# google-research/se3ds

Measured on AMD Instinct MI355X. Metric: panoramas/sec (G+D train step) at 512x1024 RGB-D, higher is better.
Workload: dtype bf16; 1 GPU; configs/highres 512x1024 full GAN step train_g_d (G+D+hinge+depth+wc losses, clip, Adam, EMA), ResNet-101 gen_dims 128, per-GPU batch 8, d_step_per_g_step 1; per_gpu_batch=8, global_batch=8, parallelism=dp1

## Files before the change

### include/se3ds_hip.h

```cpp
#ifndef SE3DS_HIP_H_
#define SE3DS_HIP_H_

#include <stddef.h>
#include <stdint.h>

#ifdef __cplusplus
extern "C" {
#endif

#define SE3DS_OK 0
#define SE3DS_E_BADSHAPE (-1)
#define SE3DS_E_BADDTYPE (-2)
#define SE3DS_E_WORKSPACE (-3)
#define SE3DS_E_LAUNCH (-4)
#define SE3DS_E_UNSUPPORTED (-5)

#define SE3DS_F32 0
#define SE3DS_I32 1
#define SE3DS_U8 2
#define SE3DS_BF16 3
#define SE3DS_FEAT_BYTE_RANGE 0x100
#define SE3DS_XYZ1_ONES_PRESET 0x200

const char* se3ds_version(void);
// ... 31 lines not shown
                                  int feat_dtype, int n, int64_t m, int64_t capacity, int channels,
                                  int height, int width, float depth_scale, float input_void,
                                  float output_void, float* depth, float* feat, float* mask,
                                  float mask_void, void* workspace, size_t workspace_bytes,
                                  void* stream);

int se3ds_warp_views_to_target(const void* const* view_feats, int feat_dtype,
                               const float* const* view_depth, const float* const* view_position,
                               int views, int n, int height, int width, int channels,
                               float void_class, float depth_scale, const float* sin_el,
                               const float* cos_el, const float* sin_hd, const float* cos_hd,
                               float* mem_xyz1, void* mem_feats, int64_t capacity, int64_t m_offset,
                               const float* target, int out_height, int out_width,
                               float output_void, float* depth, float* feat, float* mask,
                               float mask_void, void* workspace, size_t workspace_bytes,
                               void* stream);

int se3ds_project_to_feat(const float* coords, const void* feats, int feat_dtype, int n, int64_t m,
                          int channels, int height, int width, float depth_scale,
                          float input_void, float output_void, float* depth, float* feat,
                          float* mask, float mask_void, void* workspace, size_t workspace_bytes,
                          void* stream);

int se3ds_splat_debug_indices(const void* workspace, int n, int64_t m, int32_t* idx_out,
                              float* z_out, void* stream);

int se3ds_debug_fast_fxy(const float* xyz, int64_t m, int width, int height, float* fx, float* fy,
                         int32_t* verdict, void* stream);

int se3ds_unproject_perspective(const int32_t* feats, const float* depth, const float* xs,
                                const float* ys, const float* kinv, int n, int height, int width,
                                int channels, float depth_scale, float* xyz, float* feats_out,
                                void* stream);

int se3ds_interp_bilinear(const float* grid, const float* query, int b, int height, int width,
                          int channels, int64_t q, int indexing_xy, float* out, void* stream);

int se3ds_rotate_coords(const float* rays, const float* matrix, int n, int64_t q, int src_h,
                        int src_w, float* out, void* stream);

int se3ds_perspective_coords(const float* rays, const float* w2i, int64_t q, int round_nearest,
                             float add, float* out, void* stream);

int se3ds_persp_from_equirect_coords(const float* kinv_t, const float* rot, int height, int width,
                                     int eq_h, int eq_w, float* out, void* stream);

int se3ds_perspective_to_pointcloud(const float* image, const float* depth, int ih, int iw,
                                    int channels, const float* rays, const float* w2i,
                                    int round_nearest, float pad_value, const float* sin_el,
                                    const float* cos_el, const float* sin_hd, const float* cos_hd,
                                    const float* position, int height, int width, float void_class,
                                    float depth_scale, float* xyz1, int32_t* feats_out, void* stream);
int se3ds_perspective_guidance(const float* pred_rgb, const float* pred_depth, int eq_h, int eq_w,
                               const float* kinv_t, const float* rot, int height, int width,
                               float* proj_image, float* proj_depth, float* proj_mask,
                               void* stream);

int se3ds_resize(const void* x, int dtype, int n, int h, int w, int c, int oh, int ow, int method,
                 void* y, void* stream);
int se3ds_mean_f32(const float* x, int64_t n, float* out, void* stream);

int se3ds_mask_pano(const void* pano, int dtype, int n, int height, int width, int channels,
                    int masked_height, float value, void* out, void* stream);

size_t se3ds_compact_workspace_bytes(int64_t m);
int se3ds_compact_valid(const float* xyz1, const void* feats, int feat_dtype, int n, int64_t m,
                        int channels, float void_class, float* xyz1_out, void* feats_out,
                        int64_t* count_out, void* workspace, size_t workspace_bytes, void* stream);


int se3ds_weight_prep(const float* w, int64_t k, int cout, int dtype, void* wt, void* wn,
                      void* stream);
#define SE3DS_WEIGHT_PREP_FIELDS 6
int se3ds_weight_prep_multi(const int64_t* table, int nlayers, int64_t total_tiles, void* stream);

int se3ds_conv2d_fwd(const void* x, const void* wt, void* y, int dtype, int n, int h, int w,
                     int cin, int ho, int wo, int cout, int kh, int kw, int stride, int pad_t,
                     int pad_l, int wrap_w, const float* in_mask, int in_mask_binary,
                     const float* scale, const float* bias, const float* row_a,
                     const float* row_b, int act, float act_alpha, void* stream);

int se3ds_conv_transpose2x2_fwd(const void* x, const void* wn, void* y, int dtype, int n, int hi, int wi,
                                int cin, int cout, const float* bias, void* stream);

int64_t se3ds_conv2d_fwd_stats_rows(int dtype, int n, int cin, int ho, int wo, int cout, int kh,
                                    int kw, int stride, int has_in_mask, int in_mask_binary);
int se3ds_conv2d_fwd_stats(const void* x, const void* wt, void* y, int dtype, int n, int h, int w,
                           int cin, int ho, int wo, int cout, int kh, int kw, int stride,
                           int pad_t, int pad_l, int wrap_w, const float* in_mask,
                           int in_mask_binary, const float* scale, const float* bias,
                           const float* row_a, const float* row_b, int act, float act_alpha,
                           float* stats, void* stream);

int se3ds_conv2d_dgrad(const void* dy, const void* wn, void* dx, int dtype, int n, int h, int w,
                       int cin, int ho, int wo, int cout, int kh, int kw, int stride, int pad_t,
                       int pad_l, int wrap_w, const float* dy_row_scale, const float* scale,
                       const float* bias, const float* row_a, int act, float act_alpha,
                       void* stream);
int se3ds_conv2d_dgrad_acc(const void* dy, const void* wn, void* dx, int dtype, int n, int h, int w,
                       int cin, int ho, int wo, int cout, int kh, int kw, int stride, int pad_t,
                       int pad_l, int wrap_w, const float* dy_row_scale, const float* scale,
                       const float* bias, const float* row_a, int act, float act_alpha,
                       const void* addend, void* stream);

int64_t se3ds_conv2d_dgrad_bnstats_rows(int dtype, int n, int h, int w, int cin, int cout, int kh,
                                        int kw, int stride, int has_row_scale);
int se3ds_conv2d_dgrad_bnstats(const void* dy, const void* wn, void* dx, int dtype, int n, int h,
                               int w, int cin, int ho, int wo, int cout, int kh, int kw, int stride,
                               int pad_t, int pad_l, int wrap_w, const float* scale,
                               const float* row_a, const void* addend, const void* bn_x,
                               const uint8_t* bn_mask, const float* bn_mean, const float* bn_rstd,
                               int bn_act, float bn_alpha, float* stats, void* stream);

size_t se3ds_conv2d_wgrad_workspace_bytes(int n, int ho, int wo, int cin, int cout, int kh,
                                          int kw);
int se3ds_conv2d_wgrad(const void* x, const void* dy, float* dw, int dtype, int n, int h, int w,
                       int cin, int ho, int wo, int cout, int kh, int kw, int stride, int pad_t,
                       int pad_l, int wrap_w, const float* in_mask, int in_mask_binary,
                       const float* row_scale, const float* out_scale, int accumulate,
                       void* workspace, size_t workspace_bytes, void* stream);
int se3ds_conv2d_wgrad_partial(const void* x, const void* dy, float* dw, int dtype, int n, int h,
                               int w, int cin, int ho, int wo, int cout, int kh, int kw, int stride,
                               int pad_t, int pad_l, int wrap_w, const float* in_mask,
                               int in_mask_binary, const float* row_scale, void* workspace,
                               size_t workspace_bytes, int64_t* reduce_row, void* stream);
int se3ds_wgrad_reduce_multi(const int64_t* table, int rows, int64_t workgroups, void* stream);
int se3ds_wgrad_reduce_tile(void);
uint32_t se3ds_fastdiv_host(uint32_t n, uint32_t d);
int se3ds_debug_last_conv_route(void);
int se3ds_debug_conv_route_history(int back);
const char* se3ds_debug_conv_route_name(int route);

size_t se3ds_conv2d_wgrad_swapped_workspace_bytes(int n, int h, int w, int cin, int cout, int k);
int se3ds_conv2d_wgrad_swapped(const void* x, const void* dy, float* dw, int dtype, int n, int h,
                               int w, int cin, int cout, int k, int pad, int accumulate,
                               void* workspace, size_t workspace_bytes, void* stream);

int se3ds_mask_window(const float* mask, int n, int h, int w, int ho, int wo, int kh, int kw,
                      int stride, int pad_t, int pad_l, int wrap_w, float* ratio, float* um,
                      float* ru, float* bu, void* stream);

int se3ds_norm_reduce_rows_finalize(const float* partial, int64_t rows, int c, float count,
                                    const float* gamma, const float* beta, float eps, float momentum,
                                    float* moving_mean, float* moving_var, float* scale, float* shift,
                                    float* mean, float* rstd, void* stream);

int se3ds_colsum_row_scale(const void* x, int dtype, int64_t r, int c, const float* sum_row_scale,
                           const float* out_row_scale, void* scaled_out, float* sums,
                           float* colsum_out, void* workspace, size_t workspace_bytes,
                           void* stream);

size_t se3ds_norm_workspace_bytes(int g, int c);
int se3ds_norm_stats(const void* x, int dtype, int g, int64_t r, int c, const float* row_scale,
                     float* sums, float* colsum_out, void* workspace, size_t workspace_bytes,
                     void* stream);
int se3ds_norm_reduce_rows(const float* partial, int64_t rows, int c, float* sums, void* workspace,
                           size_t workspace_bytes, void* stream);
int se3ds_norm_reduce_rows_dst(const float* partial, int64_t rows, int c, float* sums, float* dst0,
                               float* dst1, void* workspace, size_t workspace_bytes, void* stream);
int se3ds_norm_finalize(const float* sums, float count, int g, int c, const float* gamma,
                        const float* beta, float eps, float momentum, float* moving_mean,
                        float* moving_var, int use_moving, float* scale, float* shift, float* mean,
                        float* rstd, void* stream);
int se3ds_norm_apply(const void* x, int dtype, int g, int64_t r, int c, const float* scale,
                     const float* shift, const void* res, const void* post, int act, float alpha,
                     void* y, void* act_mask, void* stream);
int se3ds_norm_bwd_stats(const void* dy, const void* y, const void* x, int dtype, int g, int64_t r,
                         int c, const float* mean, const float* rstd, int act, float alpha,
                         float* sums, float* dbeta_out, float* dgamma_out, const void* act_mask,
                         void* workspace, size_t workspace_bytes, void* stream);
int se3ds_norm_bwd_apply(const void* dy, const void* y, const void* x, int dtype, int g, int64_t r,
                         int c, const float* mean, const float* rstd, const float* gamma,
                         const float* sums, float count, int act, float alpha, void* dx,
                         void* dres, const void* act_mask, int in_act, float in_alpha,
                         void* stream);
int se3ds_norm_bwd_apply_rows(const void* dy, const void* x, int dtype, int64_t r, int c,
                              const float* mean, const float* rstd, const float* gamma,
                              const float* sums, float count, int act, float alpha, void* dx,
                              void* dres, const void* act_mask, const float* sum_row,
                              const float* out_row, float* colsum_dst, void* workspace,
                              size_t workspace_bytes, void* stream);
int se3ds_norm_bwd_cg_supported(int dtype, int64_t r, int c, int act, int has_mask, int in_act);
size_t se3ds_norm_bwd_cg_workspace_bytes(int c);
int se3ds_norm_bwd_cg_col_rows(int64_t r, int c);
int se3ds_norm_bwd_cg(const void* dy, const void* x, int dtype, int64_t r, int c, const float* mean,
                      const float* rstd, const float* gamma, float count, int act, float alpha,
                      void* dx, void* dres, const void* act_mask, int in_act, float in_alpha,
                      float* dbeta_out, float* dgamma_out, float* sums_out, const float* sum_row,
                      const float* out_row, float* colpart, void* workspace, size_t workspace_bytes,
                      void* stream);
int se3ds_affine_bwd(const void* dy, const void* y, int dtype, int g, int64_t r, int c,
                     const float* scale, int act, float alpha, void* dx, void* dres,
                     const void* act_mask, void* stream);

int se3ds_act_bwd(const void* dy, const void* y, int dtype, int64_t n, int act, float alpha,
                  void* dx, void* stream);
int se3ds_add(const void* a, const void* b, int dtype, int64_t n, void* out, void* stream);
int se3ds_row_scale(const void* x, int dtype, int64_t rows, int c, const float* scale, void* out,
                    void* stream);
int se3ds_maxpool2x2_fwd(const void* x, int dtype, int n, int h, int w, int c, void* y,
                         void* stream);
int se3ds_maxpool2x2_bwd(const void* dy, const void* x, const void* y, int dtype, int n, int h,
                         int w, int c, void* dx, void* stream);
int se3ds_avgpool3s2_fwd(const void* x, int dtype, int n, int h, int w, int c, void* y,
                         void* stream);
int se3ds_avgpool3s2_bwd(const void* dy, int dtype, int n, int h, int w, int c, void* dx,
                         void* stream);
int se3ds_upsample2x_fwd(const void* x, int dtype, int n, int h, int w, int c, void* y,
                         void* stream);
int se3ds_upsample2x_bwd(const void* dy, int dtype, int n, int h, int w, int c, void* dx,
                         void* stream);
int se3ds_copy_channels(const void* src, int src_dtype, int src_c, int src_c0, void* dst,
                        int dst_dtype, int dst_c, int dst_c0, int ncopy, int64_t rows,
                        void* stream);
int se3ds_fill(void* p, int dtype, int64_t n, float value, void* stream);
int se3ds_quantize(const void* in, int in_dtype, int64_t n, int pre_clamp, float pre_lo,
                   float pre_hi, float mul, float div, float lo, float hi, void* out, int out_dtype,
                   void* stream);
int se3ds_pad2d(const void* x, int dtype, int n, int h, int w, int c, int pad, int mode, int wrap_w,
// ... 204 lines not shown
```

### se3ds_amd/csrc/common.h

```cpp
#pragma once
#include <hip/hip_runtime.h>
#include <stdint.h>

#include "../../include/se3ds_hip.h"

namespace se3ds {

void set_last_error(hipError_t e, const char* where);

inline int check_launch(const char* where) {
  hipError_t e = hipGetLastError();
  if (e != hipSuccess) {
    set_last_error(e, where);
    return SE3DS_E_LAUNCH;
  }
  return SE3DS_OK;
}

#define SE3DS_CONV_ROUTES(X)                                                                      \
  X(thin_s2_dgrad) X(thin_cin_fwd) X(thin_cout_dgrad) X(thin_cout_fwd)                             \
  X(halo256_fwd_m16) X(halo256_dgrad_m16) X(halo256_dgrad_bn_m16)                                  \
  X(halo256_fwd_m32) X(halo256_dgrad_m32) X(halo256_dgrad_bn_m32)                                  \
  X(halo128_fwd_m16) X(halo128_dgrad_m16) X(halo128_dgrad_bn_m16)                                  \
  X(halo128_fwd_m32) X(halo128_dgrad_m32) X(halo128_dgrad_bn_m32)                                  \
  X(big256_fwd_m16) X(big256_dgrad_m16) X(big256_dgrad_bn_m16)                                     \
  X(big256_fwd_m32) X(big256_dgrad_m32) X(big256_dgrad_bn_m32)                                     \
  X(big128_fwd_m16) X(big128_dgrad_m16) X(big128_dgrad_bn_m16)                                     \
  X(big128_fwd_m32) X(big128_dgrad_m32) X(big128_dgrad_bn_m32)                                     \
  X(glds_f32_fwd) X(glds_f32_dgrad)                                                                \
  X(glds_bf16_fwd_m16) X(glds_bf16_dgrad_m16) X(glds_bf16_dgrad_bn_m16)                            \
  X(glds_bf16_fwd_m32) X(glds_bf16_dgrad_m32) X(glds_bf16_dgrad_bn_m32)                            \
  X(igemm_f32_fwd) X(igemm_f32_dgrad) X(igemm_bf16_fwd) X(igemm_bf16_dgrad)                        \
  X(wgrad_taps3_m16) X(wgrad_taps3_m32) X(wgrad_taps_wrap) X(thin_cin_wgrad)                       \
  X(wgrad_glds_f32) X(wgrad_glds_bf16) X(wgrad_f32) X(wgrad_bf16)                                  \
  X(wgrad_reduce_vec) X(wgrad_reduce_scalar) X(wgrad_reduce_multi)                                 \
  X(thin_cout_wgrad_t2) X(thin_cout_wgrad_t3) X(thin_cout_wgrad_t4) X(thin_cout_wgrad_t5)          \
  X(pad_channels8) X(wgrad_taps_thin) X(wgrad_swap_fixup)                                          \
  X(weight_prep_f32) X(weight_prep_bf16) X(weight_prep_vec) X(weight_prep_multi)
enum ConvRoute {
#define SE3DS_ROUTE_ENUM(name) kRoute_##name,
  SE3DS_CONV_ROUTES(SE3DS_ROUTE_ENUM)
#undef SE3DS_ROUTE_ENUM
  kConvRouteCount
};
void note_conv_route(int route);
#define SE3DS_LAUNCH(route, ...)                       \
  do {                                                 \
    ::se3ds::note_conv_route(::se3ds::kRoute_##route); \
    hipLaunchKernelGGL(__VA_ARGS__);                   \
  } while (0)

inline hipStream_t as_stream(void* s) { return reinterpret_cast<hipStream_t>(s); }

constexpr int kWave = 64;

__host__ __device__ inline int64_t ceil_div(int64_t a, int64_t b) { return (a + b - 1) / b; }

inline int grid_for(int64_t work_items, int block) {
  int64_t g = ceil_div(work_items, block);
  if (g < 1) g = 1;
  if (g > 256 * 16) g = 256 * 16;
  return (int)g;
}

__device__ __forceinline__ float bf16_to_f32(uint16_t h) {
  return __uint_as_float(((uint32_t)h) << 16);
}
typedef float se3ds_f32x2 __attribute__((ext_vector_type(2)));
typedef __bf16 se3ds_bf16x2 __attribute__((ext_vector_type(2)));
__device__ __forceinline__ uint32_t pack2_bf16(float a, float b) {
  const se3ds_f32x2 v = {a, b};
  return __builtin_bit_cast(uint32_t, __builtin_convertvector(v, se3ds_bf16x2));
}
__device__ __forceinline__ uint16_t f32_to_bf16(float f) {
  return (uint16_t)(pack2_bf16(f, f) & 0xffffu);
}

__device__ __forceinline__ float wave_sum(float v) {
#pragma unroll
  for (int o = 32; o > 0; o >>= 1) v += __shfl_xor(v, o, 64);
  return v;
}
__device__ __forceinline__ uint32_t wave_min_u32(uint32_t v) {
#pragma unroll
  for (int o = 32; o > 0; o >>= 1) {
    uint32_t t = (uint32_t)__shfl_xor((int)v, o, 64);
    v = t < v ? t : v;
  }
  return v;
}
__device__ __forceinline__ uint32_t wave_max_u32(uint32_t v) {
#pragma unroll
  for (int o = 32; o > 0; o >>= 1) {
    uint32_t t = (uint32_t)__shfl_xor((int)v, o, 64);
    v = t > v ? t : v;
  }
  return v;
}

template <typename T> struct VT;
template <> struct VT<float> {
  static constexpr int V = 4;
  static __device__ __forceinline__ void load(const float* p, float (&o)[4]) {
    float4 v = *reinterpret_cast<const float4*>(p);
    o[0] = v.x; o[1] = v.y; o[2] = v.z; o[3] = v.w;
  }
  static __device__ __forceinline__ void store(float* p, const float (&o)[4]) {
    *reinterpret_cast<float4*>(p) = make_float4(o[0], o[1], o[2], o[3]);
  }
  static __device__ __forceinline__ float ld1(const float* p) { return *p; }
  static __device__ __forceinline__ void st1(float* p, float v) { *p = v; }
};
template <> struct VT<uint16_t> {
  static constexpr int V = 8;
  static __device__ __forceinline__ void load(const uint16_t* p, float (&o)[8]) {
    uint4 v = *reinterpret_cast<const uint4*>(p);
    const uint32_t q[4] = {v.x, v.y, v.z, v.w};
#pragma unroll
    for (int e = 0; e < 4; ++e) {
      o[2 * e] = __uint_as_float(q[e] << 16);
      o[2 * e + 1] = __uint_as_float(q[e] & 0xffff0000u);
    }
  }
  static __device__ __forceinline__ void store(uint16_t* p, const float (&o)[8]) {
    uint32_t q[4];
#pragma unroll
    for (int e = 0; e < 4; ++e)
      q[e] = pack2_bf16(o[2 * e], o[2 * e + 1]);
    *reinterpret_cast<uint4*>(p) = make_uint4(q[0], q[1], q[2], q[3]);
  }
  static __device__ __forceinline__ float ld1(const uint16_t* p) { return bf16_to_f32(*p); }
  static __device__ __forceinline__ void st1(uint16_t* p, float v) { *p = f32_to_bf16(v); }
};

__device__ __forceinline__ float act_apply(float v, int act, float alpha) {
  if (act == 1) return v > 0.f ? v : 0.f;
  if (act == 2) return v > 0.f ? v : v * alpha;
  return v;
}
__device__ __forceinline__ float act_grad_from_out(float y, int act, float alpha) {
  if (act == 1) return y > 0.f ? 1.f : 0.f;
  if (act == 2) return y > 0.f ? 1.f : alpha;
  return 1.f;
}
__device__ __forceinline__ float act_grad_from_bit(unsigned bit, int act, float alpha) {
  if (act == 1) return bit ? 1.f : 0.f;
  if (act == 2) return bit ? 1.f : alpha;
  return 1.f;
}

}
```

### se3ds_amd/csrc/conv.hip

```cpp
#include <stdlib.h>

#include <cmath>
#include <type_traits>
#include "common.h"

namespace se3ds {
namespace {

typedef __attribute__((ext_vector_type(8))) __bf16 bf16x8_t;
typedef __attribute__((ext_vector_type(4))) short s16x4_t;
typedef __attribute__((ext_vector_type(16))) float f32x16_t;

constexpr int BM = 128;
constexpr int BN = 128;
constexpr int kThreads = 256;
constexpr int ROWB = 64;
constexpr int TILE_BYTES = 128 * ROWB;

enum { MODE_FWD = 0, MODE_DGRAD = 1 };

template <typename T> struct TT;
template <> struct TT<float> {
  static constexpr int EPC = 4;
  static constexpr int BK = 16;
  static __device__ __forceinline__ float to_f(float v) { return v; }
  static __device__ __forceinline__ float from_f(float v) { return v; }
};
template <> struct TT<uint16_t> {
  static constexpr int EPC = 8;
  static constexpr int BK = 32;
  static __device__ __forceinline__ float to_f(uint16_t v) { return bf16_to_f32(v); }
  static __device__ __forceinline__ uint16_t from_f(float v) { return f32_to_bf16(v); }
};

struct FastDiv { uint32_t m, s1, s2; };
inline FastDiv make_fastdiv(uint32_t d) {
  FastDiv f;
  if (d == 0) d = 1;
  uint32_t l = 0;
  while (l < 32 && ((uint64_t)1 << l) < d) ++l;
  f.m = (uint32_t)((((uint64_t)1 << 32) * (((uint64_t)1 << l) - d)) / d + 1);
  f.s1 = l < 1 ? l : 1;
  f.s2 = l - f.s1;
  return f;
}
__device__ __forceinline__ uint32_t fd_div(uint32_t n, const FastDiv& f) {
  const uint32_t t = __umulhi(n, f.m);
  return (t + ((n - t) >> f.s1)) >> f.s2;
}

struct IgemmParams {
  const void* src; int sH, sW, sC;
  const void* w; int64_t w_tap, w_n;
  void* out;
  int N, oH, oW, oC;
  int kh, kw, stride, pad_t, pad_l, wrap_w;
  int n_classes; int cls_tile_start[5]; int cls_py[4], cls_px[4];
  FastDiv fd_hw[4], fd_w[4];
  const float* src_mask;
  int mask_binary;
  const float* scale;
  const float* bias;
  const float* row_a;
  const float* row_b;
  int act; float act_alpha;
  int vec;
  int halo_ty, halo_tx;
  float* stats;
  const void* addend;
  const uint16_t* bn_x; const uint8_t* bn_mask; const float* bn_mean; const float* bn_rstd;
  int bn_act; float bn_alpha;
  int64_t o_pitch, o_off;
  int bias_mod;
#ifdef SE3DS_PROBE
  int probe;
#endif
};

__device__ __forceinline__ int swz(int row, int chunk) { return chunk ^ ((row >> 2) & 3); }

__device__ __forceinline__ void pix_of(const IgemmParams& p, int cls, int64_t m, int cH, int cW, int& n,
                                       int& a, int& b) {
  const uint32_t mu = (uint32_t)m;
  const uint32_t nn = fd_div(mu, p.fd_hw[cls]);
  const uint32_t rem = mu - nn * (uint32_t)(cH * cW);
  const uint32_t aa = fd_div(rem, p.fd_w[cls]);
  n = (int)nn; a = (int)aa; b = (int)(rem - aa * (uint32_t)cW);
}

template <typename T>
__device__ __forceinline__ void mfma_tile(f32x16_t (&acc)[2][2], const uint4 (&wf)[2][2],
                                          const uint4 (&xf)[2][2]);

template <>
__device__ __forceinline__ void mfma_tile<uint16_t>(f32x16_t (&acc)[2][2],
                                                    const uint4 (&wf)[2][2],
                                                    const uint4 (&xf)[2][2]) {
#pragma unroll
  for (int ks = 0; ks < 2; ++ks)
#pragma unroll
    for (int i = 0; i < 2; ++i)
#pragma unroll
      for (int j = 0; j < 2; ++j)
        acc[i][j] = __builtin_amdgcn_mfma_f32_32x32x16_bf16(
            __builtin_bit_cast(bf16x8_t, wf[i][ks]), __builtin_bit_cast(bf16x8_t, xf[j][ks]),
            acc[i][j], 0, 0, 0);
}

template <>
__device__ __forceinline__ void mfma_tile<float>(f32x16_t (&acc)[2][2], const uint4 (&wf)[2][2],
                                                 const uint4 (&xf)[2][2]) {
#pragma unroll
  for (int ks = 0; ks < 2; ++ks)
#pragma unroll
    for (int e = 0; e < 4; ++e)
#pragma unroll
      for (int i = 0; i < 2; ++i)
#pragma unroll
        for (int j = 0; j < 2; ++j) {
          const uint32_t wa = e == 0 ? wf[i][ks].x : e == 1 ? wf[i][ks].y
                            : e == 2 ? wf[i][ks].z : wf[i][ks].w;
          const uint32_t xb = e == 0 ? xf[j][ks].x : e == 1 ? xf[j][ks].y
                            : e == 2 ? xf[j][ks].z : xf[j][ks].w;
          acc[i][j] = __builtin_amdgcn_mfma_f32_32x32x2f32(__uint_as_float(wa),
                                                           __uint_as_float(xb), acc[i][j], 0, 0, 0);
        }
}

constexpr int kFlushSteps = 4;
template <typename T>
__device__ __forceinline__ void flush_acc(f32x16_t (&tot)[2][2], f32x16_t (&acc)[2][2]) {
  if constexpr (sizeof(T) == 4) {
#pragma unroll
    for (int i = 0; i < 2; ++i)
#pragma unroll
      for (int j = 0; j < 2; ++j)
#pragma unroll
        for (int r = 0; r < 16; ++r) {
          tot[i][j][r] += acc[i][j][r];
          acc[i][j][r] = 0.f;
        }
  }
}

struct RowInfo {
  int n, a, b;
  bool valid;
};

template <typename T, int NI>
__device__ __forceinline__ void store_pixel(const IgemmParams& p, f32x16_t (&acc)[NI][2], int j,
                                            int64_t opix, int co_base, int half, float scale) {
  using tt = TT<T>;
  T* __restrict__ out = (T*)p.out;
  const float ra = p.row_a ? p.row_a[opix] : 1.0f;
  const float rb = p.row_b ? p.row_b[opix] : 1.0f;
#pragma unroll
  for (int i = 0; i < NI; ++i)
#pragma unroll
    for (int g = 0; g < 4; ++g) {
      const int co = co_base + i * 32 + g * 8 + half * 4;
      float v[4];
// ... 102 lines not shown
            if (o < 0) pk = make_uint2(0u, 0u);
            if (mine)
              *reinterpret_cast<uint2*>(scratch + lp * RB + (i * 32 + g * 8 + half * 4) * 2) = pk;
          }
      };
      if (form == 0) emit(std::integral_constant<int, 0>());
      else if (form == 1) emit(std::integral_constant<int, 1>());
      else if (form == 2) emit(std::integral_constant<int, 2>());
      else emit(std::integral_constant<int, 3>());
      __builtin_amdgcn_wave_barrier();
      if (NI == 2 && NPASS == 1 && stats_row != nullptr && !bnb) {
#pragma unroll 8
        for (int px = 0; px < PXC; ++px) {
          const float v = bf16_to_f32(*reinterpret_cast<const uint16_t*>(scratch + px * RB + lane * 2));
          cs1 += v;
          cs2 += v * v;
        }
      }
#pragma unroll
      for (int k = 0; k < PXC / PPI; ++k) {
        const int px = k * PPI + lane / LPP, c16 = lane % LPP;
        uint4 v = *reinterpret_cast<const uint4*>(scratch + px * RB + c16 * 16);
        const int64_t po = offs[px];
        if (po >= 0) {
          if (p.addend) {
            const uint4 a = *reinterpret_cast<const uint4*>((const uint16_t*)p.addend + po * p.oC +
                                                            co_base + c16 * 8);
            uint32_t* vw = reinterpret_cast<uint32_t*>(&v);
            const uint32_t* aw = reinterpret_cast<const uint32_t*>(&a);
#pragma unroll
            for (int q = 0; q < 4; ++q) {
              const float lo = __uint_as_float(vw[q] << 16) + __uint_as_float(aw[q] << 16);
              const float hi = __uint_as_float(vw[q] & 0xffff0000u) + __uint_as_float(aw[q] & 0xffff0000u);
              vw[q] = pack2_bf16(lo, hi);
            }
          }
          *reinterpret_cast<uint4*>(out + po * p.oC + co_base + c16 * 8) = v;
          if (BNB && NI == 2 && bnb) {
            const int64_t e0 = po * p.oC + co_base + c16 * 8;
            const uint4 xr = *reinterpret_cast<const uint4*>(p.bn_x + e0);
            const unsigned mb = p.bn_mask ? p.bn_mask[e0 >> 3] : 0xffu;
            const uint32_t* vw = reinterpret_cast<const uint32_t*>(&v);
            const uint32_t* xw = reinterpret_cast<const uint32_t*>(&xr);
#pragma unroll
            for (int q = 0; q < 4; ++q) {
              const float d0 = __uint_as_float(vw[q] << 16) *
                               act_grad_from_bit((mb >> (2 * q)) & 1u, p.bn_act, p.bn_alpha);
              const float d1 = __uint_as_float(vw[q] & 0xffff0000u) *
                               act_grad_from_bit((mb >> (2 * q + 1)) & 1u, p.bn_act, p.bn_alpha);
              const float x0 = __uint_as_float(xw[q] << 16), x1 = __uint_as_float(xw[q] & 0xffff0000u);
              bs1[2 * q] += d0;
              bs2[2 * q] += d0 * (x0 - bmu[2 * q]);
              bs1[2 * q + 1] += d1;
              bs2[2 * q + 1] += d1 * (x1 - bmu[2 * q + 1]);
            }
          }
        }
      }
      __builtin_amdgcn_wave_barrier();
    }
  }
  if (BNB && NI == 2 && bnb) {
#pragma unroll
    for (int e = 0; e < 8; ++e) {
#pragma unroll
      for (int m = 8; m < 64; m <<= 1) {
        bs1[e] += __shfl_xor(bs1[e], m, 64);
        bs2[e] += __shfl_xor(bs2[e], m, 64);
      }
    }
    if (lane < 8) {
      float* r1 = stats_row + co_base + lane * 8;
      float* r2 = stats_row + p.oC + co_base + lane * 8;
      const float4 ra4 = *reinterpret_cast<const float4*>(p.bn_rstd + co_base + lane * 8);
      const float4 rb4 = *reinterpret_cast<const float4*>(p.bn_rstd + co_base + lane * 8 + 4);
      bs2[0] *= ra4.x; bs2[1] *= ra4.y; bs2[2] *= ra4.z; bs2[3] *= ra4.w;
      bs2[4] *= rb4.x; bs2[5] *= rb4.y; bs2[6] *= rb4.z; bs2[7] *= rb4.w;
      *reinterpret_cast<float4*>(r1) = make_float4(bs1[0], bs1[1], bs1[2], bs1[3]);
      *reinterpret_cast<float4*>(r1 + 4) = make_float4(bs1[4], bs1[5], bs1[6], bs1[7]);
      *reinterpret_cast<float4*>(r2) = make_float4(bs2[0], bs2[1], bs2[2], bs2[3]);
      *reinterpret_cast<float4*>(r2 + 4) = make_float4(bs2[4], bs2[5], bs2[6], bs2[7]);
    }
  } else if (NI == 2 && stats_row != nullptr) {
    stats_row[co_base + lane] = cs1;
    stats_row[p.oC + co_base + lane] = cs2;
  }
}

typedef __attribute__((ext_vector_type(4))) float f32x4_t;
template <bool BNB = false, bool HOIST = false, bool BATCH = false>
__device__ __forceinline__ void store_wave_lds16(const IgemmParams& p, f32x4_t (&acc)[4][4],
                                                 const int64_t (&opix)[4], int co_base, int lane,
                                                 unsigned char* scratch, float* stats_row = nullptr) {
  constexpr int NI = 2, PXC = 32;
  constexpr int RB = NI * 64;
  constexpr int LPP = NI * 4;
  constexpr int PPI = 64 / LPP;
  const float scale = p.scale ? *p.scale : 1.0f;
  const int g = lane >> 4, c16 = lane & 15;
  const float slope = p.act == 0 ? 1.0f : (p.act == 1 ? 0.0f : p.act_alpha);
  uint16_t* __restrict__ out = (uint16_t*)p.out;
  int64_t* offs = reinterpret_cast<int64_t*>(scratch + PXC * RB);
  float4 bv[4];
#pragma unroll
  for (int i = 0; i < 4; ++i)
    bv[i] = p.bias ? *reinterpret_cast<const float4*>(
                         p.bias + (p.bias_mod ? (co_base + i * 16 + g * 4) % p.bias_mod : co_base + i * 16 + g * 4))
                   : make_float4(0.f, 0.f, 0.f, 0.f);
  const int form = p.row_a ? (p.bias ? 3 : 2) : (p.bias ? 1 : 0);
  float ra4[4], rb4[4];
  if (HOIST) {
#pragma unroll
    for (int j = 0; j < 4; ++j) {
      const int64_t oc = opix[j] < 0 ? 0 : opix[j];
      ra4[j] = p.row_a ? p.row_a[oc] : 1.0f;
      rb4[j] = p.row_b ? p.row_b[oc] : 1.0f;
    }
  }
  float cs1 = 0.f, cs2 = 0.f;
  const bool bnb = BNB && stats_row != nullptr && p.bn_x != nullptr;
  float bs1[8], bs2[8], bmu[8];
  if (BNB && bnb) {
    const int c0 = co_base + (lane % LPP) * 8;
#pragma unroll
    for (int h4 = 0; h4 < 2; ++h4) {
      const float4 m4 = *reinterpret_cast<const float4*>(p.bn_mean + c0 + h4 * 4);
      bmu[h4 * 4] = m4.x; bmu[h4 * 4 + 1] = m4.y; bmu[h4 * 4 + 2] = m4.z; bmu[h4 * 4 + 3] = m4.w;
    }
#pragma unroll
    for (int e = 0; e < 8; ++e) { bs1[e] = 0.f; bs2[e] = 0.f; }
  }
#pragma unroll
  for (int J = 0; J < 2; ++J) {
#pragma unroll
    for (int jj = 0; jj < 2; ++jj) {
      const int j = J * 2 + jj;
      const int64_t o = opix[j];
      const int64_t oc = o < 0 ? 0 : o;
      const float ra = HOIST ? ra4[j] : (p.row_a ? p.row_a[oc] : 1.0f);
      const float rb = HOIST ? rb4[j] : (p.row_b ? p.row_b[oc] : 1.0f);
      const int lp = jj * 16 + c16;
      if (g == 0) offs[lp] = o;
      auto emit = [&](auto form_c) {
        constexpr int F = decltype(form_c)::value;
#pragma unroll
        for (int i = 0; i < 4; ++i) {
          const float b4[4] = {bv[i].x, bv[i].y, bv[i].z, bv[i].w};
          float v[4];
#pragma unroll
          for (int e = 0; e < 4; ++e) {
            float t = acc[i][j][e] * scale;
            if (F == 1) t = t + b4[e];
            else if (F == 2) t = t * ra;
            else if (F == 3) t = ((t - b4[e]) * ra + b4[e]) * rb;
            v[e] = t > 0.f ? t : t * slope;
          }
          uint2 pk;
          pk.x = pack2_bf16(v[0], v[1]);
          pk.y = pack2_bf16(v[2], v[3]);
          if (o < 0) pk = make_uint2(0u, 0u);
          *reinterpret_cast<uint2*>(scratch + lp * RB + (((2 * i + (g >> 1)) ^ (lp & 7)) << 4) + (g & 1) * 8) = pk;
        }
      };
      if (form == 0) emit(std::integral_constant<int, 0>());
      else if (form == 1) emit(std::integral_constant<int, 1>());
      else if (form == 2) emit(std::integral_constant<int, 2>());
      else emit(std::integral_constant<int, 3>());
    }
// ... 41 lines not shown
          for (int q = 0; q < 4; ++q) {
            const float lo = __uint_as_float(vw[q] << 16) + __uint_as_float(aw[q] << 16);
            const float hi = __uint_as_float(vw[q] & 0xffff0000u) + __uint_as_float(aw[q] & 0xffff0000u);
            vw[q] = pack2_bf16(lo, hi);
          }
        }
      }
#pragma unroll
      for (int k = 0; k < NK; ++k)
        if (po[k] >= 0) *reinterpret_cast<uint4*>(out + po[k] * p.oC + co_base + c8 * 8) = vv[k];
    } else {
#pragma unroll
    for (int k = 0; k < PXC / PPI; ++k) {
      const int px = k * PPI + lane / LPP, c8 = lane % LPP;
      uint4 v = *reinterpret_cast<const uint4*>(scratch + px * RB + ((c8 ^ (px & 7)) << 4));
      const int64_t po = offs[px];
      if (po >= 0) {
        if (p.addend) {
          const uint4 a = *reinterpret_cast<const uint4*>((const uint16_t*)p.addend + po * p.oC +
                                                          co_base + c8 * 8);
          uint32_t* vw = reinterpret_cast<uint32_t*>(&v);
          const uint32_t* aw = reinterpret_cast<const uint32_t*>(&a);
#pragma unroll
          for (int q = 0; q < 4; ++q) {
            const float lo = __uint_as_float(vw[q] << 16) + __uint_as_float(aw[q] << 16);
            const float hi = __uint_as_float(vw[q] & 0xffff0000u) + __uint_as_float(aw[q] & 0xffff0000u);
            vw[q] = pack2_bf16(lo, hi);
          }
        }
#ifdef SE3DS_PROBE
        if (p.probe == 3) {
          typedef __attribute__((ext_vector_type(4))) uint32_t u32x4_t;
          __builtin_nontemporal_store(__builtin_bit_cast(u32x4_t, v),
                                      reinterpret_cast<u32x4_t*>(out + po * p.oC + co_base + c8 * 8));
        } else
#endif
        *reinterpret_cast<uint4*>(out + po * p.oC + co_base + c8 * 8) = v;
        if (BNB && bnb) {
          const int64_t e0 = po * p.oC + co_base + c8 * 8;
          const uint4 xr = *reinterpret_cast<const uint4*>(p.bn_x + e0);
          const unsigned mb = p.bn_mask ? p.bn_mask[e0 >> 3] : 0xffu;
          const uint32_t* vw = reinterpret_cast<const uint32_t*>(&v);
          const uint32_t* xw = reinterpret_cast<const uint32_t*>(&xr);
#pragma unroll
          for (int q = 0; q < 4; ++q) {
            const float d0 = __uint_as_float(vw[q] << 16) *
                             act_grad_from_bit((mb >> (2 * q)) & 1u, p.bn_act, p.bn_alpha);
            const float d1 = __uint_as_float(vw[q] & 0xffff0000u) *
                             act_grad_from_bit((mb >> (2 * q + 1)) & 1u, p.bn_act, p.bn_alpha);
            const float x0 = __uint_as_float(xw[q] << 16), x1 = __uint_as_float(xw[q] & 0xffff0000u);
            bs1[2 * q] += d0;
            bs2[2 * q] += d0 * (x0 - bmu[2 * q]);
            bs1[2 * q + 1] += d1;
            bs2[2 * q + 1] += d1 * (x1 - bmu[2 * q + 1]);
          }
        }
      }
    }
    }
    __builtin_amdgcn_wave_barrier();
  }
  if (BNB && bnb) {
#pragma unroll
    for (int e = 0; e < 8; ++e) {
#pragma unroll
      for (int m = 8; m < 64; m <<= 1) {
        bs1[e] += __shfl_xor(bs1[e], m, 64);
        bs2[e] += __shfl_xor(bs2[e], m, 64);
      }
    }
    if (lane < 8) {
      float* r1 = stats_row + co_base + lane * 8;
      float* r2 = stats_row + p.oC + co_base + lane * 8;
      const float4 ra4 = *reinterpret_cast<const float4*>(p.bn_rstd + co_base + lane * 8);
      const float4 rb4 = *reinterpret_cast<const float4*>(p.bn_rstd + co_base + lane * 8 + 4);
      bs2[0] *= ra4.x; bs2[1] *= ra4.y; bs2[2] *= ra4.z; bs2[3] *= ra4.w;
      bs2[4] *= rb4.x; bs2[5] *= rb4.y; bs2[6] *= rb4.z; bs2[7] *= rb4.w;
      *reinterpret_cast<float4*>(r1) = make_float4(bs1[0], bs1[1], bs1[2], bs1[3]);
      *reinterpret_cast<float4*>(r1 + 4) = make_float4(bs1[4], bs1[5], bs1[6], bs1[7]);
      *reinterpret_cast<float4*>(r2) = make_float4(bs2[0], bs2[1], bs2[2], bs2[3]);
      *reinterpret_cast<float4*>(r2 + 4) = make_float4(bs2[4], bs2[5], bs2[6], bs2[7]);
    }
  } else if (stats_row != nullptr) {
    stats_row[co_base + lane] = cs1;
    stats_row[p.oC + co_base + lane] = cs2;
  }
}

template <int NI, bool BNB = false>
__device__ __forceinline__ void store_wave_lds(const IgemmParams& p, f32x16_t (&acc)[NI][2],
                                               const int64_t (&opix)[2], int co_base, int lane,
                                               unsigned char* scratch, float* stats_row = nullptr) {
  const float scale = p.scale ? *p.scale : 1.0f;
  auto bias4 = [&](int cl) {
    return p.bias ? *reinterpret_cast<const float4*>(
                        p.bias + (p.bias_mod ? (co_base + cl) % p.bias_mod : co_base + cl))
                  : make_float4(0.f, 0.f, 0.f, 0.f);
  };
  store_wave_lds_impl<NI, 32, BNB>(p, acc, opix, co_base, lane, scratch, scale, bias4, stats_row);
}

template <typename T, int MODE, int NI = 2, bool BNB = false>
__device__ __forceinline__ void store_tile(const IgemmParams& p, f32x16_t (&acc)[NI][2],
                                           int64_t m_base, int co_base, int64_t Mc, int cH, int cW,
                                           int py, int px, int half, int l32,
                                           unsigned char* scratch = nullptr,
                                           float* stats_row = nullptr, int cls = 0) {
  const int s = p.stride;
  const float scale = p.scale ? *p.scale : 1.0f;
  int64_t opix[2];
#pragma unroll
  for (int j = 0; j < 2; ++j) {
    int64_t m = m_base + j * 32 + l32;
    opix[j] = -1;
    if (m >= Mc) continue;
    int n, a, b;
    pix_of(p, cls, m, cH, cW, n, a, b);
    if (MODE == MODE_DGRAD) { a = py + a * s; b = px + b * s; }
    opix[j] = ((int64_t)n * p.oH + a) * p.o_pitch + p.o_off + b;
  }
  if (sizeof(T) == 2 && scratch != nullptr && (p.oC & 7) == 0 && co_base + NI * 32 <= p.oC) {
    if (NI == 4 && stats_row != nullptr) {
      store_wave_lds<2, BNB>(p, *reinterpret_cast<f32x16_t(*)[2][2]>(&acc[0]), opix, co_base,
                             half * 32 + l32, scratch, stats_row);
      store_wave_lds<2, BNB>(p, *reinterpret_cast<f32x16_t(*)[2][2]>(&acc[NI - 2]), opix,
                             co_base + 64, half * 32 + l32, scratch, stats_row);
    } else {
      store_wave_lds<NI, BNB>(p, acc, opix, co_base, half * 32 + l32, scratch, stats_row);
    }
    return;
  }
#pragma unroll
  for (int j = 0; j < 2; ++j)
    if (opix[j] >= 0) store_pixel<T, NI>(p, acc, j, opix[j], co_base, half, scale);
}

template <int MODE, int CB, bool BNB = false>
__device__ __forceinline__ void store_tile16(const IgemmParams& p, f32x4_t (&acc)[CB][4], int64_t m_base,
                                             int co_base, int64_t Mc, int cH, int cW, int py, int px,
                                             int lane, unsigned char* scratch, float* stats_row,
                                             int cls = 0) {
  const int s = p.stride;
  int64_t opix[4];
#pragma unroll
  for (int j = 0; j < 4; ++j) {
    const int64_t m = m_base + j * 16 + (lane & 15);
    opix[j] = -1;
    if (m >= Mc) continue;
    int n, a, b;
    pix_of(p, cls, m, cH, cW, n, a, b);
    if (MODE == MODE_DGRAD) { a = py + a * s; b = px + b * s; }
    opix[j] = ((int64_t)n * p.oH + a) * p.o_pitch + p.o_off + b;
  }
  store_wave_lds16<BNB, true, true>(p, *reinterpret_cast<f32x4_t(*)[4][4]>(&acc[0]), opix, co_base, lane,
                                    scratch, stats_row);
  if (CB == 8)
    store_wave_lds16<BNB, true, true>(p, *reinterpret_cast<f32x4_t(*)[4][4]>(&acc[CB - 4]), opix, co_base + 64,
                                      lane, scratch, stats_row);
}

template <typename T, int MODE>
__global__ void __launch_bounds__(kThreads, 2)
igemm_kernel(const IgemmParams p) {
  using tt = TT<T>;
  constexpr int EPC = tt::EPC, BK = tt::BK;
  __shared__ __attribute__((aligned(16))) unsigned char smem[4 * TILE_BYTES];
  const int tid = threadIdx.x;
  const int lane = tid & 63, wave = tid >> 6;
// ... 2443 lines not shown
        d[0] = make_uint2(v[u].x, v[u].y);
        d[1] = make_uint2(v[u].z, v[u].w);
      }
    }
    {
      constexpr int kB = 2;
      const int npix = PH * PW;
      for (int q0 = tid; q0 < npix; q0 += kB * NT) {
        uint16_t v[kB][kThinCinMax];
        float mk[kB];
#pragma unroll
        for (int u = 0; u < kB; ++u) {
          const int pix = q0 + u * NT;
          mk[u] = 1.0f;
#pragma unroll
          for (int c = 0; c < kThinCinMax; ++c) v[u][c] = 0;
          if (pix < npix) {
            const int r = pix / PW, q = pix - r * PW;
            const int sy = oy0 * st - p.pad_t + r;
            int sx = ox0 * st - p.pad_l + q;
            if (p.wrap_w) sx = sx < 0 ? sx + p.W : (sx >= p.W ? sx - p.W : sx);
            if (sy >= 0 && sy < p.H && sx >= 0 && sx < p.W) {
              const int64_t sp = ((int64_t)n * p.H + sy) * p.W + sx;
              const uint16_t* px = p.x + sp * Ci;
#pragma unroll
              for (int c = 0; c < kThinCinMax; ++c)
                if (c < Ci) v[u][c] = px[c];
              if (p.src_mask) mk[u] = p.src_mask[sp];
            }
          }
        }
#pragma unroll
        for (int u = 0; u < kB; ++u) {
          const int pix = q0 + u * NT;
          if (pix < npix) {
#pragma unroll
            for (int c = 0; c < kThinCinMax; ++c)
              if (c < Ci)
                xs[pix * Ci + c] = p.src_mask ? f32_to_bf16(bf16_to_f32(v[u][c]) * mk[u]) : v[u][c];
          }
        }
      }
    }
    __syncthreads();
    for (int sidx = 0; sidx < PX / 16; ++sidx) {
      const int row = sidx >> 1, col0 = (sidx & 1) * 16 + half * 8;
      uint16_t eb[8];
      const unsigned char* dp = dys + (row * kThinCols + col0) * DYS + (nb * 32 + l32) * 2;
#pragma unroll
      for (int j = 0; j < 8; ++j) eb[j] = *reinterpret_cast<const uint16_t*>(dp + j * DYS);
      const uint4 bf = make_uint4((uint32_t)eb[0] | ((uint32_t)eb[1] << 16), (uint32_t)eb[2] | ((uint32_t)eb[3] << 16),
                                  (uint32_t)eb[4] | ((uint32_t)eb[5] << 16), (uint32_t)eb[6] | ((uint32_t)eb[7] << 16));
      const int xbase = (row * st * PW + col0 * st) * Ci;
#pragma unroll
      for (int i = 0; i < 4; ++i) {
        if (((wave + 8 * i) >> 2) >= MB) break;
        uint16_t ea[8];
#pragma unroll
        for (int j = 0; j < 8; ++j) ea[j] = xs[xbase + ko[i] + j * st * Ci];
        const uint4 af = make_uint4((uint32_t)ea[0] | ((uint32_t)ea[1] << 16), (uint32_t)ea[2] | ((uint32_t)ea[3] << 16),
                                    (uint32_t)ea[4] | ((uint32_t)ea[5] << 16), (uint32_t)ea[6] | ((uint32_t)ea[7] << 16));
        acc[i] = __builtin_amdgcn_mfma_f32_32x32x16_bf16(__builtin_bit_cast(bf16x8_t, af),
                                                         __builtin_bit_cast(bf16x8_t, bf), acc[i], 0, 0,
                                                         0);
      }
    }
  }
  float* slab = p.part + (int64_t)blockIdx.x * K * 128;
#pragma unroll
  for (int i = 0; i < 4; ++i) {
    const int mb = (wave + 8 * i) >> 2;
    if (mb >= MB) break;
#pragma unroll
    for (int e = 0; e < 16; ++e) {
      const int k = mb * 32 + (e >> 2) * 8 + half * 4 + (e & 3);
      if (k < K) slab[(int64_t)k * 128 + nb * 32 + l32] = acc[i][e];
    }
  }
}

struct ThinCoutWgradParams {
  const uint16_t* x; const uint16_t* dy; float* part;
  int N, H, W, Cin, Cout, pad;
};
constexpr int kThinQRows = 8, kThinQSlabs = 256;
__host__ __device__ inline int thin_cw_pixel_bytes(int cin) { return cin * 2 + 32; }
__host__ __device__ inline size_t thin_cout_wgrad_lds(int cin) {
  return (size_t)(kThinQRows + 2) * (kThinCols + 2) * thin_cw_pixel_bytes(cin) +
         (size_t)kThinQRows * kThinCols * 4 * 2;
}
template <int MAXT>
__global__ void __launch_bounds__(kThinWThreads)
thin_cout_wgrad_kernel(const ThinCoutWgradParams p) {
  typedef __attribute__((address_space(3))) s16x4_t* lds_seg;
  constexpr int NT = kThinWThreads, PX = kThinQRows * kThinCols;
  constexpr int PH = kThinQRows + 2, PW = kThinCols + 2;
  extern __shared__ __attribute__((aligned(16))) unsigned char tq_smem[];
  const int Ci = p.Cin, Co = p.Cout, PB = thin_cw_pixel_bytes(Ci);
  unsigned char* xs = tq_smem;
  uint16_t* dys = reinterpret_cast<uint16_t*>(tq_smem + (size_t)PH * PW * PB);
  const int tid = threadIdx.x, lane = tid & 63;
  const int wave = __builtin_amdgcn_readfirstlane(tid >> 6);
  const int half = lane >> 5, l32 = lane & 31;
  const int g16 = (lane >> 4) & 1, i16 = lane & 15, jrow = i16 >> 2, qcol = i16 & 3;
  const int cblocks = Ci / 32, ntile = 9 * cblocks;
  f32x16_t acc[MAXT];
#pragma unroll
  for (int i = 0; i < MAXT; ++i)
#pragma unroll
    for (int e = 0; e < 16; ++e) acc[i][e] = 0.f;
  int xoff[MAXT];
#pragma unroll
  for (int i = 0; i < MAXT; ++i) {
    int t = wave + 8 * i;
    t = t < ntile ? t : ntile - 1;
    const int tap = t / cblocks, cb = t - tap * cblocks;
    const int ky = tap / 3, kx = tap - ky * 3;
    xoff[i] = (ky * PW + kx + half * 8 + jrow) * PB + (cb * 32 + g16 * 16 + qcol * 4) * 2;
  }
  const int tiles_x = ceil_div(p.W, kThinCols), tiles_y = ceil_div(p.H, kThinQRows);
  const int64_t n_tiles = (int64_t)p.N * tiles_y * tiles_x;
  constexpr int NV = (PH * PW * 16 + NT - 1) / NT;
  const int cpp = Ci / 8, total = PH * PW * cpp;
  const bool pow2 = (cpp & (cpp - 1)) == 0;
  const int csh = 31 - __builtin_clz((unsigned)cpp);
  const int fc = tid & (cpp - 1), fp0 = tid >> csh, fpp = NT >> csh;
  auto chunk_of = [&](int u, int& pix, int& c) -> bool {
    if (pow2) {
      pix = fp0 + u * fpp; c = fc;
      return pix < PH * PW;
    }
    const int i = tid + u * NT;
    pix = i / cpp; c = i - pix * cpp;
    return i < total;
  };
  const uint32_t utiles_x = (uint32_t)tiles_x, utiles_y = (uint32_t)tiles_y;
  auto tile_pos = [&](uint32_t t, int& n, int& oy0, int& ox0) {
    const uint32_t ty_n = t / utiles_x;
    ox0 = (int)(t - ty_n * utiles_x) * kThinCols;
    const uint32_t nn = ty_n / utiles_y;
    oy0 = (int)(ty_n - nn * utiles_y) * kThinQRows;
    n = (int)nn;
  };
  uint4 nxt[NV];
  constexpr int ND = (PX * 4 + NT - 1) / NT;
  uint16_t nxd[ND];
  const int rowlen = kThinCols * Co;
  auto fetch = [&](int64_t tile) {
    int n, oy0, ox0;
    tile_pos((uint32_t)tile, n, oy0, ox0);
#pragma unroll
    for (int u = 0; u < ND; ++u) {
      const int i = tid + u * NT;
      nxd[u] = 0;
      if (i < kThinQRows * rowlen) {
        const int ry = i / rowlen, e = i - ry * rowlen;
        const int oy = oy0 + ry, ox_e = ox0 * Co + e;
        if (oy < p.H && ox_e < p.W * Co) nxd[u] = p.dy[((int64_t)n * p.H + oy) * p.W * Co + ox_e];
      }
    }
    const int sy0 = oy0 - p.pad, sx0 = ox0 - p.pad;
    const bool interior = sy0 >= 0 && sy0 + PH <= p.H && sx0 >= 0 && sx0 + PW <= p.W;
    const int64_t base = (((int64_t)n * p.H + sy0) * p.W + sx0) * Ci;
#pragma unroll
    for (int u = 0; u < NV; ++u) {
      int pix, c;
      nxt[u] = make_uint4(0u, 0u, 0u, 0u);
      if (chunk_of(u, pix, c)) {
        const int r = pix / PW, q = pix - r * PW;
        if (interior || ((unsigned)(sy0 + r) < (unsigned)p.H && (unsigned)(sx0 + q) < (unsigned)p.W))
          nxt[u] = *reinterpret_cast<const uint4*>(p.x + (base + (int64_t)((r * p.W + q) * Ci + c * 8)));
      }
    }
  };
  if ((int64_t)blockIdx.x < n_tiles) fetch(blockIdx.x);
  for (int64_t tile = blockIdx.x; tile < n_tiles; tile += gridDim.x) {
    int n, oy0, ox0;
    tile_pos((uint32_t)tile, n, oy0, ox0);
    __syncthreads();
#pragma unroll
    for (int u = 0; u < ND; ++u) {
      const int i = tid + u * NT;
      if (i < kThinQRows * rowlen) {
        const int ry = i / rowlen, e = i - ry * rowlen;
        int cx, c;
        switch (Co) {
          case 1: cx = e; c = 0; break;
          case 2: cx = e >> 1; c = e & 1; break;
          case 3: cx = e / 3; c = e - cx * 3; break;
          default: cx = e >> 2; c = e & 3; break;
        }
        dys[c * PX + ry * kThinCols + cx] = nxd[u];
      }
    }
#pragma unroll
    for (int u = 0; u < NV; ++u) {
      int pix, c;
      if (chunk_of(u, pix, c)) *reinterpret_cast<uint4*>(xs + pix * PB + c * 16) = nxt[u];
    }
    __syncthreads();
    if (tile + gridDim.x < n_tiles) fetch(tile + gridDim.x);
#pragma unroll 2
    for (int sidx = 0; sidx < PX / 16; ++sidx) {
      const int row = sidx >> 1, cs = (sidx & 1) * 16;
      uint4 af = make_uint4(0u, 0u, 0u, 0u);
      if (l32 < Co)
        af = *reinterpret_cast<const uint4*>(dys + l32 * PX + row * kThinCols + cs + half * 8);
      const unsigned char* sp = xs + (row * PW + cs) * PB;
      uint4 bf[MAXT];
#pragma unroll
      for (int i = 0; i < MAXT; ++i) {
        const unsigned char* xp = sp + xoff[i];
        const uint2 b0 = __builtin_bit_cast(uint2, __builtin_amdgcn_ds_read_tr16_b64_v4i16((lds_seg)xp));
        const uint2 b1 = __builtin_bit_cast(
            uint2, __builtin_amdgcn_ds_read_tr16_b64_v4i16((lds_seg)(xp + 4 * PB)));
        bf[i] = make_uint4(b0.x, b0.y, b1.x, b1.y);
      }
#pragma unroll
      for (int i = 0; i < MAXT; ++i)
        acc[i] = __builtin_amdgcn_mfma_f32_32x32x16_bf16(__builtin_bit_cast(bf16x8_t, af),
                                                         __builtin_bit_cast(bf16x8_t, bf[i]), acc[i], 0,
                                                         0, 0);
    }
  }
  float* slab = p.part + (int64_t)blockIdx.x * 9 * Ci * Co;
  if (half == 0) {
#pragma unroll
    for (int i = 0; i < MAXT; ++i) {
      const int t = wave + 8 * i;
      if (t >= ntile) break;
      const int tap = t / cblocks, cb = t - tap * cblocks;
#pragma unroll
      for (int c = 0; c < 4; ++c)
        if (c < Co) slab[((int64_t)tap * Ci + cb * 32 + l32) * Co + c] = acc[i][c];
    }
  }
}

constexpr int kThinFRows = 16, kThinFThreads = 512;
struct ThinCinLds {
  int kp, ws, ph, pw;
  size_t xs_off, wk_off, koff_off, bytes;
};
__host__ __device__ inline ThinCinLds thin_cin_lds(int kh, int kw, int cin, int stride) {
  ThinCinLds l;
  l.kp = (kh * kw * cin + 15) / 16 * 16;
  l.ws = l.kp + 8;
  l.ph = (kThinFRows - 1) * stride + kh;
  l.pw = (kThinCols - 1) * stride + kw;
  l.xs_off = (size_t)(kThinFThreads / 64) * kEpiScratch<2>;
  l.wk_off = l.xs_off + ((size_t)l.ph * l.pw * cin * 2 + 15) / 16 * 16;
  l.koff_off = l.wk_off + (size_t)128 * l.ws * 2;
  l.bytes = l.koff_off + (size_t)l.kp * 2;
  return l;
}
__global__ void __launch_bounds__(kThinFThreads)
thin_cin_fwd_kernel(const IgemmParams p) {
  constexpr int NI = 4, NT = kThinFThreads;
  extern __shared__ __attribute__((aligned(16))) unsigned char tc_smem[];
  const ThinCinLds L = thin_cin_lds(p.kh, p.kw, p.sC, p.stride);
  unsigned char* scratch = tc_smem;
  uint16_t* xs = reinterpret_cast<uint16_t*>(tc_smem + L.xs_off);
  uint16_t* wk = reinterpret_cast<uint16_t*>(tc_smem + L.wk_off);
  int16_t* koff = reinterpret_cast<int16_t*>(tc_smem + L.koff_off);
  const int tid = threadIdx.x, lane = tid & 63;
  const int wave = __builtin_amdgcn_readfirstlane(tid >> 6);
  const int half = lane >> 5, l32 = lane & 31;
  const int Ci = p.sC, K = p.kh * p.kw * Ci, KP = L.kp, WS = L.ws;
  const int st = p.stride;
  const int PH = L.ph, PW = L.pw;
  const int tiles_x = ceil_div(p.oW, kThinCols), tiles_y = ceil_div(p.oH, kThinFRows);
  const int64_t n_tiles = (int64_t)p.N * tiles_y * tiles_x;
  const uint16_t* __restrict__ src = (const uint16_t*)p.src;
  const uint16_t* __restrict__ wt = (const uint16_t*)p.w;
  for (int k = tid; k < KP; k += NT) {
    int o = 0;
    if (k < K) {
      const int tap = k / Ci, ci = k - tap * Ci;
      const int ky = tap / p.kw, kx = tap - ky * p.kw;
      o = (ky * PW + kx) * Ci + ci;
    }
// ... 32 lines not shown
            int sx = ox0 * st - p.pad_l + q;
            if (p.wrap_w) sx = sx < 0 ? sx + p.sW : (sx >= p.sW ? sx - p.sW : sx);
            if (sy >= 0 && sy < p.sH && sx >= 0 && sx < p.sW) {
              const int64_t sp = ((int64_t)n * p.sH + sy) * p.sW + sx;
              const uint16_t* px = src + sp * Ci;
#pragma unroll
              for (int c = 0; c < kThinCinMax; ++c)
                if (c < Ci) v[u][c] = px[c];
              if (p.src_mask) mk[u] = p.src_mask[sp];
            }
          }
        }
#pragma unroll
        for (int u = 0; u < kB; ++u) {
          const int pix = q0 + u * NT;
          if (pix < npix) {
#pragma unroll
            for (int c = 0; c < kThinCinMax; ++c)
              if (c < Ci)
                xs[pix * Ci + c] = p.src_mask ? f32_to_bf16(bf16_to_f32(v[u][c]) * mk[u]) : v[u][c];
          }
        }
      }
    }
    for (int g = 0; g < p.oC; g += NI * 32) {
      if (!one_group) {
        __syncthreads();
        load_weights(g);
      }
      __syncthreads();
      f32x16_t acc[NI][2];
#pragma unroll
      for (int i = 0; i < NI; ++i)
#pragma unroll
        for (int j = 0; j < 2; ++j)
#pragma unroll
          for (int e = 0; e < 16; ++e) acc[i][j][e] = 0.f;
      const int base0 = ((wave * 2) * st * PW + l32 * st) * Ci;
      const int base1 = base0 + st * PW * Ci;
      for (int ks = 0; ks < KP; ks += 16) {
        uint4 xf[2];
        int o[8];
#pragma unroll
        for (int q = 0; q < 8; ++q) o[q] = koff[ks + half * 8 + q];
#pragma unroll
        for (int j = 0; j < 2; ++j) {
          const int base = j ? base1 : base0;
          uint16_t e[8];
#pragma unroll
          for (int q = 0; q < 8; ++q) e[q] = xs[base + o[q]];
          xf[j] = make_uint4((uint32_t)e[0] | ((uint32_t)e[1] << 16), (uint32_t)e[2] | ((uint32_t)e[3] << 16),
                             (uint32_t)e[4] | ((uint32_t)e[5] << 16), (uint32_t)e[6] | ((uint32_t)e[7] << 16));
        }
#pragma unroll
        for (int i = 0; i < NI; ++i) {
          const uint4 wf = *reinterpret_cast<const uint4*>(&wk[(i * 32 + l32) * WS + ks + half * 8]);
#pragma unroll
          for (int j = 0; j < 2; ++j)
            acc[i][j] = __builtin_amdgcn_mfma_f32_32x32x16_bf16(__builtin_bit_cast(bf16x8_t, wf),
                                                                __builtin_bit_cast(bf16x8_t, xf[j]),
                                                                acc[i][j], 0, 0, 0);
        }
      }
      int64_t opix[2];
#pragma unroll
      for (int j = 0; j < 2; ++j) {
        const int oy = oy0 + wave * 2 + j, ox = ox0 + l32;
        opix[j] = (oy < p.oH && ox < p.oW) ? ((int64_t)n * p.oH + oy) * p.oW + ox : -1;
      }
      unsigned char* scr = scratch + wave * kEpiScratch<2>;
      store_wave_lds<2>(p, *reinterpret_cast<f32x16_t(*)[2][2]>(&acc[0]), opix, g, lane, scr);
      store_wave_lds<2>(p, *reinterpret_cast<f32x16_t(*)[2][2]>(&acc[2]), opix, g + 64, lane, scr);
    }
  }
}

constexpr int kThinRows = 4, kThinPH = kThinRows + 2, kThinPW = kThinCols + 2;
__host__ __device__ inline int thin_pixel_bytes(int cin) { return cin * 2 + 16; }
__host__ __device__ inline int thin_weight_bytes(int cin) { return 9 * cin * 2 + 16; }
__host__ __device__ inline size_t thin_lds_bytes(int cin, int cout) {
  return (size_t)kThinPH * kThinPW * thin_pixel_bytes(cin) + (size_t)(cout + 1) * thin_weight_bytes(cin);
}

__global__ void __launch_bounds__(256)
thin_cout_fwd_kernel(const IgemmParams p) {
  extern __shared__ __attribute__((aligned(16))) unsigned char t_smem[];
  const int C = p.sC, K = 9 * C;
  const int pstride = thin_pixel_bytes(C), wstride = thin_weight_bytes(C);
  unsigned char* xs = t_smem;
  unsigned char* ws = t_smem + kThinPH * kThinPW * pstride;
  const int tid = threadIdx.x, lane = tid & 63;
  const int wave = __builtin_amdgcn_readfirstlane(tid >> 6);
  const int half = lane >> 5, l32 = lane & 31;
  const int tiles_x = ceil_div(p.oW, kThinCols), tiles_y = ceil_div(p.oH, kThinRows);
  const int64_t n_tiles = (int64_t)p.N * tiles_y * tiles_x;
  const uint16_t* __restrict__ src = (const uint16_t*)p.src;
  {
    const uint16_t* __restrict__ w = (const uint16_t*)p.w;
    const int chunks = K / 8;
    for (int i = tid; i < p.oC * chunks; i += 256) {
      const int co = i / chunks, c = i - co * chunks;
      *reinterpret_cast<uint4*>(ws + co * wstride + c * 16) =
          *reinterpret_cast<const uint4*>(w + (int64_t)co * K + c * 8);
    }
    for (int i = tid; i < chunks; i += 256)
      *reinterpret_cast<uint4*>(ws + p.oC * wstride + i * 16) = make_uint4(0u, 0u, 0u, 0u);
  }
  constexpr int NV = (kThinPH * kThinPW * 16 + 255) / 256;
  const int cpp = C / 8;
  const int csh = 31 - __builtin_clz((unsigned)cpp);
  const int fc = tid & (cpp - 1), fp0 = tid >> csh, fpp = 256 >> csh;
  const uint32_t utiles_x = (uint32_t)tiles_x, utiles_y = (uint32_t)tiles_y;
  auto tile_pos = [&](uint32_t t, int& n, int& oy0, int& ox0) {
    const uint32_t ty_n = t / utiles_x;
    ox0 = (int)(t - ty_n * utiles_x) * kThinCols;
    const uint32_t nn = ty_n / utiles_y;
    oy0 = (int)(ty_n - nn * utiles_y) * kThinRows;
    n = (int)nn;
  };
  uint4 nxt[NV];
  auto fetch = [&](int64_t tile) {
    int n, oy0, ox0;
    tile_pos((uint32_t)tile, n, oy0, ox0);
    const int sy0 = oy0 - p.pad_t, sx0 = ox0 - p.pad_l;
    const bool interior = sy0 >= 0 && sy0 + kThinPH <= p.sH && sx0 >= 0 && sx0 + kThinPW <= p.sW;
    const int64_t rowbase = ((int64_t)n * p.sH + sy0) * p.sW;
#pragma unroll
    for (int u = 0; u < NV; ++u) {
      const int pix = fp0 + u * fpp;
      nxt[u] = make_uint4(0u, 0u, 0u, 0u);
      if (pix < kThinPH * kThinPW) {
        const int r = pix / kThinPW, q = pix - r * kThinPW;
        if (interior) {
          nxt[u] = *reinterpret_cast<const uint4*>(
              src + ((rowbase + sx0) * C + (int64_t)((r * p.sW + q) * C + fc * 8)));
        } else {
          int sx = sx0 + q;
          if (p.wrap_w) sx = sx < 0 ? sx + p.sW : (sx >= p.sW ? sx - p.sW : sx);
          if ((unsigned)(sy0 + r) < (unsigned)p.sH && (unsigned)sx < (unsigned)p.sW)
            nxt[u] = *reinterpret_cast<const uint4*>(
                src + ((rowbase + (int64_t)r * p.sW + sx) * C + fc * 8));
        }
      }
    }
  };
  if ((int64_t)blockIdx.x < n_tiles) fetch(blockIdx.x);
  for (int64_t tile = blockIdx.x; tile < n_tiles; tile += gridDim.x) {
  int n, oy0, ox0;
  tile_pos((uint32_t)tile, n, oy0, ox0);
  __syncthreads();
#pragma unroll
  for (int u = 0; u < NV; ++u) {
    const int pix = fp0 + u * fpp;
    if (pix < kThinPH * kThinPW) *reinterpret_cast<uint4*>(xs + pix * pstride + fc * 16) = nxt[u];
  }
  __syncthreads();
  if (tile + gridDim.x < n_tiles) fetch(tile + gridDim.x);
  f32x16_t acc;
#pragma unroll
  for (int i = 0; i < 16; ++i) acc[i] = 0.f;
  const int kc_n = C / 16;
  const bool wrow_ok = l32 < p.oC;
#pragma unroll
  for (int tap = 0; tap < 9; ++tap) {
    const int ky = tap / 3, kx = tap - ky * 3;
    const unsigned char* xrow = xs + ((wave + ky) * kThinPW + l32 + kx) * pstride + half * 16;
    const unsigned char* wrow = ws + (wrow_ok ? l32 : p.oC) * wstride + tap * C * 2 + half * 16;
    for (int kc = 0; kc < kc_n; kc += 4) {
      uint4 xf[4], wf[4];
#pragma unroll
      for (int u = 0; u < 4; ++u) {
        xf[u] = *reinterpret_cast<const uint4*>(xrow + (kc + u) * 32);
        wf[u] = *reinterpret_cast<const uint4*>(wrow + (kc + u) * 32);
      }
#pragma unroll
      for (int u = 0; u < 4; ++u)
        acc = __builtin_amdgcn_mfma_f32_32x32x16_bf16(__builtin_bit_cast(bf16x8_t, wf[u]),
                                                      __builtin_bit_cast(bf16x8_t, xf[u]), acc, 0,
                                                      0, 0);
    }
  }
  const int oy = oy0 + wave, ox = ox0 + l32;
  if (half == 0 && oy < p.oH && ox < p.oW) {
    const float scale = p.scale ? *p.scale : 1.0f;
    uint16_t* out = (uint16_t*)p.out + (((int64_t)n * p.oH + oy) * p.oW + ox) * p.oC;
#pragma unroll
    for (int c = 0; c < 4; ++c)
      if (c < p.oC) {
        float t = acc[c] * scale;
        if (p.bias) t = t + p.bias[c];
        if (p.act == 1) t = t > 0.f ? t : 0.f;
        else if (p.act == 2) t = t > 0.f ? t : t * p.act_alpha;
        out[c] = f32_to_bf16(t);
      }
  }
  }
}

template <typename T>
__global__ void __launch_bounds__(256)
weight_prep_kernel(const float* __restrict__ w, int64_t K, int Cout, T* __restrict__ wt,
                   T* __restrict__ wn) {
  __shared__ float tile[32][33];
  const int64_t k0 = (int64_t)blockIdx.x * 32;
  const int c0 = blockIdx.y * 32;
  const int tx = threadIdx.x & 31, ty = threadIdx.x >> 5;
  for (int r = ty; r < 32; r += 8) {
    int64_t k = k0 + r;
    int c = c0 + tx;
    float v = (k < K && c < Cout) ? w[k * Cout + c] : 0.0f;
    tile[r][tx] = v;
    if (wn && k < K && c < Cout) wn[k * Cout + c] = TT<T>::from_f(v);
  }
  __syncthreads();
  for (int r = ty; r < 32; r += 8) {
    int c = c0 + r;
    int64_t k = k0 + tx;
    if (c < Cout && k < K) wt[(int64_t)c * K + k] = TT<T>::from_f(tile[tx][r]);
  }
}

__global__ void __launch_bounds__(256)
weight_prep_vec_kernel(const float* __restrict__ w, int64_t K, int Cout, uint16_t* __restrict__ wt,
                       uint16_t* __restrict__ wn) {
  __shared__ float tile[64][65];
  const int64_t k0 = (int64_t)blockIdx.x * 64;
  const int c0 = blockIdx.y * 64;
  const int tid = threadIdx.x;
  {
    const int cq = (tid & 15) * 4, r0 = tid >> 4;
#pragma unroll
    for (int i = 0; i < 4; ++i) {
      const int r = r0 + 16 * i;
      const int64_t k = k0 + r;
      const int c = c0 + cq;
      float4 v = make_float4(0.f, 0.f, 0.f, 0.f);
      if (k < K && c < Cout) {
// ... 81 lines not shown
  return total;
}

}

void note_conv_route(int route) { t_route_ring[t_route_n++ % kRouteRing] = route; }

}

using namespace se3ds;


static bool thin_on() { return getenv("SE3DS_NO_THIN") == nullptr; }

static int big_tile_mode() {
  const char* e = getenv("SE3DS_BIG_TILE");
  return e ? atoi(e) : -1;
}

static int halo_tile_channels(const IgemmParams& p) {
  const char* e = getenv("SE3DS_HALO_TILE");
  const int mode = e ? atoi(e) : -1;
  if (mode == 0) return 0;
  if ((p.oC % 128) != 0) return 0;
  if (mode == 128 || (p.oC % 256) != 0) return 128;
  if (mode == 256) return 256;
  const int64_t tiles = (int64_t)p.N * ceil_div(p.oH, 8) * ceil_div(p.oW, 32);
  const int64_t items256 = tiles * (p.oC / 256);
  const double eff256 = (double)items256 / (double)(ceil_div(items256, (int64_t)256) * 256);
  const int64_t items128 = items256 * 2;
  const double eff128 = 0.85 * (double)items128 / (double)(ceil_div(items128, (int64_t)256) * 256);
  return eff256 >= eff128 ? 256 : 128;
}

static bool halo_m16() {
  const char* e = getenv("SE3DS_HALO_M16");
  return e ? atoi(e) != 0 : true;
}

static int big_tile_channels(const IgemmParams& p, int mode) {
  const int g_big_tile = big_tile_mode();
  if (g_big_tile == 0) return 0;
  const int co = (p.oC % 256) == 0 ? 256 : ((p.oC % 128) == 0 ? 128 : 0);
  if (!co) return 0;
  if (g_big_tile == 1) return co;
  int64_t m = 0;
  const int s = mode == MODE_FWD ? 1 : p.stride;
  for (int py = 0; py < s; ++py)
    for (int px = 0; px < s; ++px)
      m += (int64_t)p.N * ((p.oH - py + s - 1) / s) * ((p.oW - px + s - 1) / s);
  const double kCus = 256.0;
  const double big_items = (double)ceil_div(m, (int64_t)256) * (p.oC / co);
  const double small_items = (double)ceil_div(m, (int64_t)128) * ceil_div(p.oC, 128);
  if (co != 256) return 0;
  const double gain = 1.25;
  const double t_small = std::ceil(small_items / (2 * kCus)) * 2.0;
  const double t_big = std::ceil(big_items / kCus) * (co == 256 ? 4.0 : 2.0) / gain;
  return t_big < t_small ? co : 0;
}

static int64_t fwd_stats_rows(const IgemmParams& p, int dtype, int stride, int kh, int kw,
                              bool glds, int mode = MODE_FWD) {
  if (!glds || dtype != SE3DS_BF16) return 0;
  if (mode == MODE_DGRAD && stride != 1) return 0;
  const int64_t M = (int64_t)p.N * p.oH * p.oW;
  if (stride == 1 && kh == 3 && kw == 3 && halo_tile_channels(p))
    return (int64_t)p.N * ceil_div(p.oH, 8) * ceil_div(p.oW, 32) * 4;
  if (big_tile_channels(p, mode)) return ceil_div(M, (int64_t)256) * 4;
  if ((p.oC % BN) == 0) return ceil_div(M, (int64_t)BM) * (BM / 64);
  return 0;
}

extern "C" {

static int conv_common(int mode, const void* src, const void* w, void* out, int dtype, int n,
                       int h, int wdt, int cin, int ho, int wo, int cout, int kh, int kw,
                       int stride, int pad_t, int pad_l, int wrap_w, const float* src_mask,
                       int mask_binary, const float* scale, const float* bias, const float* row_a,
                       const float* row_b, int act, float act_alpha, void* stream,
                       float* stats = nullptr, const void* addend = nullptr,
                       const void* bn_x = nullptr, const uint8_t* bn_mask = nullptr,
                       const float* bn_mean = nullptr, const float* bn_rstd = nullptr,
                       int bn_act = 0, float bn_alpha = 0.f, int64_t o_pitch = 0, int64_t o_off = 0,
                       int bias_mod = 0) {
  if (n <= 0 || h <= 0 || wdt <= 0 || cin <= 0 || ho <= 0 || wo <= 0 || cout <= 0 || kh <= 0 ||
      kw <= 0 || stride <= 0 || stride > 2)
    return SE3DS_E_BADSHAPE;
  if (wrap_w && mode == MODE_DGRAD && (stride != 1 || wo != wdt)) return SE3DS_E_UNSUPPORTED;
  if (dtype != SE3DS_F32 && dtype != SE3DS_BF16) return SE3DS_E_BADDTYPE;
  if ((int64_t)n * h * wdt >= ((int64_t)1 << 31) || (int64_t)n * ho * wo >= ((int64_t)1 << 31))
    return SE3DS_E_BADSHAPE;
  IgemmParams p;
  p.src = src; p.w = w; p.out = out;
  p.N = n; p.kh = kh; p.kw = kw; p.stride = stride; p.pad_t = pad_t; p.pad_l = pad_l;
  p.wrap_w = wrap_w; p.src_mask = src_mask; p.mask_binary = mask_binary; p.scale = scale;
  p.bias = bias; p.row_a = row_a;
  p.row_b = row_b; p.act = act; p.act_alpha = act_alpha;
  const int bk = dtype == SE3DS_F32 ? 16 : 32;
  const int64_t K = (int64_t)kh * kw * cin;
  if (mode == MODE_FWD) {
    p.sH = h; p.sW = wdt; p.sC = cin; p.oH = ho; p.oW = wo; p.oC = cout;
    p.w_tap = cin; p.w_n = K;
  } else {
    p.sH = ho; p.sW = wo; p.sC = cout; p.oH = h; p.oW = wdt; p.oC = cin;
    p.w_tap = (int64_t)cin * cout; p.w_n = cout;
  }
  p.vec = (p.sC % bk) == 0;
  p.o_pitch = o_pitch > 0 ? o_pitch : p.oW;
  p.o_off = o_off;
  p.bias_mod = bias_mod;
  const bool pitched = o_pitch > 0 || bias_mod > 0;
#ifdef SE3DS_PROBE
  { const char* e = getenv("SE3DS_PROBE_MODE"); p.probe = e ? atoi(e) : 0; }
#endif
  p.stats = nullptr;
  p.addend = addend;
  hipStream_t s = as_stream(stream);
  const bool glds = (p.sC % (2 * bk)) == 0 && (src_mask == nullptr || mask_binary);
  if (stats != nullptr && !(fwd_stats_rows(p, dtype, stride, kh, kw, glds, mode) > 0))
    return SE3DS_E_UNSUPPORTED;
  if (stats != nullptr && mode == MODE_DGRAD &&
      (bn_x == nullptr || bn_mean == nullptr || bn_rstd == nullptr || (p.oC & 7) != 0))
    return SE3DS_E_UNSUPPORTED;
  p.stats = stats;
  p.bn_x = (mode == MODE_DGRAD && stats != nullptr) ? (const uint16_t*)bn_x : nullptr;
  p.bn_mask = bn_mask; p.bn_mean = bn_mean; p.bn_rstd = bn_rstd;
  p.bn_act = bn_act; p.bn_alpha = bn_alpha;
  if (mode == MODE_DGRAD && dtype == SE3DS_BF16 && kh == 4 && kw == 4 && stride == 2 && cin <= 4 &&
      cout == 128 && src_mask == nullptr && row_a == nullptr && bias == nullptr && act == 0 &&
      !wrap_w && (pad_t == 0 || pad_t == 2) && (pad_l == 0 || pad_l == 2) &&
      thin_on()) {
    int64_t blocks = (int64_t)p.N * ceil_div(p.oH, kThinSRows) * ceil_div(p.oW, kThinSCols);
    if (blocks > 2 * 256) blocks = 2 * 256;
    SE3DS_LAUNCH(thin_s2_dgrad, thin_s2_dgrad_kernel, dim3((unsigned)blocks), dim3(256), 0, s, p);
    return check_launch("conv2d_dgrad(thin s2)");
  }
  if (mode == MODE_FWD && dtype == SE3DS_BF16 && cin <= kThinCinMax && (cout % 128) == 0 &&
      kh * kw * cin <= kThinKMax && kh <= 7 && kw <= 7 && stats == nullptr && addend == nullptr &&
      !pitched && thin_on()) {
    const ThinCinLds L = thin_cin_lds(kh, kw, cin, stride);
    static size_t lds_set = 0;
    if (L.bytes > lds_set) {
      if (hipFuncSetAttribute((const void*)thin_cin_fwd_kernel,
                              hipFuncAttributeMaxDynamicSharedMemorySize, (int)L.bytes) != hipSuccess)
        return SE3DS_E_LAUNCH;
      lds_set = L.bytes;
    }
    int64_t blocks = (int64_t)p.N * ceil_div(p.oH, kThinFRows) * ceil_div(p.oW, kThinCols);
    const int64_t resident = 256;
    if (blocks > resident) blocks = resident;
    SE3DS_LAUNCH(thin_cin_fwd, thin_cin_fwd_kernel, dim3((unsigned)blocks), dim3(kThinFThreads),
                 L.bytes, s, p);
    return check_launch("conv2d_fwd(thin cin)");
  }
  if (mode == MODE_DGRAD && dtype == SE3DS_BF16 && kh == 3 && kw == 3 && stride == 1 && cout <= 4 &&
      (cin % 64) == 0 && cin <= kThinDCinMax && src_mask == nullptr && row_a == nullptr &&
      thin_on()) {
    int64_t blocks = (int64_t)p.N * ceil_div(p.oH, kThinDRows) * ceil_div(p.oW, kThinCols);
    if (blocks > 2 * 256) blocks = 2 * 256;
    SE3DS_LAUNCH(thin_cout_dgrad, thin_cout_dgrad_kernel, dim3((unsigned)blocks), dim3(256), 0, s, p);
    return check_launch("conv2d_dgrad(thin)");
  }
  if (mode == MODE_FWD && dtype == SE3DS_BF16 && kh == 3 && kw == 3 && stride == 1 && cout <= 4 &&
      (cin % 64) == 0 && cin <= 128 && src_mask == nullptr && row_a == nullptr &&
      stats == nullptr && addend == nullptr && thin_on()) {
    const size_t lds = thin_lds_bytes(cin, cout);
    static size_t lds_set = 0;
    if (lds > lds_set) {
      if (hipFuncSetAttribute((const void*)thin_cout_fwd_kernel,
                              hipFuncAttributeMaxDynamicSharedMemorySize, (int)lds) != hipSuccess)
        return SE3DS_E_LAUNCH;
      lds_set = lds;
    }
    int64_t blocks = (int64_t)p.N * ceil_div(p.oH, kThinRows) * ceil_div(p.oW, kThinCols);
    if (blocks > 2 * 256) blocks = 2 * 256;
    SE3DS_LAUNCH(thin_cout_fwd, thin_cout_fwd_kernel, dim3((unsigned)blocks), dim3(256), lds, s, p);
    return check_launch("conv2d_fwd(thin)");
  }
  if (glds && dtype == SE3DS_BF16 && stride == 1 && kh == 3 && kw == 3) {
    const int co = halo_tile_channels(p);
    if (co) {
      p.halo_ty = ceil_div(p.oH, 8);
      p.halo_tx = ceil_div(p.oW, 32);
      const int64_t items = (int64_t)p.N * p.halo_ty * p.halo_tx * (p.oC / co);
      dim3 grid((unsigned)(items < 256 ? items : 256));
      if (co == 256 && halo_m16()) {
        if (mode == MODE_FWD) SE3DS_LAUNCH(halo256_fwd_m16, (igemm_halo_kernel<MODE_FWD, 256, 2, false, true>), grid, dim3(512), 0, s, p);
        else if (p.bn_x) SE3DS_LAUNCH(halo256_dgrad_bn_m16, (igemm_halo_kernel<MODE_DGRAD, 256, 2, true, true>), grid, dim3(512), 0, s, p);
        else SE3DS_LAUNCH(halo256_dgrad_m16, (igemm_halo_kernel<MODE_DGRAD, 256, 2, false, true>), grid, dim3(512), 0, s, p);
      } else if (co == 256) {
        if (mode == MODE_FWD) SE3DS_LAUNCH(halo256_fwd_m32, (igemm_halo_kernel<MODE_FWD, 256, 2>), grid, dim3(512), 0, s, p);
        else if (p.bn_x) SE3DS_LAUNCH(halo256_dgrad_bn_m32, (igemm_halo_kernel<MODE_DGRAD, 256, 2, true>), grid, dim3(512), 0, s, p);
        else SE3DS_LAUNCH(halo256_dgrad_m32, (igemm_halo_kernel<MODE_DGRAD, 256, 2>), grid, dim3(512), 0, s, p);
      } else {
        if (halo_m16()) {
          if (mode == MODE_FWD) SE3DS_LAUNCH(halo128_fwd_m16, (igemm_halo_kernel<MODE_FWD, 128, 3, false, true>), grid, dim3(512), 0, s, p);
          else if (p.bn_x) SE3DS_LAUNCH(halo128_dgrad_bn_m16, (igemm_halo_kernel<MODE_DGRAD, 128, 3, true, true>), grid, dim3(512), 0, s, p);
          else SE3DS_LAUNCH(halo128_dgrad_m16, (igemm_halo_kernel<MODE_DGRAD, 128, 3, false, true>), grid, dim3(512), 0, s, p);
        } else if (mode == MODE_FWD) SE3DS_LAUNCH(halo128_fwd_m32, (igemm_halo_kernel<MODE_FWD, 128, 3>), grid, dim3(512), 0, s, p);
        else if (p.bn_x) SE3DS_LAUNCH(halo128_dgrad_bn_m32, (igemm_halo_kernel<MODE_DGRAD, 128, 3, true>), grid, dim3(512), 0, s, p);
        else SE3DS_LAUNCH(halo128_dgrad_m32, (igemm_halo_kernel<MODE_DGRAD, 128, 3>), grid, dim3(512), 0, s, p);
      }
      return check_launch(mode == MODE_FWD ? "conv2d_fwd(halo)" : "conv2d_dgrad(halo)");
    }
  }
  if (glds && dtype == SE3DS_BF16) {
    const int co = big_tile_channels(p, mode);
    if (co) {
      const int tiles = fill_classes(p, mode, 256);
      if (tiles <= 0) return SE3DS_OK;
      dim3 grid((unsigned)tiles, (unsigned)(p.oC / co));
      if (co == 256 && halo_m16()) {
        if (mode == MODE_FWD) SE3DS_LAUNCH(big256_fwd_m16, (igemm_big_kernel<MODE_FWD, 256, false, true>), grid, dim3(512), 0, s, p);
        else if (p.bn_x) SE3DS_LAUNCH(big256_dgrad_bn_m16, (igemm_big_kernel<MODE_DGRAD, 256, true, true>), grid, dim3(512), 0, s, p);
        else SE3DS_LAUNCH(big256_dgrad_m16, (igemm_big_kernel<MODE_DGRAD, 256, false, true>), grid, dim3(512), 0, s, p);
      } else if (co == 256) {
        if (mode == MODE_FWD) SE3DS_LAUNCH(big256_fwd_m32, (igemm_big_kernel<MODE_FWD, 256>), grid, dim3(512), 0, s, p);
        else if (p.bn_x) SE3DS_LAUNCH(big256_dgrad_bn_m32, (igemm_big_kernel<MODE_DGRAD, 256, true>), grid, dim3(512), 0, s, p);
        else SE3DS_LAUNCH(big256_dgrad_m32, (igemm_big_kernel<MODE_DGRAD, 256>), grid, dim3(512), 0, s, p);
      } else if (halo_m16()) {
        if (mode == MODE_FWD) SE3DS_LAUNCH(big128_fwd_m16, (igemm_big_kernel<MODE_FWD, 128, false, true>), grid, dim3(512), 0, s, p);
        else if (p.bn_x) SE3DS_LAUNCH(big128_dgrad_bn_m16, (igemm_big_kernel<MODE_DGRAD, 128, true, true>), grid, dim3(512), 0, s, p);
        else SE3DS_LAUNCH(big128_dgrad_m16, (igemm_big_kernel<MODE_DGRAD, 128, false, true>), grid, dim3(512), 0, s, p);
      } else {
        if (mode == MODE_FWD) SE3DS_LAUNCH(big128_fwd_m32, (igemm_big_kernel<MODE_FWD, 128>), grid, dim3(512), 0, s, p);
        else if (p.bn_x) SE3DS_LAUNCH(big128_dgrad_bn_m32, (igemm_big_kernel<MODE_DGRAD, 128, true>), grid, dim3(512), 0, s, p);
        else SE3DS_LAUNCH(big128_dgrad_m32, (igemm_big_kernel<MODE_DGRAD, 128>), grid, dim3(512), 0, s, p);
      }
      return check_launch(mode == MODE_FWD ? "conv2d_fwd(big)" : "conv2d_dgrad(big)");
    }
  }
  int tiles = fill_classes(p, mode);
  if (tiles <= 0) return SE3DS_OK;
  dim3 grid((unsigned)tiles, (unsigned)ceil_div(p.oC, BN));
  if (glds) {
    if (dtype == SE3DS_F32) {
      if (mode == MODE_FWD) SE3DS_LAUNCH(glds_f32_fwd, (igemm_glds_kernel<float, MODE_FWD>), grid, dim3(kThreads), 0, s, p);
      else SE3DS_LAUNCH(glds_f32_dgrad, (igemm_glds_kernel<float, MODE_DGRAD>), grid, dim3(kThreads), 0, s, p);
    } else {
      if ((p.oC % BN) == 0 && halo_m16()) {
        if (mode == MODE_FWD) SE3DS_LAUNCH(glds_bf16_fwd_m16, (igemm_glds_kernel<uint16_t, MODE_FWD, false, true>), grid, dim3(kThreads), 0, s, p);
        else if (p.bn_x) SE3DS_LAUNCH(glds_bf16_dgrad_bn_m16, (igemm_glds_kernel<uint16_t, MODE_DGRAD, true, true>), grid, dim3(kThreads), 0, s, p);
        else SE3DS_LAUNCH(glds_bf16_dgrad_m16, (igemm_glds_kernel<uint16_t, MODE_DGRAD, false, true>), grid, dim3(kThreads), 0, s, p);
      } else if (mode == MODE_FWD) SE3DS_LAUNCH(glds_bf16_fwd_m32, (igemm_glds_kernel<uint16_t, MODE_FWD>), grid, dim3(kThreads), 0, s, p);
      else if (p.bn_x) SE3DS_LAUNCH(glds_bf16_dgrad_bn_m32, (igemm_glds_kernel<uint16_t, MODE_DGRAD, true>), grid, dim3(kThreads), 0, s, p);
      else SE3DS_LAUNCH(glds_bf16_dgrad_m32, (igemm_glds_kernel<uint16_t, MODE_DGRAD>), grid, dim3(kThreads), 0, s, p);
    }
    return check_launch(mode == MODE_FWD ? "conv2d_fwd(glds)" : "conv2d_dgrad(glds)");
  }
  if (dtype == SE3DS_F32) {
    if (mode == MODE_FWD) SE3DS_LAUNCH(igemm_f32_fwd, (igemm_kernel<float, MODE_FWD>), grid, dim3(kThreads), 0, s, p);
    else SE3DS_LAUNCH(igemm_f32_dgrad, (igemm_kernel<float, MODE_DGRAD>), grid, dim3(kThreads), 0, s, p);
  } else {
    if (mode == MODE_FWD) SE3DS_LAUNCH(igemm_bf16_fwd, (igemm_kernel<uint16_t, MODE_FWD>), grid, dim3(kThreads), 0, s, p);
    else SE3DS_LAUNCH(igemm_bf16_dgrad, (igemm_kernel<uint16_t, MODE_DGRAD>), grid, dim3(kThreads), 0, s, p);
  }
  return check_launch(mode == MODE_FWD ? "conv2d_fwd" : "conv2d_dgrad");
}

int se3ds_conv2d_fwd(const void* x, const void* wt, void* y, int dtype, int n, int h, int w,
                     int cin, int ho, int wo, int cout, int kh, int kw, int stride, int pad_t,
                     int pad_l, int wrap_w, const float* in_mask, int in_mask_binary,
                     const float* scale, const float* bias, const float* row_a,
                     const float* row_b, int act, float act_alpha, void* stream) {
  return conv_common(MODE_FWD, x, wt, y, dtype, n, h, w, cin, ho, wo, cout, kh, kw, stride, pad_t,
                     pad_l, wrap_w, in_mask, in_mask_binary, scale, bias, row_a, row_b, act,
                     act_alpha, stream);
}

int64_t se3ds_conv2d_fwd_stats_rows(int dtype, int n, int cin, int ho, int wo, int cout, int kh,
                                    int kw, int stride, int has_in_mask, int in_mask_binary) {
  if (dtype != SE3DS_BF16 || stride < 1 || stride > 2 || (cin % 64) != 0 ||
      (has_in_mask && !in_mask_binary))
    return 0;
  const char* e = getenv("SE3DS_FUSED_BN_STATS");
  const int lvl = e ? atoi(e) : 2;
  if (lvl == 0) return 0;
  IgemmParams p;
  p.N = n; p.oH = ho; p.oW = wo; p.oC = cout; p.stride = stride;
  if (lvl == 1 && !(stride == 1 && kh == 3 && kw == 3 && halo_tile_channels(p))) return 0;
  return fwd_stats_rows(p, dtype, stride, kh, kw, true);
}

int se3ds_conv_transpose2x2_fwd(const void* x, const void* wn, void* y, int dtype, int n, int hi, int wi,
                                int cin, int cout, const float* bias, void* stream) {
  if (cout % 4 != 0) return SE3DS_E_UNSUPPORTED;
  const size_t esz = dtype == SE3DS_F32 ? 4 : 2;
  for (int py = 0; py < 2; ++py) {
    const char* wpy = (const char*)wn + (size_t)py * 2 * cout * cin * esz;
    const int rc = conv_common(MODE_FWD, x, wpy, y, dtype, n, hi, wi, cin, hi, wi, 2 * cout, 1, 1, 1, 0, 0,
                               0, nullptr, 0, nullptr, bias, nullptr, nullptr, 0, 0.f, stream, nullptr,
                               nullptr, nullptr, nullptr, nullptr, nullptr, 0, 0.f, 2 * (int64_t)wi,
                               (int64_t)py * wi, cout);
    if (rc != SE3DS_OK) return rc;
  }
  return SE3DS_OK;
}

int se3ds_conv2d_fwd_stats(const void* x, const void* wt, void* y, int dtype, int n, int h, int w,
                           int cin, int ho, int wo, int cout, int kh, int kw, int stride,
                           int pad_t, int pad_l, int wrap_w, const float* in_mask,
                           int in_mask_binary, const float* scale, const float* bias,
                           const float* row_a, const float* row_b, int act, float act_alpha,
                           float* stats, void* stream) {
  return conv_common(MODE_FWD, x, wt, y, dtype, n, h, w, cin, ho, wo, cout, kh, kw, stride, pad_t,
                     pad_l, wrap_w, in_mask, in_mask_binary, scale, bias, row_a, row_b, act,
                     act_alpha, stream, stats);
}

int se3ds_conv2d_dgrad(const void* dy, const void* wn, void* dx, int dtype, int n, int h, int w,
                       int cin, int ho, int wo, int cout, int kh, int kw, int stride, int pad_t,
                       int pad_l, int wrap_w, const float* dy_row_scale, const float* scale,
                       const float* bias, const float* row_a, int act, float act_alpha,
                       void* stream) {
  return conv_common(MODE_DGRAD, dy, wn, dx, dtype, n, h, w, cin, ho, wo, cout, kh, kw, stride,
                     pad_t, pad_l, wrap_w, dy_row_scale, 0, scale, bias, row_a, nullptr, act,
                     act_alpha, stream);
}

int se3ds_conv2d_dgrad_acc(const void* dy, const void* wn, void* dx, int dtype, int n, int h, int w,
                           int cin, int ho, int wo, int cout, int kh, int kw, int stride, int pad_t,
                           int pad_l, int wrap_w, const float* dy_row_scale, const float* scale,
                           const float* bias, const float* row_a, int act, float act_alpha,
                           const void* addend, void* stream) {
  return conv_common(MODE_DGRAD, dy, wn, dx, dtype, n, h, w, cin, ho, wo, cout, kh, kw, stride,
                     pad_t, pad_l, wrap_w, dy_row_scale, 0, scale, bias, row_a, nullptr, act,
                     act_alpha, stream, nullptr, addend);
}

int64_t se3ds_conv2d_dgrad_bnstats_rows(int dtype, int n, int h, int w, int cin, int cout, int kh,
                                        int kw, int stride, int has_row_scale) {
  if (dtype != SE3DS_BF16 || stride != 1 || (cout % 64) != 0 || (cin % 8) != 0 || has_row_scale)
    return 0;
  IgemmParams p;
  p.N = n; p.oH = h; p.oW = w; p.oC = cin; p.stride = stride;
  return fwd_stats_rows(p, dtype, stride, kh, kw, true, MODE_DGRAD);
}

int se3ds_conv2d_dgrad_bnstats(const void* dy, const void* wn, void* dx, int dtype, int n, int h,
                               int w, int cin, int ho, int wo, int cout, int kh, int kw, int stride,
                               int pad_t, int pad_l, int wrap_w, const float* scale,
                               const float* row_a, const void* addend, const void* bn_x,
                               const uint8_t* bn_mask, const float* bn_mean, const float* bn_rstd,
                               int bn_act, float bn_alpha, float* stats, void* stream) {
  if (stats == nullptr) return SE3DS_E_UNSUPPORTED;
  return conv_common(MODE_DGRAD, dy, wn, dx, dtype, n, h, w, cin, ho, wo, cout, kh, kw, stride,
                     pad_t, pad_l, wrap_w, nullptr, 0, scale, nullptr, row_a, nullptr, 0, 0.f,
                     stream, stats, addend, bn_x, bn_mask, bn_mean, bn_rstd, bn_act, bn_alpha);
}

static int wgrad_splits(int64_t L, int64_t tiles, int64_t nel) {
  const double kStepUs = 2.15, kBytesPerUs = 3.0e6, kSlots = 512.0;
  int best = 1;
  double best_cost = 1e30;
  for (int s = 1; s <= 256; ++s) {
    int64_t per = (L + s - 1) / s;
    if (s > 1 && per < 256) break;
    double steps = (double)((per + 63) / 64);
    double rounds = (double)((tiles * s + (int64_t)kSlots - 1) / (int64_t)kSlots);
    double cost = rounds * steps * kStepUs + (s > 1 ? 5.0 : 0.0) +
                  (double)s * (double)nel * 8.0 / kBytesPerUs * (s > 1 ? 1.0 : 0.5);
    if (cost < best_cost) { best_cost = cost; best = s; }
  }
  return best;
}

static constexpr int wgrad_slots() { return 256; }

static int wgrad_taps_splits(int n, int ho, int wo, int cin, int cout, int kh, int kw, int* steps) {
  if (kh != 3 || kw != 3 || (cin % 64) != 0 || (cout % 128) != 0) return 0;
  const int64_t total = (int64_t)n * ceil_div(ho, 2) * ceil_div(wo, 32);
  if (total > (1 << 30)) return 0;
  *steps = (int)total;
  const int64_t tiles = (int64_t)(cin / 64) * (cout / 128);
  const double kStepUs = 1.3, kBytesPerUs = 3.0e6;
  const int64_t nel = (int64_t)9 * cin * cout;
  int best = 1;
  double best_cost = 1e30;
  for (int s = 1; s <= 512 && s <= total; ++s) {
    const double per = (double)ceil_div(total, (int64_t)s);
    if (s > 1 && per < 8) break;
    const double rounds = (double)ceil_div(tiles * s, (int64_t)wgrad_slots());
    const double cost = rounds * (per * kStepUs + 4.0) +
                        (double)s * (double)nel * 8.0 / kBytesPerUs * (s > 1 ? 1.0 : 0.5);
    if (cost < best_cost) { best_cost = cost; best = s; }
  }
  return best;
}

static bool thin_cin_wgrad_ok(int cin, int cout, int kh, int kw) {
  return cin <= kThinCinMax && cout == 128 && kh * kw * cin <= kThinKMax && kh <= 7 && kw <= 7 &&
         thin_on();
}

size_t se3ds_conv2d_wgrad_workspace_bytes(int n, int ho, int wo, int cin, int cout, int kh,
                                          int kw) {
  int tsteps = 0;
  const int tsplits = wgrad_taps_splits(n, ho, wo, cin, cout, kh, kw, &tsteps);
  const size_t taps_bytes = sizeof(float) * (size_t)tsplits * (size_t)kh * kw * cin * cout + 16;
  int64_t L = (int64_t)n * ho * wo;
  int64_t row_tiles = cin <= 16 ? ceil_div((int64_t)kh * kw * cin, 128)
                                : (int64_t)kh * kw * ceil_div(cin, 128);
  int64_t tiles = row_tiles * ceil_div(cout, 128);
  int splits = wgrad_splits(L, tiles, (int64_t)kh * kw * cin * cout);
  size_t bytes = sizeof(float) * (size_t)splits * (size_t)kh * kw * cin * cout + 16;
  if (thin_cin_wgrad_ok(cin, cout, kh, kw)) {
    const size_t thin = sizeof(float) * (size_t)256 * (size_t)kh * kw * cin * cout + 16;
    bytes = bytes > thin ? bytes : thin;
  }
  return bytes > taps_bytes ? bytes : taps_bytes;
}

int se3ds_conv2d_wgrad(const void* x, const void* dy, float* dw, int dtype, int n, int h, int w,
                       int cin, int ho, int wo, int cout, int kh, int kw, int stride, int pad_t,
                       int pad_l, int wrap_w, const float* in_mask, int in_mask_binary,
                       const float* row_scale, const float* out_scale, int accumulate,
                       void* workspace, size_t workspace_bytes, void* stream) {
  if (n <= 0 || h <= 0 || w <= 0 || cin <= 0 || ho <= 0 || wo <= 0 || cout <= 0 || kh <= 0 ||
      kw <= 0 || stride <= 0)
// ... 55 lines not shown
  p.dw = (float*)workspace;
  p.ci_tiles = (int)ceil_div(cin, 128);
  p.linear_k = cin <= 16 ? 1 : 0;
  const int64_t L = (int64_t)n * ho * wo;
  const int64_t row_tiles = p.linear_k ? ceil_div((int64_t)kh * kw * cin, 128)
                                       : (int64_t)kh * kw * p.ci_tiles;
  const int64_t tiles = row_tiles * ceil_div(cout, 128);
  p.splits = wgrad_splits(L, tiles, (int64_t)kh * kw * cin * cout);
  p.l_per_split = ceil_div(ceil_div(L, p.splits), WG_BL) * WG_BL;
  dim3 grid((unsigned)row_tiles, (unsigned)ceil_div(cout, 128), (unsigned)p.splits);
  const int epc = dtype == SE3DS_F32 ? 4 : 8;
  const bool glds = !p.linear_k && (in_mask == nullptr || in_mask_binary) &&
                    row_scale == nullptr &&
                    (cin % epc) == 0 && (cout % epc) == 0;
  if (glds) {
    p.l_per_split = ceil_div(ceil_div(L, p.splits), 64) * 64;
    if (dtype == SE3DS_F32) SE3DS_LAUNCH(wgrad_glds_f32, wgrad_glds_kernel<float>, grid, dim3(kThreads), 0, s, p);
    else SE3DS_LAUNCH(wgrad_glds_bf16, wgrad_glds_kernel<uint16_t>, grid, dim3(kThreads), 0, s, p);
  } else if (dtype == SE3DS_F32) {
    SE3DS_LAUNCH(wgrad_f32, wgrad_kernel<float>, grid, dim3(kThreads), 0, s, p);
  } else {
    SE3DS_LAUNCH(wgrad_bf16, wgrad_kernel<uint16_t>, grid, dim3(kThreads), 0, s, p);
  }
  const int64_t nel = (int64_t)kh * kw * cin * cout;
  launch_wgrad_reduce((const float*)workspace, p.splits, nel, accumulate, out_scale, dw, s);
  return check_launch("conv2d_wgrad");
}

int se3ds_conv2d_wgrad_partial(const void* x, const void* dy, float* dw, int dtype, int n, int h,
                               int w, int cin, int ho, int wo, int cout, int kh, int kw, int stride,
                               int pad_t, int pad_l, int wrap_w, const float* in_mask,
                               int in_mask_binary, const float* row_scale, void* workspace,
                               size_t workspace_bytes, int64_t* reduce_row, void* stream) {
  if (reduce_row == nullptr) return SE3DS_E_BADSHAPE;
  reduce_row[4] = 0;
  t_defer_row = reduce_row;
  const int rc = se3ds_conv2d_wgrad(x, dy, dw, dtype, n, h, w, cin, ho, wo, cout, kh, kw, stride,
                                    pad_t, pad_l, wrap_w, in_mask, in_mask_binary, row_scale,
                                    nullptr, 0, workspace, workspace_bytes, stream);
  t_defer_row = nullptr;
  return rc;
}

int se3ds_wgrad_reduce_multi(const int64_t* table, int rows, int64_t workgroups, void* stream) {
  if (rows <= 0 || workgroups <= 0) return SE3DS_OK;
  if (workgroups >= ((int64_t)1 << 31)) return SE3DS_E_BADSHAPE;
  SE3DS_LAUNCH(wgrad_reduce_multi, wgrad_reduce_multi_kernel, dim3((unsigned)workgroups), dim3(256),
               0, as_stream(stream), table, rows);
  return check_launch("wgrad_reduce_multi");
}

int se3ds_wgrad_reduce_tile(void) { return kRedTile; }

uint32_t se3ds_fastdiv_host(uint32_t n, uint32_t d) {
  const FastDiv f = make_fastdiv(d);
  const uint32_t t = (uint32_t)(((uint64_t)n * f.m) >> 32);
  return (t + ((n - t) >> f.s1)) >> f.s2;
}

static int wgrad_taps_thin_splits(int n, int h, int w, int cin, int cout, int k, int* steps) {
  if (k != 3 || cout > 8 || (cin % 64) != 0) return 0;
  const int64_t total = (int64_t)n * ceil_div(h, 2) * ceil_div(w, 32);
  if (total > (1 << 30)) return 0;
  *steps = (int)total;
  const int64_t tiles = cin / 64;
  int64_t sp = ceil_div((int64_t)256, tiles);
  if (sp > total / 8) sp = total / 8;
  if (sp < 1) sp = 1;
  return (int)sp;
}

size_t se3ds_conv2d_wgrad_swapped_workspace_bytes(int n, int h, int w, int cin, int cout, int k) {
  const size_t a = se3ds_conv2d_wgrad_workspace_bytes(n, h, w, cout, cin, k, k) +
                   sizeof(float) * (size_t)k * k * cin * cout + 64;
  int steps = 0;
  const int sp = wgrad_taps_thin_splits(n, h, w, cin, cout, k, &steps);
  const size_t b = sp ? (size_t)n * h * w * 16 + 256 + sizeof(float) * (size_t)sp * 9 * cin * cout + 64
                      : 0;
  const size_t c = (k == 3 && cout <= 4) ? sizeof(float) * (size_t)kThinQSlabs * 9 * cin * cout + 64 : 0;
  const size_t ab = a > b ? a : b;
  return ab > c ? ab : c;
}

int se3ds_conv2d_wgrad_swapped(const void* x, const void* dy, float* dw, int dtype, int n, int h,
                               int w, int cin, int cout, int k, int pad, int accumulate,
                               void* workspace, size_t workspace_bytes, void* stream) {
  if (workspace_bytes < se3ds_conv2d_wgrad_swapped_workspace_bytes(n, h, w, cin, cout, k))
    return SE3DS_E_WORKSPACE;
  if (dtype == SE3DS_BF16 && k == 3 && cout <= 4 && (cin % 32) == 0 && cin <= 128 &&
      workspace_bytes >= sizeof(float) * (size_t)kThinQSlabs * 9 * cin * cout &&
      thin_on()) {
    hipStream_t s = as_stream(stream);
    ThinCoutWgradParams q;
    q.x = (const uint16_t*)x; q.dy = (const uint16_t*)dy; q.part = (float*)workspace;
    q.N = n; q.H = h; q.W = w; q.Cin = cin; q.Cout = cout; q.pad = pad;
    const size_t lds = thin_cout_wgrad_lds(cin);
    int64_t blocks = (int64_t)n * ceil_div(h, kThinQRows) * ceil_div(w, kThinCols);
    if (blocks > kThinQSlabs) blocks = kThinQSlabs;
    const int tiles_per_wave = ceil_div(9 * (cin / 32), 8);
#define SE3DS_THIN_CW(M)                                                                          \
  do {                                                                                            \
    static size_t lds_set = 0;                                                                    \
    if (lds > lds_set) {                                                                          \
      if (hipFuncSetAttribute((const void*)thin_cout_wgrad_kernel<M>,                             \
                              hipFuncAttributeMaxDynamicSharedMemorySize, (int)lds) != hipSuccess) \
        return SE3DS_E_LAUNCH;                                                                    \
      lds_set = lds;                                                                              \
    }                                                                                             \
    SE3DS_LAUNCH(thin_cout_wgrad_t##M, thin_cout_wgrad_kernel<M>, dim3((unsigned)blocks),         \
                 dim3(kThinWThreads), lds, s, q);                                                 \
  } while (0)
    switch (tiles_per_wave) {
      case 2: SE3DS_THIN_CW(2); break;
      case 3: SE3DS_THIN_CW(3); break;
      case 4: SE3DS_THIN_CW(4); break;
      default: SE3DS_THIN_CW(5); break;
    }
#undef SE3DS_THIN_CW
    const int64_t tnel = (int64_t)9 * cin * cout;
    launch_wgrad_reduce((const float*)workspace, (int)blocks, tnel, accumulate, nullptr, dw, s);
    return check_launch("conv2d_wgrad(thin cout)");
  }
  if (dtype == SE3DS_BF16) {
    int tsteps = 0;
    const int tsplits = wgrad_taps_thin_splits(n, h, w, cin, cout, k, &tsteps);
    if (tsplits > 0) {
      hipStream_t s = as_stream(stream);
      const int64_t px = (int64_t)n * h * w;
      uint16_t* dyp = (uint16_t*)workspace;
      float* part = (float*)((char*)workspace + ((size_t)px * 16 + 255) / 256 * 256);
      SE3DS_LAUNCH(pad_channels8, pad_channels8_kernel, dim3(grid_for(px, 256)), dim3(256), 0, s,
                   (const uint16_t*)dy, cout, px, dyp);
      WgradTapsParams q;
      q.x = (const uint16_t*)x; q.H = h; q.W = w; q.Cin = cin;
      q.dy = dyp; q.Ho = h; q.Wo = w; q.Cout = cout;
      q.N = n; q.pad_t = pad; q.pad_l = pad; q.wrap_w = 0; q.src_mask = nullptr;
      q.dw = part;
      q.steps_y = ceil_div(h, 2); q.steps_x = ceil_div(w, 32);
      q.total_steps = tsteps;
      q.steps_per_split = ceil_div(tsteps, tsplits);
      q.dy_cstride = 8; q.co_valid = cout;
      dim3 tgrid((unsigned)(cin / 64), 1, (unsigned)tsplits);
      SE3DS_LAUNCH(wgrad_taps_thin, wgrad_taps_kernel, tgrid, dim3(512), 0, s, q);
      const int64_t tnel = (int64_t)9 * cin * cout;
      launch_wgrad_reduce((const float*)part, tsplits, tnel, accumulate, nullptr, dw, s);
      return check_launch("conv2d_wgrad(taps, thin)");
    }
  }
  float* tmp = (float*)workspace;
  const size_t tmp_bytes = (sizeof(float) * (size_t)k * k * cin * cout + 63) / 64 * 64;
  int rc = se3ds_conv2d_wgrad(dy, x, tmp, dtype, n, h, w, cout, h, w, cin, k, k, 1, k - 1 - pad,
                              k - 1 - pad, 0, nullptr, 0, nullptr, nullptr, 0,
                              (char*)workspace + tmp_bytes, workspace_bytes - tmp_bytes, stream);
  if (rc != SE3DS_OK) return rc;
  SE3DS_LAUNCH(wgrad_swap_fixup, wgrad_swap_fixup_kernel,
               dim3(grid_for((int64_t)k * k * cin * cout, 256)), dim3(256), 0, as_stream(stream),
               tmp, k, cin, cout, accumulate, dw);
  return check_launch("conv2d_wgrad_swapped");
}

int se3ds_debug_conv_route_history(int back) {
  if (back < 0 || back >= kRouteRing || (unsigned)back >= t_route_n) return -1;
  return t_route_ring[(t_route_n - 1 - (unsigned)back) % kRouteRing];
}
int se3ds_debug_last_conv_route(void) { return se3ds_debug_conv_route_history(0); }
const char* se3ds_debug_conv_route_name(int route) {
  static const char* const kNames[] = {
#define SE3DS_ROUTE_NAME(name) #name,
      SE3DS_CONV_ROUTES(SE3DS_ROUTE_NAME)
#undef SE3DS_ROUTE_NAME
  };
  return route >= 0 && route < kConvRouteCount ? kNames[route] : nullptr;
}

int se3ds_weight_prep(const float* w, int64_t k, int cout, int dtype, void* wt, void* wn,
                      void* stream) {
  if (k <= 0 || cout <= 0) return SE3DS_E_BADSHAPE;
  dim3 grid((unsigned)ceil_div(k, 32), (unsigned)ceil_div(cout, 32));
  hipStream_t s = as_stream(stream);
  if (dtype == SE3DS_F32)
    SE3DS_LAUNCH(weight_prep_f32, weight_prep_kernel<float>, grid, dim3(256), 0, s, w, k, cout,
                 (float*)wt, (float*)wn);
  else if (dtype == SE3DS_BF16 && (cout % 4) == 0 && (k % 8) == 0 &&
           (((uintptr_t)w | (uintptr_t)wt) & 15) == 0 && (((uintptr_t)wn) & 7) == 0)
    SE3DS_LAUNCH(weight_prep_vec, weight_prep_vec_kernel,
                 dim3((unsigned)ceil_div(k, 64), (unsigned)ceil_div(cout, 64)), dim3(256), 0, s, w,
                 k, cout, (uint16_t*)wt, (uint16_t*)wn);
  else if (dtype == SE3DS_BF16)
    SE3DS_LAUNCH(weight_prep_bf16, weight_prep_kernel<uint16_t>, grid, dim3(256), 0, s, w, k, cout,
                 (uint16_t*)wt, (uint16_t*)wn);
  else
    return SE3DS_E_BADDTYPE;
  return check_launch("weight_prep");
}

}
```

### se3ds_amd/csrc/norm.hip

```cpp
#include "common.h"
#include <type_traits>
#include <cstdlib>

namespace se3ds {
namespace {

struct Layout2D {
  int cx;
  int ry;
  int vec;
  int ctiles;
};
inline Layout2D make_layout(int C, int V) {
  Layout2D l;
  l.vec = (C % V == 0) ? V : 1;
  int cvec = C / l.vec;
  int cx = 1;
  while (cx < cvec && cx < 256) cx <<= 1;
  l.cx = cx;
  l.ry = 256 / cx;
  l.ctiles = (int)ceil_div(cvec, cx);
  return l;
}

// ... 314 lines not shown
    mean_out[c] = mean;
    rstd_out[c] = rstd;
  }
}


template <typename T, int VEC>
__global__ void __launch_bounds__(256)
norm_apply_kernel(const T* __restrict__ x, const float* __restrict__ scale,
                  const float* __restrict__ shift, const T* __restrict__ res,
                  const T* __restrict__ post, int64_t R, int C, int cx, int ry, int act,
                  float alpha, T* __restrict__ y, uint8_t* __restrict__ amask) {
  const int g = blockIdx.z;
  const int tx = threadIdx.x % cx, ty = threadIdx.x / cx;
  const int c0 = (blockIdx.y * cx + tx) * VEC;
  if (c0 >= C) return;
  float sc[VEC], sh[VEC];
#pragma unroll
  for (int e = 0; e < VEC; ++e) {
    sc[e] = scale[(int64_t)g * C + c0 + e];
    sh[e] = shift[(int64_t)g * C + c0 + e];
  }
  for (int64_t r = (int64_t)blockIdx.x * ry + ty; r < R; r += (int64_t)gridDim.x * ry) {
    const int64_t off = ((int64_t)g * R + r) * C + c0;
    float xv[VEC], rv[VEC], pv[VEC], o[VEC];
    if constexpr (VEC > 1) {
      VT<T>::load(x + off, reinterpret_cast<float(&)[VT<T>::V]>(xv));
      if (res) VT<T>::load(res + off, reinterpret_cast<float(&)[VT<T>::V]>(rv));
      if (post) VT<T>::load(post + off, reinterpret_cast<float(&)[VT<T>::V]>(pv));
    } else {
      xv[0] = VT<T>::ld1(x + off);
      if (res) rv[0] = VT<T>::ld1(res + off);
      if (post) pv[0] = VT<T>::ld1(post + off);
    }
#pragma unroll
    for (int e = 0; e < VEC; ++e) {
      float v = xv[e] * sc[e] + sh[e];
      if (res) v += rv[e];
      v = act_apply(v, act, alpha);
      if (post) v += pv[e];
      o[e] = v;
    }
    if constexpr (VEC > 1) VT<T>::store(y + off, reinterpret_cast<float(&)[VT<T>::V]>(o));
    else VT<T>::st1(y + off, o[0]);
    if constexpr (VEC == 8 && sizeof(T) == 2) {
      if (amask) {
        unsigned bits = 0;
#pragma unroll
        for (int e = 0; e < VEC; ++e) {
          const uint16_t hb = f32_to_bf16(o[e]);
          bits |= ((hb & 0x7fffu) != 0 && (hb & 0x8000u) == 0) ? (1u << e) : 0u;
        }
        amask[off >> 3] = (uint8_t)bits;
      }
    }
  }
}

template <int ACT, bool HAS_RES>
__global__ void __launch_bounds__(256)
norm_apply_fast_kernel(const uint16_t* __restrict__ x, const float* __restrict__ scale,
                       const float* __restrict__ shift, const uint16_t* __restrict__ res, int64_t R,
                       int C, int cx, int ry, float alpha, uint16_t* __restrict__ y,
                       uint8_t* __restrict__ amask) {
  typedef uint16_t T;
  constexpr int VEC = 8;
  const int g = blockIdx.z;
  const int tx = threadIdx.x % cx, ty = threadIdx.x / cx;
  const int c0 = (blockIdx.y * cx + tx) * VEC;
  if (c0 >= C) return;
  float sc[VEC], sh[VEC];
  VT<float>::load(scale + (int64_t)g * C + c0, reinterpret_cast<float(&)[4]>(sc[0]));
  VT<float>::load(scale + (int64_t)g * C + c0 + 4, reinterpret_cast<float(&)[4]>(sc[4]));
  VT<float>::load(shift + (int64_t)g * C + c0, reinterpret_cast<float(&)[4]>(sh[0]));
  VT<float>::load(shift + (int64_t)g * C + c0 + 4, reinterpret_cast<float(&)[4]>(sh[4]));
  for (int64_t r = (int64_t)blockIdx.x * ry + ty; r < R; r += (int64_t)gridDim.x * ry) {
    const int64_t off = ((int64_t)g * R + r) * C + c0;
    float xv[VEC], rv[VEC], o[VEC];
    VT<T>::load(x + off, xv);
    if (HAS_RES) VT<T>::load(res + off, rv);
    unsigned bits = 0;
#pragma unroll
    for (int e = 0; e < VEC; ++e) {
      float v = xv[e] * sc[e] + sh[e];
      if (HAS_RES) v += rv[e];
      if (ACT == 1) v = v > 0.f ? v : 0.f;
      if (ACT == 2) v = v > 0.f ? v : v * alpha;
      o[e] = v;
      const uint16_t hb = f32_to_bf16(v);
      bits |= ((hb & 0x7fffu) != 0 && (hb & 0x8000u) == 0) ? (1u << e) : 0u;
    }
    VT<T>::store(y + off, o);
    if (amask) amask[off >> 3] = (uint8_t)bits;
  }
}

template <typename T, int VEC>
__global__ void __launch_bounds__(256)
norm_bwd_apply_kernel(const T* __restrict__ dy, const T* __restrict__ y, const T* __restrict__ x,
                      const float* __restrict__ mean, const float* __restrict__ rstd,
                      const float* __restrict__ gamma, const float* __restrict__ sums, float count,
                      int64_t R, int C, int cx, int ry, int act, float alpha, T* __restrict__ dx,
                      T* __restrict__ dres, const uint8_t* __restrict__ amask, int in_act,
                      float in_alpha) {
  const int g = blockIdx.z;
  const int tx = threadIdx.x % cx, ty = threadIdx.x / cx;
  const int c0 = (blockIdx.y * cx + tx) * VEC;
  if (c0 >= C) return;
  float gr[VEC], k1[VEC], c0k[VEC];
  const float inv_count = 1.0f / count;
#pragma unroll
  for (int e = 0; e < VEC; ++e) {
    const int64_t gc = (int64_t)g * C + c0 + e;
    const float mu = mean[gc], rs = rstd[gc];
    gr[e] = (gamma ? gamma[c0 + e] : 1.0f) * rs;
    const float s0 = sums[((int64_t)g * 2) * C + c0 + e] * inv_count;
    const float s1 = sums[((int64_t)g * 2 + 1) * C + c0 + e] * inv_count;
    k1[e] = gr[e] * rs * s1;
    c0k[e] = mu * k1[e] - gr[e] * s0;
  }
  for (int64_t r = (int64_t)blockIdx.x * ry + ty; r < R; r += (int64_t)gridDim.x * ry) {
    const int64_t off = ((int64_t)g * R + r) * C + c0;
    float dv[VEC], yv[VEC], xv[VEC], o[VEC], dr[VEC];
    const bool use_mask = VEC == 8 && amask != nullptr;
    unsigned mbits = 0;
    if constexpr (VEC > 1) {
      VT<T>::load(dy + off, reinterpret_cast<float(&)[VT<T>::V]>(dv));
      if (act) {
        if (use_mask) mbits = amask[off >> 3];
        else VT<T>::load(y + off, reinterpret_cast<float(&)[VT<T>::V]>(yv));
      }
      VT<T>::load(x + off, reinterpret_cast<float(&)[VT<T>::V]>(xv));
    } else {
      dv[0] = VT<T>::ld1(dy + off);
      if (act) yv[0] = VT<T>::ld1(y + off);
      xv[0] = VT<T>::ld1(x + off);
    }
#pragma unroll
    for (int e = 0; e < VEC; ++e) {
      const float ag = !act ? 1.f
                       : (use_mask ? act_grad_from_bit((mbits >> e) & 1u, act, alpha)
                                   : act_grad_from_out(yv[e], act, alpha));
      float d = dv[e] * ag;
      dr[e] = d;
      o[e] = fmaf(gr[e], d, fmaf(-k1[e], xv[e], c0k[e]));
      if (in_act) o[e] *= act_grad_from_out(xv[e], in_act, in_alpha);
    }
    if constexpr (VEC > 1) {
      VT<T>::store(dx + off, reinterpret_cast<float(&)[VT<T>::V]>(o));
      if (dres) VT<T>::store(dres + off, reinterpret_cast<float(&)[VT<T>::V]>(dr));
    } else {
      VT<T>::st1(dx + off, o[0]);
      if (dres) VT<T>::st1(dres + off, dr[0]);
    }
  }
}

template <int ACT, int IN_ACT, bool ROWS = false, bool PRO = false>
__global__ void __launch_bounds__(256)
norm_bwd_apply_fast_kernel(const uint16_t* __restrict__ dy, const uint16_t* __restrict__ x,
                           const float* __restrict__ mean, const float* __restrict__ rstd,
                           const float* __restrict__ gamma, const float* __restrict__ sums,
                           float count, int64_t R, int C, int cx, int ry, float alpha,
                           uint16_t* __restrict__ dx, uint16_t* __restrict__ dres,
                           const uint8_t* __restrict__ amask, float in_alpha,
                           const float* __restrict__ sum_row = nullptr,
                           const float* __restrict__ out_row = nullptr,
// ... 575 lines not shown
```

### se3ds_amd/hipops/nn.py

```python
import math
import threading
from collections import namedtuple
from types import SimpleNamespace
from typing import List, Optional

import numpy as np
import os

import torch
import torch.distributed as dist

from se3ds_amd import _lib

ACT_NONE, ACT_RELU, ACT_LRELU = 0, 1, 2
BN_EPS, BN_MOMENTUM = 1e-3, 0.99
IN_EPS = 1e-3


def _L():
  return _lib.lib()


def _all_reduce_sum(t, group, kind):
  from se3ds_amd.trainers import dist_utils
# ... 68 lines not shown
        self.grad_views[name] = self._grad[o:o + n].view(shape)
    return self._grad

  def load_dict(self, d):
    for k, v in d.items():
      t = torch.as_tensor(np.asarray(v), dtype=torch.float32).to(self.theta.device)
      self.views[k].copy_(t.reshape(self.views[k].shape))
    self.version += 1

  def to_dict(self):
    return {k: v.detach().cpu().numpy().copy() for k, v in self.views.items()}

  def segments(self, groups):
    if not isinstance(groups, dict):
      groups = {g: (g,) for g in groups}
    out = {}
    for name, prefixes in groups.items():
      idx = [i for i, n in enumerate(self.trainable_names)
             if any(n.startswith(pre + '/') for pre in prefixes)]
      if not idx:
        continue
      assert idx == list(range(idx[0], idx[-1] + 1)), f'{name} is not contiguous'
      o0 = self._off_tr[self.trainable_names[idx[0]]][0]
      last = self._off_tr[self.trainable_names[idx[-1]]]
      out[name] = (idx[0], idx[-1] + 1, o0, last[0] + last[1])
    return out

  def chunk_tables(self, chunk=65536):
    chunks, starts = [], [0]
    for t, name in enumerate(self.trainable_names):
      o, n, _ = self._off_tr[name]
      for s in range(0, n, chunk):
        chunks.append((t, o + s, min(chunk, n - s)))
      starts.append(len(chunks))
    dev = self.theta.device
    return (torch.tensor(chunks, dtype=torch.int64, device=dev).reshape(-1, 3).contiguous(),
            torch.tensor(starts, dtype=torch.int64, device=dev))


class _LazyGradViews(dict):

  def __init__(self, store):
    super().__init__()
    self._store = store

  def __missing__(self, name):
    self._store.grad
    return dict.__getitem__(self, name)


def _gdev(gen):
  return gen.device if gen is not None else torch.device('cpu')


def glorot_uniform(shape, gen):
  rf = int(np.prod(shape[:-2])) if len(shape) > 2 else 1
  fan_in, fan_out = shape[-2] * rf, shape[-1] * rf
  limit = math.sqrt(6.0 / (fan_in + fan_out))
  return (torch.rand(shape, generator=gen, dtype=torch.float32, device=_gdev(gen)) * 2 - 1) * limit


def zeros_init(shape, gen):
  return torch.zeros(shape, dtype=torch.float32, device=_gdev(gen))


def ones_init(shape, gen):
  return torch.ones(shape, dtype=torch.float32, device=_gdev(gen))


def truncated_normal_init(shape, gen, std=0.05):
  dev = _gdev(gen)
  t = torch.randn(shape, generator=gen, dtype=torch.float32, device=dev)
  for _ in range(8):
    bad = t.abs() > 2
    if not bool(bad.any()):
      break
    t = torch.where(bad, torch.randn(shape, generator=gen, dtype=torch.float32, device=dev), t)
  return t.clamp(-2, 2) * std


BnSrc = namedtuple('BnSrc', 'x amask mean rstd act alpha')
BnStats = namedtuple('BnStats', 'rows gver')
RowSink = namedtuple('RowSink', 'out_scale bias_scale bias_grad')


class Var:
  __slots__ = ('data', '_grad', 'gver', 'requires_grad', 'col_stats', 'grad_pre_act', 'shared',
               'grad_ev', 'bn_src', 'bn_stats', 'row_sink', 'grad_scaled')

  def __init__(self, data, requires_grad=True):
    self.data = data
    self._grad = None
    self.gver = 0
    self.bn_src = None
    self.bn_stats = None
    self.row_sink = None
    self.grad_scaled = None
    self.requires_grad = requires_grad
    self.col_stats = None
    self.grad_pre_act = False
    self.shared = False
    self.grad_ev = None

  @property
  def shape(self):
    return self.data.shape

  @property
  def grad(self):
    return self._grad

  @grad.setter
  def grad(self, g):
    self._grad = g
    self.gver += 1

  def take_bn_stats(self):
    s, self.bn_stats = self.bn_stats, None
    return s.rows if s is not None and s.gver == self.gver else None

  def take_grad_scaled(self, who):
    gs = self.grad_scaled
    if gs is not None and gs != self.gver:
      raise RuntimeError(f'{who}: pre-scaled output gradient was modified by a second '
                         'consumer (set SE3DS_FUSED_ROW_SCALE=0)')
    self.grad_scaled = None
    return gs is not None


class Ctx:

  def __init__(self, device, dtype=torch.float32, training=False, record=False,
               group=None, world=None):
    self.device = torch.device(device)
    self.dtype = dtype
    self.code = _lib.dtype_code(torch.empty(0, dtype=dtype))
    self.training = training
    self.tape = [] if record else None
    self.param_grads = True
    self.binary_masks = True
    self.on_segment = None
    self.batch_limit = None
    self.act_taps = None
    self.taps = None
    self.bn_use_moving = False
    self.after_collective = None
    self._mask_cache = {}
    self.streams = None
    self.wgrad_defer = None
    self._tl = threading.local()
    self._forked = set()
    self.pair = None
    self.collectives = 0
    self._bwd_pending = None
    self._cur_paired = False
    self.group = group
    if world is None:
      world = dist.get_world_size(group) if group is not None else 1
    self.world = int(world)
    if group is not None and self.world != dist.get_world_size(group):
      raise ValueError(f'Ctx: world={self.world} does not match the replica group '
                       f'({dist.get_world_size(group)} ranks)')
    if group is None and self.world > 1 and not (dist.is_initialized() and
                                                 dist.get_world_size() == self.world):
      raise ValueError(f'Ctx: world={self.world} without a group needs a default process group '
                       'of that size')
    self._ws = {}

  def ws(self, key, nbytes):
    if self.streams is not None:
      key = (key, torch.cuda.current_stream(self.device).cuda_stream)
    elif self.pair is not None:
      key = (key, self.branch_tag)
    t = self._ws.get(key)
    if t is None or t.numel() < nbytes:
      t = torch.empty((int(nbytes),), dtype=torch.uint8, device=self.device)
      self._ws[key] = t
    return t

  def empty(self, shape, dtype=None):
    return torch.empty(shape, dtype=dtype or self.dtype, device=self.device)

  @property
  def branch_tag(self):
    return getattr(self._tl, 'tag', 0)

  @branch_tag.setter
  def branch_tag(self, tag):
    self._tl.tag = tag
# ... 577 lines not shown
_RED_TABLES = {}


def _wgrad(ctx, layer, args, wsz):
  L = _L()
  if ctx.wgrad_defer is None:
    ws = _global_ws(ctx.device, 'wgrad', wsz)
    _chk(L.se3ds_conv2d_wgrad(*args, None, 0, ws.data_ptr(), ws.numel(), _lib.stream()),
         'se3ds_conv2d_wgrad')
    return
  ws = layer._wgrad_slab
  if ws is None or ws.numel() < wsz:
    ws = torch.empty((int(wsz),), dtype=torch.uint8, device=ctx.device)
    layer._wgrad_slab = ws
    _RED_TABLES.clear()
  row = (_lib.c_i64 * 5)()
  _chk(L.se3ds_conv2d_wgrad_partial(*args, ws.data_ptr(), ws.numel(), row, _lib.stream()),
       'se3ds_conv2d_wgrad_partial')
  if row[4]:
    ctx.wgrad_defer.append((row[0], row[1], row[2], row[3]))


def flush_wgrad_reduces(ctx):
  rows = ctx.wgrad_defer
  if not rows:
    return
  ctx.wgrad_defer = []
  _reduce_rows(ctx, rows)


def reduce_or_defer(ctx, row):
  if ctx.wgrad_defer is not None:
    ctx.wgrad_defer.append(row)
  else:
    _reduce_rows(ctx, [row])


def _reduce_rows(ctx, rows):
  key = (str(ctx.device), tuple(rows))
  ent = _RED_TABLES.get(key)
  if ent is None:
    tile = int(_L().se3ds_wgrad_reduce_tile())
    tab, first = [], 0
    for part, splits, n4, dst in rows:
      tab.append([part, splits, n4, dst, first])
      first += (n4 + tile - 1) // tile
    ent = (torch.tensor(tab, dtype=torch.int64, device=ctx.device), first)
    if len(_RED_TABLES) >= 256:
      _RED_TABLES.clear()
    _RED_TABLES[key] = ent
  with _Timed('wgrad', 0.0, 'split reduce (batched)'):
    _chk(_L().se3ds_wgrad_reduce_multi(ent[0].data_ptr(), len(rows), ent[1], _lib.stream()),
         'se3ds_wgrad_reduce_multi')


_Geom = namedtuple('_Geom', 'code n h w cin ho wo cout kh kw stride pad_t pad_l wrap')

def _partial_masks(ctx, mask, geo, recording):
  _, n, h, w, _, ho, wo, _, k, _, s, pt, pl, wrap = geo
  m = in_mask = mask
  if m is None:
    m = torch.empty((n, h, w), dtype=torch.float32, device=ctx.device)
    _chk(_L().se3ds_fill(m.data_ptr(), _lib.F32, m.numel(), 1.0, _lib.stream()), 'se3ds_fill')
  cache = ctx._mask_cache if mask is not None else None
  key = (m.data_ptr(), tuple(m.shape), k, s, pt, pl, wrap, ho, wo, bool(recording))
  ent = cache.get(key) if cache is not None and _MASK_CACHE else None
  if ent is None:
    ratio, um, ru, bu = mask_window(ctx, m, n, h, w, ho, wo, k, s, pt, pl, wrap, recording)
    if (cache is not None and _MASK_CACHE and ctx.binary_masks and k == 1 and s == 1 and pt == 0 and
        pl == 0):
      um = m
    if cache is not None:
      cache[key] = (ratio, um, ru, bu, m)
  else:
    ratio, um, ru, bu = ent[:4]
  if in_mask is not None and k == 1 and ctx.binary_masks and _DROP_1X1_MASK:
    in_mask = None
  return ratio, um, ru, bu, in_mask


def conv2d(ctx: Ctx, x: Var, layer: ConvLayer, pad=0, wrap=False, mask=None, act=ACT_NONE,
           alpha=0.0):
  assert not layer.transpose
  xd = x.data
  n, h, w, cin = xd.shape
  assert cin == layer.cin, (cin, layer.cin)
  k, s = layer.k, layer.stride
  ho, pt = conv_out_size(h, k, s, layer.padding, pad)
  wo, pl = conv_out_size(w, k, s, layer.padding, pad)
  geo = _Geom(ctx.code, n, h, w, cin, ho, wo, layer.cout, k, k, s, pt, pl,
              1 if (wrap and pad > 0) else 0)
  L = _L()
  wt, wn = layer.operands(ctx)
  partial = layer.kind in ('partial', 'partial_spectral')
  recording = ctx.tape is not None
  ratio, um, ru, bu, in_mask = _partial_masks(ctx, mask, geo, recording) if partial else (None,) * 5
  scale = layer.sn['sig'][1:] if layer.kind == 'spectral' else None
  bias = layer.bias
  y = ctx.empty((n, ho, wo, layer.cout))
  flops = 2.0 * n * ho * wo * cin * layer.cout * k * k
  tag = f'{k}x{k}s{s} {cin}->{layer.cout} @{ho}x{wo} n{n} {layer.kind}'
  stats_rows = 0
  if ctx.training and recording and not ctx.bn_use_moving:
    stats_rows = int(L.se3ds_conv2d_fwd_stats_rows(ctx.code, n, cin, ho, wo, layer.cout, k, k, s,
                                                   1 if in_mask is not None else 0,
                                                   1 if ctx.binary_masks else 0))
  args = (xd.data_ptr(), wt.data_ptr(), y.data_ptr(), *geo, _lib.ptr(in_mask),
          1 if ctx.binary_masks else 0, _lib.ptr(scale), _lib.ptr(bias), _lib.ptr(ratio),
          _lib.ptr(um if (partial and bias is not None) else None), act, float(alpha))
  out = Var(y)
  with _Timed('fwd', flops, tag):
    if stats_rows > 0:
      out.col_stats = torch.empty((stats_rows, 2, layer.cout), dtype=torch.float32, device=ctx.device)
      _chk(L.se3ds_conv2d_fwd_stats(*args, out.col_stats.data_ptr(), _lib.stream()),
           'se3ds_conv2d_fwd_stats')
    else:
      _chk(L.se3ds_conv2d_fwd(*args, _lib.stream()), 'se3ds_conv2d_fwd')
  if act != ACT_NONE and ctx.act_taps is not None:
    ctx.act_taps[layer.name] = y
  if (recording and partial and bias is not None and ctx.binary_masks and act == ACT_NONE and
      layer.cout % 8 == 0 and xd.dtype == torch.bfloat16):
    out.row_sink = RowSink(ru, bu, lambda: layer.store.grad_views[layer.name + '/bias'])
  if recording:
    sv = SimpleNamespace(ctx=ctx, x=x, out=out, layer=layer, geo=geo, act=act, alpha=float(alpha),
                         partial=partial, ratio=ratio, ru=ru, bu=bu, in_mask=in_mask, wn=wn,
                         scale=scale, flops=flops, tag=tag)
    ctx.record(lambda: _conv2d_bwd(sv))
  return (out, um) if partial else out


def _conv2d_bwd(sv):
  ctx, out, layer, geo, L = sv.ctx, sv.out, sv.layer, sv.geo, _L()
  dy = out.grad
  pre_scaled = out.take_grad_scaled(layer.name)
  out.grad = None
  if dy is None:
    return
  lim = ctx.batch_limit
  if lim is not None and lim < geo.n:
    assert not sv.partial and dy.shape[0] == lim and not ctx.param_grads
    geo = geo._replace(n=lim)
  if sv.act != ACT_NONE and not out.grad_pre_act:
    _chk(L.se3ds_act_bwd(dy.data_ptr(), out.data.data_ptr(), ctx.code, dy.numel(), sv.act,
                         sv.alpha, dy.data_ptr(), _lib.stream()), 'se3ds_act_bwd')
  out.grad_pre_act = False
  rows, cout = geo.n * geo.ho * geo.wo, geo.cout
  dys, row_scale, bias_done = dy, None, False
  if sv.partial and pre_scaled:
    bias_done = True
  elif sv.partial:
    row_scale = sv.ru if layer.has_bias else sv.ratio
    if ctx.binary_masks:
      dys = ctx.empty(dy.shape)
      if ctx.param_grads and layer.has_bias and dy.dtype == torch.bfloat16 and cout % 8 == 0:
        sums = torch.empty((1, 2, cout), dtype=torch.float32, device=ctx.device)
        ws = ctx.ws('norm', L.se3ds_norm_workspace_bytes(1, cout))
        _chk(L.se3ds_colsum_row_scale(dy.data_ptr(), ctx.code, rows, cout, sv.bu.data_ptr(),
                                      row_scale.data_ptr(), dys.data_ptr(), sums.data_ptr(),
                                      layer.store.grad_views[layer.name + '/bias'].data_ptr(),
                                      ws.data_ptr(), ws.numel(), _lib.stream()),
             'se3ds_colsum_row_scale')
        bias_done = True
      else:
        _chk(L.se3ds_row_scale(dy.data_ptr(), ctx.code, rows, cout, row_scale.data_ptr(),
                               dys.data_ptr(), _lib.stream()), 'se3ds_row_scale')
      row_scale = None
  if ctx.param_grads:
    _conv2d_bwd_params(sv, geo, dy, dys, row_scale, bias_done)
  if sv.x.requires_grad:
    _conv2d_bwd_input(sv, geo, dys, row_scale, lim)


def _conv2d_bwd_params(sv, geo, dy, dys, row_scale, bias_done):
  ctx, layer, L = sv.ctx, sv.layer, _L()
  _, n, h, w, cin, ho, wo, cout, k, _, s, pt, pl, wrap = geo
  xd, st = sv.x.data, layer.store
  if layer.has_bias and not bias_done:
    _colsum(ctx, dy.data_ptr(), ctx.code, n * ho * wo, cout,
            row_scale=sv.bu if sv.partial else None, out=st.grad_views[layer.name + '/bias'])
  ptrs = (xd.data_ptr(), dys.data_ptr(), st.grad_views[layer.name + '/kernel'].data_ptr())
  if (cout <= 16 and cin > 16 and s == 1 and ho == h and wo == w and pt == pl and not wrap and
      not sv.partial):
    wsz = L.se3ds_conv2d_wgrad_swapped_workspace_bytes(n, h, w, cin, cout, k)
    ws = _global_ws(ctx.device, 'wgrad', wsz)
    with _Timed('wgrad', sv.flops, sv.tag):
      _chk(L.se3ds_conv2d_wgrad_swapped(*ptrs, ctx.code, n, h, w, cin, cout, k, pt, 0, ws.data_ptr(),
                                        ws.numel(), _lib.stream()), 'se3ds_conv2d_wgrad_swapped')
  else:
    wsz = L.se3ds_conv2d_wgrad_workspace_bytes(n, ho, wo, cin, cout, k, k)
    with _Timed('wgrad', sv.flops, sv.tag):
      _wgrad(ctx, layer, (*ptrs, *geo, _lib.ptr(sv.in_mask), 1 if ctx.binary_masks else 0,
                          _lib.ptr(row_scale)), wsz)


def _conv2d_bwd_input(sv, geo, dys, row_scale, lim):
  ctx, x, xd, n, L = sv.ctx, sv.x, sv.x.data, geo.n, _L()
  prev = x.grad
  shape = (n,) + tuple(xd.shape[1:])
  have_prev = prev is not None and tuple(prev.shape) == shape and prev.dtype == xd.dtype
  bn_rows = 0
  if (x.bn_src is not None and row_scale is None and lim is None and _FUSED_BN_BWD and
      (prev is None or have_prev)):
    bn_rows = int(L.se3ds_conv2d_dgrad_bnstats_rows(ctx.code, n, geo.h, geo.w, geo.cin, geo.cout,
                                                    geo.kh, geo.kw, geo.stride, 0))
  if bn_rows > 0:
    stats = torch.empty((bn_rows, 2, geo.cin), dtype=torch.float32, device=ctx.device)
  if have_prev:
    _grad_wait(x)
    dx = prev
  else:
    dx = ctx.empty(shape)
  args = (dys.data_ptr(), sv.wn.data_ptr(), dx.data_ptr(), *geo)
  tail = (_lib.ptr(row_scale), _lib.ptr(sv.scale), None, _lib.ptr(sv.in_mask), ACT_NONE, 0.0)
  with _Timed('dgrad', sv.flops if bn_rows > 0 else sv.flops * n / xd.shape[0], sv.tag):
    if bn_rows > 0:
      bn = x.bn_src
      _chk(L.se3ds_conv2d_dgrad_bnstats(
          *args, _lib.ptr(sv.scale), _lib.ptr(sv.in_mask), prev.data_ptr() if have_prev else None,
          bn.x.data_ptr(), _lib.ptr(bn.amask), bn.mean.data_ptr(), bn.rstd.data_ptr(), bn.act,
          float(bn.alpha), stats.data_ptr(), _lib.stream()), 'se3ds_conv2d_dgrad_bnstats')
    elif have_prev:
      _chk(L.se3ds_conv2d_dgrad_acc(*args, *tail, prev.data_ptr(), _lib.stream()),
           'se3ds_conv2d_dgrad_acc')
    else:
      _chk(L.se3ds_conv2d_dgrad(*args, *tail, _lib.stream()), 'se3ds_conv2d_dgrad')
  if have_prev:
    x.gver += 1
    _grad_mark(x)
  else:
    accumulate(x, dx)
  if bn_rows > 0:
    x.bn_stats = BnStats(stats, x.gver)


def conv_transpose2d(ctx: Ctx, x: Var, layer: ConvLayer):
  assert layer.transpose and layer.stride == 2 and layer.k in (2, 3)
  xd = x.data
  n, hi, wi, cin_t = xd.shape
  assert cin_t == layer.cin
  k = layer.k
  H, W = 2 * hi, 2 * wi
  geo = _Geom(ctx.code, n, H, W, layer.cout, hi, wi, cin_t, k, k, 2, 0, 0, 0)
  L = _L()
  wt, wn = layer.operands(ctx)
  y = ctx.empty((n, H, W, layer.cout))
  bias = layer.bias
  flops = 2.0 * n * hi * wi * cin_t * layer.cout * k * k
  tag = f'convT {k}x{k}s2 {cin_t}->{layer.cout} @{hi}x{wi}->{H}x{W} n{n}'
  with _Timed('convT_fwd', flops, tag):
    if k == 2 and layer.cout % 4 == 0 and _CONVT_2X2:
      _chk(L.se3ds_conv_transpose2x2_fwd(xd.data_ptr(), wn.data_ptr(), y.data_ptr(), ctx.code, n, hi,
                                         wi, cin_t, layer.cout, _lib.ptr(bias), _lib.stream()),
           'se3ds_conv_transpose2x2_fwd')
    else:
      _chk(L.se3ds_conv2d_dgrad(xd.data_ptr(), wn.data_ptr(), y.data_ptr(), *geo, None, None,
                                _lib.ptr(bias), None, ACT_NONE, 0.0, _lib.stream()),
           'se3ds_conv2d_dgrad')
  out = Var(y)
  if ctx.tape is not None:
    def bwd():
      dy = out.grad
      out.grad = None
      if dy is None:
        return
      if ctx.param_grads:
        if bias is not None:
          _colsum(ctx, dy.data_ptr(), ctx.code, n * H * W, layer.cout,
                  out=layer.store.grad_views[layer.name + '/bias'])
        wsz = L.se3ds_conv2d_wgrad_workspace_bytes(n, hi, wi, layer.cout, cin_t, k, k)
        gk = layer.store.grad_views[layer.name + '/kernel']
        with _Timed('convT_wgrad', flops, tag):
          _wgrad(ctx, layer, (dy.data_ptr(), xd.data_ptr(), gk.data_ptr(), *geo, None, 0, None), wsz)
      if x.requires_grad:
        dx = ctx.empty(xd.shape)
        with _Timed('convT_dgrad', flops, tag):
          _chk(L.se3ds_conv2d_fwd(dy.data_ptr(), wt.data_ptr(), dx.data_ptr(), *geo, None, 0, None,
                                  None, None, None, ACT_NONE, 0.0, _lib.stream()), 'se3ds_conv2d_fwd')
        accumulate(x, dx)
    ctx.record(bwd)
  return out


class NormLayer:

  def __init__(self, store: ParamStore, name, c, kind='batch'):
    self.store, self.name, self.c, self.kind = store, name, c, kind
    store.add(name + '/gamma', (c,), ones_init)
    store.add(name + '/beta', (c,), zeros_init)
    if kind == 'batch':
      store.add(name + '/moving_mean', (c,), zeros_init, trainable=False)
      store.add(name + '/moving_variance', (c,), ones_init, trainable=False)
    self._cg_colpart = None


_NORM_DEBUG = {} if os.environ.get('SE3DS_NORM_DEBUG') else None
_FUSED_BN_BWD = os.environ.get('SE3DS_FUSED_BN_BWD', '0') == '1'
_FUSED_ROW_SCALE = os.environ.get('SE3DS_FUSED_ROW_SCALE', '1') != '0'
_NORM_CG = os.environ.get('SE3DS_NORM_CG', '1') != '0'
_CONVT_2X2 = os.environ.get('SE3DS_CONVT_2X2', '1') != '0'
_MASK_CACHE = os.environ.get('SE3DS_MASK_CACHE', '1') != '0'
_DROP_1X1_MASK = os.environ.get('SE3DS_DROP_1X1_MASK', '1') != '0'


def _norm_debug(who, xd, layer):
  if _NORM_DEBUG is not None:
    key = (who, tuple(xd.shape), layer.kind)
    _NORM_DEBUG[key] = _NORM_DEBUG.get(key, 0) + 1


def _norm_stats(ctx, x, layer, g, r, c, use_moving):
  st, L, inst = layer.store, _L(), layer.kind == 'instance'
  scale = torch.empty((g, c), dtype=torch.float32, device=ctx.device)
  shift, mean, rstd = torch.empty_like(scale), torch.empty_like(scale), torch.empty_like(scale)
  count = float(r)
  affine = (st[layer.name + '/gamma'].data_ptr(), st[layer.name + '/beta'].data_ptr(),
            IN_EPS if inst else BN_EPS, BN_MOMENTUM)
  mm = st[layer.name + '/moving_mean'] if not inst else None
  mv = st[layer.name + '/moving_variance'] if not inst else None
  outs = (scale.data_ptr(), shift.data_ptr(), mean.data_ptr(), rstd.data_ptr(), _lib.stream())
  fused = x.col_stats
  fused = fused if fused is not None and not inst and fused.shape[2] == c else None
  if use_moving:
    _chk(L.se3ds_norm_finalize(None, 1.0, g, c, *affine, mm.data_ptr(), mv.data_ptr(), 1, *outs),
         'se3ds_norm_finalize')
  elif fused is not None and ctx.world == 1 and fused.shape[0] <= 2048:
    _chk(L.se3ds_norm_reduce_rows_finalize(fused.data_ptr(), fused.shape[0], c, count, *affine,
                                           mm.data_ptr(), mv.data_ptr(), *outs),
         'se3ds_norm_reduce_rows_finalize')
    x.col_stats = None
  else:
    if fused is not None:
      sums = torch.empty((1, 2, c), dtype=torch.float32, device=ctx.device)
      ws = ctx.ws('norm', L.se3ds_norm_workspace_bytes(max(1, (fused.shape[0] + 511) // 512), c))
      _chk(L.se3ds_norm_reduce_rows(fused.data_ptr(), fused.shape[0], c, sums.data_ptr(),
                                    ws.data_ptr(), ws.numel(), _lib.stream()),
           'se3ds_norm_reduce_rows')
      x.col_stats = None
    else:
      _norm_debug(layer.name, x.data, layer)
      sums = _colsum(ctx, x.data.data_ptr(), ctx.code, r, c, groups=g)
    if not inst and ctx.world > 1:
      ctx.allreduce_sum(sums)
      count = float(r * ctx.world)
    _chk(L.se3ds_norm_finalize(sums.data_ptr(), count, g, c, *affine, _lib.ptr(mm), _lib.ptr(mv), 0,
                               *outs), 'se3ds_norm_finalize')
  return scale, shift, mean, rstd, count


def norm_act(ctx: Ctx, x: Var, layer: NormLayer, act=ACT_NONE, alpha=0.0, res: Var = None,
             post: Var = None, in_act=None) -> Var:
  xd, inst = x.data, layer.kind == 'instance'
  n, h, w, c = xd.shape
  g, r = (n, h * w) if inst else (1, n * h * w)
  use_moving = (not inst) and (not ctx.training or ctx.bn_use_moving)
  scale, shift, mean, rstd, count = _norm_stats(ctx, x, layer, g, r, c, use_moving)
  y = ctx.empty(xd.shape)
  amask = None
  if (ctx.tape is not None and act != ACT_NONE and post is None and c % 8 == 0 and
      xd.dtype == torch.bfloat16):
    amask = torch.empty(xd.numel() // 8, dtype=torch.uint8, device=ctx.device)
  _chk(_L().se3ds_norm_apply(xd.data_ptr(), ctx.code, g, r, c, scale.data_ptr(), shift.data_ptr(),
                             _lib.ptr(res.data if res is not None else None),
                             _lib.ptr(post.data if post is not None else None), act, float(alpha),
                             y.data_ptr(), _lib.ptr(amask), _lib.stream()), 'se3ds_norm_apply')
  out = Var(y)
  if act != ACT_NONE and ctx.act_taps is not None:
    ctx.act_taps[layer.name] = y
  if (ctx.tape is not None and not inst and not use_moving and post is None and c % 8 == 0 and
      xd.dtype == torch.bfloat16 and (act == ACT_NONE or amask is not None)):
    out.bn_src = BnSrc(xd, amask, mean, rstd, act, alpha)
  sync_bwd = (not inst) and ctx.world > 1 and not use_moving
  if ctx.tape is not None:
    sv = SimpleNamespace(ctx=ctx, x=x, out=out, layer=layer, res=res, post=post, act=act,
                         alpha=float(alpha), in_act=in_act, amask=amask, scale=scale, mean=mean,
                         rstd=rstd, gamma=layer.store[layer.name + '/gamma'], count=count, g=g, r=r,
                         c=c, use_moving=use_moving, sync_bwd=sync_bwd)
    ctx.record(lambda: _norm_bwd(sv), sync=sync_bwd)
  return out


def _norm_bwd(sv):
  ctx, out, xd, c, L = sv.ctx, sv.out, sv.x.data, sv.c, _L()
  dy = out.grad
  fused = out.take_bn_stats()
  out.grad = None
  if dy is None:
    if sv.sync_bwd:
      ctx.allreduce_then(torch.zeros((sv.g, 2, c), dtype=torch.float32, device=ctx.device),
                         lambda: None)
    return
  if sv.post is not None:
    raise NotImplementedError
  lim = ctx.batch_limit
  g, shape = sv.g, xd.shape
  if lim is not None and lim < xd.shape[0]:
    assert sv.layer.kind == 'instance' and dy.shape[0] == lim and not ctx.param_grads
    g, shape = lim, (lim,) + tuple(xd.shape[1:])
  ws = ctx.ws('norm', L.se3ds_norm_workspace_bytes(g, c))
  dres = ctx.empty(shape) if sv.res is not None and sv.res.requires_grad else None
  dx = ctx.empty(shape)
  if sv.use_moving:
    _norm_bwd_moving(sv, dy, dx, dres, g, ws)
  elif (_NORM_CG and not sv.sync_bwd and g == 1 and fused is None and lim is None and
        L.se3ds_norm_bwd_cg_supported(ctx.code, sv.r, c, sv.act, 1 if sv.amask is not None else 0,
                                      sv.in_act[0] if sv.in_act else 0)):
    _norm_bwd_cg(sv, dy, dx, dres)
  else:
    _norm_bwd_split(sv, dy, dx, dres, g, ws, fused, lim)


def _norm_deliver(sv, dx, dres, pre_act, scaled=False):
  if pre_act:
    sv.x.grad_pre_act = True
  accumulate(sv.x, dx)
  if scaled:
    sv.x.grad_scaled = sv.x.gver
  if dres is not None:
    accumulate(sv.res, dres)


def _norm_bwd_sums(sv, dy, g, ws, fused):
  ctx, xd, c, L = sv.ctx, sv.x.data, sv.c, _L()
  bs = torch.empty((g, 2, c), dtype=torch.float32, device=ctx.device)
  direct = ctx.param_grads and g == 1
  gv, name = sv.layer.store.grad_views, sv.layer.name
  dst = lambda which: gv[name + which].data_ptr() if direct else None
  if fused is not None and g == 1 and fused.shape[2] == c:
    rows = fused.shape[0]
    rws = ctx.ws('norm', L.se3ds_norm_workspace_bytes(max(1, (rows + 511) // 512), c))
    _chk(L.se3ds_norm_reduce_rows_dst(fused.data_ptr(), rows, c, bs.data_ptr(), dst('/beta'),
                                      dst('/gamma'), rws.data_ptr(), rws.numel(), _lib.stream()),
         'se3ds_norm_reduce_rows_dst')
    _norm_debug('fused-bwd', xd, sv.layer)
  else:
    _chk(L.se3ds_norm_bwd_stats(
        dy.data_ptr(), sv.out.data.data_ptr(), xd.data_ptr(), ctx.code, g, sv.r, c,
        sv.mean.data_ptr(), sv.rstd.data_ptr(), sv.act, sv.alpha, bs.data_ptr(), dst('/beta'),
        dst('/gamma'), _lib.ptr(sv.amask), ws.data_ptr(), ws.numel(), _lib.stream()),
         'se3ds_norm_bwd_stats')
  if ctx.param_grads and not direct:
    tot = _colsum(ctx, bs.data_ptr(), _lib.F32, g, 2 * c)
    gv[name + '/beta'].copy_(tot[0, 0, :c])
    gv[name + '/gamma'].copy_(tot[0, 0, c:])
  return bs


def _norm_bwd_moving(sv, dy, dx, dres, g, ws):
  ctx = sv.ctx
  if ctx.param_grads:
    _norm_bwd_sums(sv, dy, g, ws, None)
  _chk(_L().se3ds_affine_bwd(dy.data_ptr(), sv.out.data.data_ptr(), ctx.code, g, sv.r, sv.c,
                             sv.scale.data_ptr(), sv.act, sv.alpha, dx.data_ptr(), _lib.ptr(dres),
                             _lib.ptr(sv.amask), _lib.stream()), 'se3ds_affine_bwd')
  _norm_deliver(sv, dx, dres, False)


def _norm_bwd_cg(sv, dy, dx, dres):
  ctx, x, layer, r, c, L = sv.ctx, sv.x, sv.layer, sv.r, sv.c, _L()
  sink = x.row_sink
  use_rows = (sink is not None and _FUSED_ROW_SCALE and ctx.param_grads and not sv.in_act and
              x.grad is None)
  cws = ctx.ws('norm_cg', L.se3ds_norm_bwd_cg_workspace_bytes(c))
  colpart, nrows = None, 0
  if use_rows:
    nrows = int(L.se3ds_norm_bwd_cg_col_rows(r, c))
    colpart = layer._cg_colpart
    if colpart is None or colpart.numel() < nrows * c:
      colpart = layer._cg_colpart = torch.empty(nrows * c, dtype=torch.float32, device=ctx.device)
  gv, pg = layer.store.grad_views, ctx.param_grads
  in_a, in_alpha = sv.in_act or (0, 0.0)
  _chk(L.se3ds_norm_bwd_cg(
      dy.data_ptr(), x.data.data_ptr(), ctx.code, r, c, sv.mean.data_ptr(), sv.rstd.data_ptr(),
      sv.gamma.data_ptr(), sv.count, sv.act, sv.alpha, dx.data_ptr(), _lib.ptr(dres),
      _lib.ptr(sv.amask), in_a, float(in_alpha),
      gv[layer.name + '/beta'].data_ptr() if pg else None,
      gv[layer.name + '/gamma'].data_ptr() if pg else None, None,
      sink.bias_scale.data_ptr() if use_rows else None,
      sink.out_scale.data_ptr() if use_rows else None, _lib.ptr(colpart), cws.data_ptr(),
      cws.numel(), _lib.stream()), 'se3ds_norm_bwd_cg')
  _norm_debug('cg', x.data, layer)
  if use_rows:
    _norm_debug('fused-rows', x.data, layer)
    reduce_or_defer(ctx, (colpart.data_ptr(), nrows, c // 4, sink.bias_grad().data_ptr()))
  _norm_deliver(sv, dx, dres, bool(sv.in_act), scaled=use_rows)


def _norm_bwd_split(sv, dy, dx, dres, g, ws, fused, lim):
  ctx, x, xd, c, L = sv.ctx, sv.x, sv.x.data, sv.c, _L()
  bs = _norm_bwd_sums(sv, dy, g, ws, fused)
  shared = (sv.r, c, sv.mean.data_ptr(), sv.rstd.data_ptr(), sv.gamma.data_ptr(), bs.data_ptr(),
            sv.count, sv.act, sv.alpha, dx.data_ptr(), _lib.ptr(dres), _lib.ptr(sv.amask))

  def finish():
    sink, rc = x.row_sink, -5
    if (sink is not None and _FUSED_ROW_SCALE and ctx.param_grads and g == 1 and not sv.in_act and
        x.grad is None and lim is None and xd.dtype == torch.bfloat16):
      cws = ctx.ws('norm_rows', L.se3ds_norm_workspace_bytes(3, c))
      rc = L.se3ds_norm_bwd_apply_rows(
          dy.data_ptr(), xd.data_ptr(), ctx.code, *shared, sink.bias_scale.data_ptr(),
          sink.out_scale.data_ptr(), sink.bias_grad().data_ptr(), cws.data_ptr(), cws.numel(),
          _lib.stream())
      if rc == 0:
        _norm_debug('fused-rows', xd, sv.layer)
      elif rc not in (-5, -3):
        _chk(rc, 'se3ds_norm_bwd_apply_rows')
    if rc != 0:
      in_a, in_alpha = sv.in_act or (0, 0.0)
      _chk(L.se3ds_norm_bwd_apply(dy.data_ptr(), sv.out.data.data_ptr(), xd.data_ptr(), ctx.code,
                                  g, *shared, in_a, float(in_alpha), _lib.stream()),
           'se3ds_norm_bwd_apply')
    _norm_deliver(sv, dx, dres, bool(sv.in_act), scaled=rc == 0)
  if sv.sync_bwd:
    ctx.allreduce_then(bs, finish)
  else:
    finish()


def add(ctx: Ctx, a: Var, b: Var) -> Var:
  y = ctx.empty(a.data.shape)
  _chk(_L().se3ds_add(a.data.data_ptr(), b.data.data_ptr(), ctx.code, y.numel(), y.data_ptr(),
                      _lib.stream()), 'se3ds_add')
  out = Var(y)
  if ctx.tape is not None:
    def bwd():
      dy = out.grad
      out.grad = None
      if dy is None:
        return
      if a.requires_grad and b.requires_grad and a.grad is None and b.grad is None:
        a.grad = dy
        b.grad = dy.clone()
      else:
        accumulate(a, dy)
        accumulate(b, dy if a.grad is not dy else dy.clone())
    ctx.record(bwd)
  return out


def maxpool2x2(ctx: Ctx, x: Var) -> Var:
  xd = x.data
  n, h, w, c = xd.shape
  y = ctx.empty((n, (h + 1) // 2, (w + 1) // 2, c))
  L = _L()
  _chk(L.se3ds_maxpool2x2_fwd(xd.data_ptr(), ctx.code, n, h, w, c, y.data_ptr(), _lib.stream()),
       'se3ds_maxpool2x2_fwd')
  out = Var(y)
  if ctx.tape is not None:
    def bwd():
      dy = out.grad
      out.grad = None
      if dy is None or not x.requires_grad:
        return
      dx = ctx.empty(xd.shape)
      _chk(L.se3ds_maxpool2x2_bwd(dy.data_ptr(), xd.data_ptr(), y.data_ptr(), ctx.code, n, h, w, c,
                                  dx.data_ptr(), _lib.stream()), 'se3ds_maxpool2x2_bwd')
      accumulate(x, dx)
    ctx.record(bwd)
  return out


def maxpool2x2_mask(ctx: Ctx, m: torch.Tensor) -> torch.Tensor:
  n, h, w = m.shape
  y = torch.empty((n, (h + 1) // 2, (w + 1) // 2), dtype=torch.float32, device=m.device)
  _chk(_L().se3ds_maxpool2x2_fwd(m.data_ptr(), _lib.F32, n, h, w, 1, y.data_ptr(), _lib.stream()),
       'se3ds_maxpool2x2_fwd')
  return y


def avgpool3s2(ctx: Ctx, x: Var) -> Var:
  xd = x.data
  n, h, w, c = xd.shape
  y = ctx.empty((n, (h + 1) // 2, (w + 1) // 2, c))
  L = _L()
  _chk(L.se3ds_avgpool3s2_fwd(xd.data_ptr(), ctx.code, n, h, w, c, y.data_ptr(), _lib.stream()),
       'se3ds_avgpool3s2_fwd')
  out = Var(y, x.requires_grad)
  if ctx.tape is not None:
    def bwd(n=n):
      dy = out.grad
      out.grad = None
      if dy is None or not x.requires_grad:
        return
      lim = ctx.batch_limit
      if lim is not None and lim < n:
        assert dy.shape[0] == lim
        n = lim
      dx = ctx.empty((n,) + tuple(xd.shape[1:]))
      _chk(L.se3ds_avgpool3s2_bwd(dy.data_ptr(), ctx.code, n, h, w, c, dx.data_ptr(),
                                  _lib.stream()), 'se3ds_avgpool3s2_bwd')
      accumulate(x, dx)
    ctx.record(bwd)
# ... 50 lines not shown
```

### se3ds_amd/models/image_models.py

```python
import os
from typing import Dict, List, Optional, Tuple

import torch

from se3ds_amd import _lib
from se3ds_amd import constants
from se3ds_amd import gin_lite as gin
from se3ds_amd.hipops import nn
from se3ds_amd.hipops.nn import ACT_LRELU, ACT_NONE, ACT_RELU, Ctx, ParamStore, Var
from se3ds_amd.models import layers


_DUAL_STREAM = os.environ.get('SE3DS_DUAL_STREAM', '1') != '0'
_DUAL_STREAM_DP = os.environ.get('SE3DS_DUAL_STREAM_DP', '0') == '1'


def _conv_layers_of(obj, out=None, seen=None):
  out = [] if out is None else out
  seen = set() if seen is None else seen
  if id(obj) in seen:
    return out
  seen.add(id(obj))
  if isinstance(obj, nn.ConvLayer):
    out.append(obj)
# ... 122 lines not shown
    def agent(nm, cin, cout):
      conv = agent_fn(store, name + '/' + nm, cin, cout, 1, 1, 'SAME', use_bias=False)
      return conv, layers.SyncBatchNormalization(store, name + '/' + nm + '_bn', cout)
    self.agent4, self.agent4_bn = agent('agent4', d * 2, d * 8)
    if resnet_version == '50':
      filters = [6, 4, 3, 3]
    elif resnet_version == '101':
      filters = [23, 4, 3, 3]
    elif resnet_version == '152':
      filters = [36, 8, 3, 3]
    else:
      raise ValueError('resnet_version should be one of ["50", "101", "152"], '
                       f'got {resnet_version} instead.')
    self.deconv1 = layers.ResStackTranspose(store, name + '/deconv1', d * 8, d * 4, filters[0],
                                            strides=1, circular_pad=circular_pad, conv_fn=conv_fn)
    self.deconv2 = layers.ResStackTranspose(store, name + '/deconv2', d * 4, d * 2, filters[1],
                                            strides=2, circular_pad=circular_pad, conv_fn=conv_fn)
    self.deconv3 = layers.ResStackTranspose(store, name + '/deconv3', d * 2, d, filters[2],
                                            strides=2, circular_pad=circular_pad, conv_fn=conv_fn)
    self.deconv4 = layers.ResStackTranspose(store, name + '/deconv4', d, d, filters[3],
                                            strides=2, circular_pad=circular_pad, conv_fn=conv_fn)
    self.agent0, self.agent0_bn = agent('agent0', d, d)
    self.agent1, self.agent1_bn = agent('agent1', d * 4, d)
    self.agent2, self.agent2_bn = agent('agent2', d * 8, d * 2)
    self.agent3, self.agent3_bn = agent('agent3', d * 16, d * 4)
    self.final_conv = layers.ResStackTranspose(store, name + '/final_conv', d, d, 3,
                                               circular_pad=circular_pad)
    self.final_deconv = layers.Conv2DTranspose(store, name + '/final_deconv', d, output_dim, 2, 2,
                                               use_bias=True)

  SEGMENT_BLOCKS = 4

  def segments(self):
    n = self.name
    segs = {n + '_head': (n + '/upc', n + '/agent4', n + '/agent4_bn', n + '/deconv1/upsample')}
    nb, g = len(self.deconv1.block), self.SEGMENT_BLOCKS
    for i in range(0, nb, g):
      segs[f'{n}/deconv1/blocks{i}'] = tuple(f'{n}/deconv1/block{j}' for j in range(i, min(i + g, nb)))
    tail = [n + '/deconv2', n + '/deconv3', n + '/deconv4']
    for k in range(4):
      tail += [f'{n}/agent{k}', f'{n}/agent{k}_bn']
    segs[n + '_tail'] = tuple(tail + [n + '/final_conv', n + '/final_deconv'])
    return segs

  def _agent(self, ctx, conv, bn, x, mask):
    if self.partial_conv:
      y, _ = conv(ctx, x, mask)
    else:
      y = conv(ctx, x)
    return bn(ctx, y, act=ACT_RELU)

  def __call__(self, ctx: Ctx, x: Var, skip: List[Var], masks=None) -> Var:
    if masks is None:
      masks = [None] * len(skip)
    ctx.mark_segment(self.name + '_head')
    out = self.upc_conv(ctx, x)
    out = self.upc_bn(ctx, out, act=ACT_LRELU, alpha=0.2)
    out = nn.upsample2x(ctx, out)
    out = self._agent(ctx, self.agent4, self.agent4_bn, out, None)
    out = self.deconv1(ctx, out, mark=self.name + '/deconv1', group=self.SEGMENT_BLOCKS)
    ctx.mark_segment(self.name + '_tail')
    out = nn.add(ctx, out, self._agent(ctx, self.agent3, self.agent3_bn, skip[3], masks[3]))
    out = self.deconv2(ctx, out)
    out = nn.add(ctx, out, self._agent(ctx, self.agent2, self.agent2_bn, skip[2], masks[2]))
    out = self.deconv3(ctx, out)
    out = nn.add(ctx, out, self._agent(ctx, self.agent1, self.agent1_bn, skip[1], masks[1]))
    out = self.deconv4(ctx, out)
    out = nn.add(ctx, out, self._agent(ctx, self.agent0, self.agent0_bn, skip[0], masks[0]))
    out = self.final_conv(ctx, out)
    return self.final_deconv(ctx, out)


class _Head:

  def __init__(self, store, name, d, out_ch, circular_pad, conv_fn):
    self.bn = [layers.SyncBatchNormalization(store, name + f'/bn{i}', d) for i in range(3)]
    self.pad = layers.PadLayer(1, circular_pad=circular_pad)
    self.conv = [conv_fn(store, name + '/conv0', d, d, 3, 1, 'VALID'),
                 conv_fn(store, name + '/conv1', d, d, 3, 1, 'VALID'),
                 conv_fn(store, name + '/conv2', d, out_ch, 3, 1, 'VALID')]

  def __call__(self, ctx, x):
    for i in range(3):
      x = self.bn[i](ctx, x, in_act=(ACT_LRELU, 0.3) if i > 0 else None)
      x = self.conv[i](ctx, x, pad=self.pad, act=ACT_LRELU if i < 2 else ACT_NONE, alpha=0.3)
    return x


@gin.configurable
class ResNetGenerator(_Model):
  _SEGMENTS = {
      'encoder_head': ('encoder/conv1', 'encoder/bn1'),
      'encoder/stack1': ('encoder/stack1',), 'encoder/stack2': ('encoder/stack2',),
      'encoder/stack3': ('encoder/stack3',), 'encoder/stack4': ('encoder/stack4',),
      'encoder_tail': ('encoder/final_conv', 'encoder/final_bn'),
      'rgb_conv': ('rgb_conv',), 'depth_conv': ('depth_conv',), 'context': ('context',)}

  def __init__(self, image_size: int = 256, gen_dims: int = 96, z_dim: int = 128,
               resnet_version: str = '50', context_layer: str = 'convs',
               conv_mode: str = 'spectral', use_blurred_mask: bool = True, device='cuda',
               seed: Optional[int] = 0, dtype=torch.float32):
    self.hidden_dims = gen_dims
    self.resnet_version = resnet_version
    self.z_dim = z_dim
    self.circular_pad = True
    if context_layer not in ['convs', 'none']:
      raise NotImplementedError
    self.context_layer = context_layer
    self.use_blurred_mask = use_blurred_mask
    conv_fn = layers.SpectralConv if conv_mode == 'spectral' else layers.Conv2D
    self.store = ParamStore()
    d, s = gen_dims, self.store
    cin = 5 if use_blurred_mask else 4
    self.encoder = ResNetEncoder(s, 'encoder', image_size=image_size, in_channels=cin,
                                 hidden_dims=d, resnet_version=resnet_version,
                                 flatten_output=False, circular_pad=True, conv_fn=conv_fn)
    self.decoder = ResNetDecoder(s, 'decoder', output_dim=d, image_size=image_size, hidden_dims=d,
                                 resnet_version=resnet_version, flatten_output=False,
                                 circular_pad=True, conv_fn=conv_fn)
    self.depth_decoder = ResNetDecoder(s, 'depth_decoder', output_dim=d, image_size=image_size,
                                       hidden_dims=d, resnet_version=resnet_version,
                                       flatten_output=False, circular_pad=True, conv_fn=conv_fn)
    self.rgb_conv = _Head(s, 'rgb_conv', d, 3, True, conv_fn)
    self.depth_conv = _Head(s, 'depth_conv', d, 1, True, conv_fn)
    if context_layer == 'convs':
      chans = [d * 4, d * 4, d * 8, d * 4, d * 4]
      self.ctx_bn = [layers.SyncBatchNormalization(s, f'context/bn{i}', chans[i]) for i in range(4)]
      self.ctx_pad = layers.PadLayer(1, circular_pad=True)
      self.ctx_conv = [layers.SpectralConv(s, f'context/conv{i}', chans[i], chans[i + 1], 3, 1,
                                           'VALID') for i in range(4)]
    self.SEGMENTS = dict(self._SEGMENTS)
    self.SEGMENTS.update(self.decoder.segments())
    self.SEGMENTS.update(self.depth_decoder.segments())
    self._finish(device, seed, dtype)

  def forward(self, ctx: Ctx, cond: Dict[str, torch.Tensor]):
    gi, gd = cond['proj_image'], cond['proj_depth']
    gm, bm = cond['proj_mask'], cond['blurred_mask']
    _lib.require_cuda(gi, gd, gm, bm)
    parts = [gi, gd, bm] if self.use_blurred_mask else [gi, gd]
    x = Var(nn.concat_channels(ctx, [p.to(torch.float32) for p in parts]), requires_grad=False)
    n, h, w, _ = x.shape
    mask = gm.to(torch.float32).reshape(n, h, w).contiguous()
    sn_ev = None
    if ctx.streams is not None:
      side = ctx.streams[1]
      side.wait_stream(torch.cuda.current_stream(ctx.device))
      with torch.cuda.stream(side):
        self.spectral.power_iteration(ctx.training)
        sn_ev = torch.cuda.Event()
        sn_ev.record()
    else:
      self.spectral.power_iteration(ctx.training)
    hidden, skip = self.encoder(ctx, x, mask)
    if sn_ev is not None:
      torch.cuda.current_stream(ctx.device).wait_event(sn_ev)
    taps = ctx.taps
    if taps is not None:
      taps.update(b1=skip[0], s1=skip[1], s2=skip[2], s3=skip[3], enc=hidden)
    if self.context_layer == 'convs':
      ctx.mark_segment('context')
      for i in range(4):
        hidden = self.ctx_bn[i](ctx, hidden, in_act=(ACT_LRELU, 0.3) if i > 0 else None)
        hidden = self.ctx_conv[i](ctx, hidden, pad=self.ctx_pad,
                                  act=ACT_LRELU if i < 3 else ACT_NONE, alpha=0.3)
    hh, hw = hidden.shape[1], hidden.shape[2]
    if ctx.streams is not None:
# ... 103 lines not shown
```

### se3ds_amd/models/layers.py

```python
from typing import Optional, Tuple

import torch

from se3ds_amd.hipops import nn
from se3ds_amd.hipops.nn import ACT_LRELU, ACT_NONE, ACT_RELU, ConvLayer, Ctx, NormLayer, Var


class PadLayer:

  def __init__(self, padding: int, circular_pad: bool = False, mode='CONSTANT',
               constant_value=0):
    self.padding = padding
    self.circular_pad = circular_pad
    self.mode = mode
    self.constant_value = constant_value

  def wraps(self, training) -> bool:
    return bool(self.circular_pad and not training)

  def __call__(self, inputs: torch.Tensor, training=None) -> torch.Tensor:
    return nn.pad2d(inputs, self.padding, self.wraps(training), self.mode, self.constant_value)


class PartialConv:
  spectral_norm = False

  def __init__(self, store, name, in_channels, filters, kernel_size, strides=1, padding='VALID',
               use_bias=True):
    kind = 'partial_spectral' if self.spectral_norm else 'partial'
    self.conv = ConvLayer(store, name, in_channels, filters, kernel_size, strides, padding,
                          use_bias, kind)

  def __call__(self, ctx: Ctx, feature: Var, mask: Optional[torch.Tensor] = None,
               pad: Optional[PadLayer] = None) -> Tuple[Var, torch.Tensor]:
    p = pad.padding if pad is not None else 0
    wrap = pad.wraps(ctx.training) if pad is not None else False
    return nn.conv2d(ctx, feature, self.conv, pad=p, wrap=wrap, mask=mask)


class PartialSpectralConv(PartialConv):
  spectral_norm = True


class SpectralConv:

  def __init__(self, store, name, in_channels, filters, kernel_size, strides=1, padding='VALID',
               use_bias=True):
    self.conv = ConvLayer(store, name, in_channels, filters, kernel_size, strides, padding,
                          use_bias, 'spectral')

  def __call__(self, ctx: Ctx, feature: Var, pad: Optional[PadLayer] = None, act=ACT_NONE,
               alpha=0.0) -> Var:
    p = pad.padding if pad is not None else 0
    wrap = pad.wraps(ctx.training) if pad is not None else False
    return nn.conv2d(ctx, feature, self.conv, pad=p, wrap=wrap, act=act, alpha=alpha)


class Conv2D:

  def __init__(self, store, name, in_channels, filters, kernel_size, strides=1, padding='VALID',
               use_bias=True):
    self.conv = ConvLayer(store, name, in_channels, filters, kernel_size, strides, padding,
                          use_bias, 'plain')

  def __call__(self, ctx: Ctx, feature: Var, pad: Optional[PadLayer] = None, act=ACT_NONE,
               alpha=0.0) -> Var:
    p = pad.padding if pad is not None else 0
    wrap = pad.wraps(ctx.training) if pad is not None else False
    return nn.conv2d(ctx, feature, self.conv, pad=p, wrap=wrap, act=act, alpha=alpha)


class Conv2DTranspose:

  def __init__(self, store, name, in_channels, filters, kernel_size, strides=2, use_bias=True):
    self.conv = ConvLayer(store, name, in_channels, filters, kernel_size, strides, 'SAME',
                          use_bias, 'plain', transpose=True)

  def __call__(self, ctx: Ctx, x: Var) -> Var:
    return nn.conv_transpose2d(ctx, x, self.conv)


class SyncBatchNormalization:
  def __init__(self, store, name, channels):
    self.norm = NormLayer(store, name, channels, 'batch')

  def __call__(self, ctx: Ctx, x: Var, act=ACT_NONE, alpha=0.0, res: Var = None,
               in_act=None) -> Var:
    return nn.norm_act(ctx, x, self.norm, act=act, alpha=alpha, res=res, in_act=in_act)


class InstanceNormalization:
  def __init__(self, store, name, channels):
    self.norm = NormLayer(store, name, channels, 'instance')

  def __call__(self, ctx: Ctx, x: Var, act=ACT_NONE, alpha=0.0) -> Var:
    return nn.norm_act(ctx, x, self.norm, act=act, alpha=alpha)


class Bottleneck:

  def __init__(self, store, name, in_channels, filters=128, strides=1, expansion=4,
               downsample=None, circular_pad=False, partial_fn=PartialConv):
    self.conv1 = partial_fn(store, name + '/conv1', in_channels, filters, 1, 1, 'SAME')
    self.bn1 = SyncBatchNormalization(store, name + '/bn1', filters)
    self.pad1 = PadLayer(1, circular_pad=circular_pad)
    self.conv2 = partial_fn(store, name + '/conv2', filters, filters, 3, strides, 'VALID')
    self.bn2 = SyncBatchNormalization(store, name + '/bn2', filters)
    self.conv3 = partial_fn(store, name + '/conv3', filters, expansion * filters, 1, 1, 'SAME')
    self.bn3 = SyncBatchNormalization(store, name + '/bn3', expansion * filters)
    self.downsample = downsample
    if downsample is not None:
      self.ds_norm = SyncBatchNormalization(store, name + '/ds_norm', expansion * filters)

  def __call__(self, ctx: Ctx, x: Var, mask=None):
    out, update_mask = self.conv1(ctx, x, mask)
    out = self.bn1(ctx, out, act=ACT_RELU)
    out, update_mask = self.conv2(ctx, out, update_mask, pad=self.pad1)
    out = self.bn2(ctx, out, act=ACT_RELU)
    out, update_mask = self.conv3(ctx, out, update_mask)
    residual = x
    if self.downsample is not None:
      residual, _ = self.downsample(ctx, x, mask)
      residual = self.ds_norm(ctx, residual)
    out = self.bn3(ctx, out, act=ACT_RELU, res=residual)
    return out, update_mask


class ResStack:

  def __init__(self, store, name, inplanes, planes, blocks, strides=1, expansion=4,
               circular_pad=False, conv_fn=Conv2D):
    partial_fn = PartialSpectralConv if conv_fn is SpectralConv else PartialConv
    downsample = None
    cin = inplanes
    if strides != 1 or inplanes != planes * expansion:
      downsample = partial_fn(store, name + '/downsample', cin, planes * expansion, 1, strides,
                              'SAME', use_bias=False)
    self.blocks = [Bottleneck(store, name + '/block0', cin, planes, strides, expansion, downsample,
                              circular_pad, partial_fn)]
    for i in range(1, blocks):
      self.blocks.append(Bottleneck(store, name + f'/block{i}', planes * expansion, planes,
                                    expansion=expansion, circular_pad=circular_pad,
                                    partial_fn=partial_fn))

  def __call__(self, ctx: Ctx, x: Var, mask=None):
    out, update_mask = self.blocks[0](ctx, x, mask)
    for block in self.blocks[1:]:
      out, update_mask = block(ctx, out, update_mask)
    return out, update_mask


class TransBasicBlock:

  def __init__(self, store, name, inplanes, planes, strides=1, upsample=None, circular_pad=False,
               conv_fn=Conv2D):
    self.pad_a = PadLayer(1, circular_pad=circular_pad)
    self.conv_a = conv_fn(store, name + '/conv_a', inplanes, inplanes, 3, 1, 'VALID',
                          use_bias=False)
    self.bn_a = SyncBatchNormalization(store, name + '/bn_a', inplanes)
    self.transposed = upsample is not None and strides != 1
    if self.transposed:
      self.conv_b = Conv2DTranspose(store, name + '/conv_b', inplanes, planes, 3, strides,
                                    use_bias=False)
    else:
      self.pad_b = PadLayer(1, circular_pad=circular_pad)
      self.conv_b = conv_fn(store, name + '/conv_b', inplanes, planes, 3, strides, 'VALID',
                            use_bias=False)
    self.bn_b = SyncBatchNormalization(store, name + '/bn_b', planes)
    self.upsample = upsample

  def __call__(self, ctx: Ctx, x: Var) -> Var:
# ... 48 lines not shown
```

Before: 41.72 panoramas/sec.

## Fuse BN affine into head convs and emit BN stats from 2x2 transposed conv

Adds pre-affine variants of the thin-Cout forward conv and the swapped wgrad kernel. They apply a BatchNorm scale/shift to bf16 inputs while staging them into LDS, so a separate norm_apply pass over the head activation can be deferred. It also lets the 2x2 transposed conv emit per-column BN statistics through a pitched stats layout, raises the default fused-BN-stats level, and adds a profitability gate for fused dgrad+BN stats. The Python-side head pre-affine and convT-stats paths default to off, so only the stats-level change and the dgrad gate affect the default run. These add template variants and extra per-element FMAs in load paths.

```diff
diff --git a/include/se3ds_hip.h b/include/se3ds_hip.h
--- a/include/se3ds_hip.h
+++ b/include/se3ds_hip.h
@@ -137,6 +137,10 @@
 
 int se3ds_conv_transpose2x2_fwd(const void* x, const void* wn, void* y, int dtype, int n, int hi, int wi,
                                 int cin, int cout, const float* bias, void* stream);
+int64_t se3ds_conv_transpose2x2_fwd_stats_rows(int dtype, int n, int hi, int wi, int cin, int cout);
+int se3ds_conv_transpose2x2_fwd_stats(const void* x, const void* wn, void* y, int dtype, int n, int hi,
+                                      int wi, int cin, int cout, const float* bias, float* stats,
+                                      void* stream);
 
 int64_t se3ds_conv2d_fwd_stats_rows(int dtype, int n, int cin, int ho, int wo, int cout, int kh,
                                     int kw, int stride, int has_in_mask, int in_mask_binary);
@@ -160,6 +164,8 @@
 
 int64_t se3ds_conv2d_dgrad_bnstats_rows(int dtype, int n, int h, int w, int cin, int cout, int kh,
                                         int kw, int stride, int has_row_scale);
+int se3ds_conv2d_dgrad_bn_stats_profitable(int dtype, int n, int h, int w, int cin, int cout, int kh,
+                                           int kw, int stride);
 int se3ds_conv2d_dgrad_bnstats(const void* dy, const void* wn, void* dx, int dtype, int n, int h,
                                int w, int cin, int ho, int wo, int cout, int kh, int kw, int stride,
                                int pad_t, int pad_l, int wrap_w, const float* scale,
@@ -190,6 +196,19 @@
 int se3ds_conv2d_wgrad_swapped(const void* x, const void* dy, float* dw, int dtype, int n, int h,
                                int w, int cin, int cout, int k, int pad, int accumulate,
                                void* workspace, size_t workspace_bytes, void* stream);
+
+int se3ds_conv2d_fwd_preaffine_supported(int dtype, int cin, int cout, int kh, int kw, int stride);
+int se3ds_conv2d_fwd_preaffine(const void* x, const float* pre_scale, const float* pre_shift,
+                               const void* wt, void* y, int dtype, int n, int h, int w, int cin,
+                               int ho, int wo, int cout, int kh, int kw, int stride, int pad_t,
+                               int pad_l, int wrap_w, const float* scale, const float* bias, int act,
+                               float act_alpha, void* stream);
+int se3ds_conv2d_wgrad_swapped_preaffine_supported(int dtype, int cin, int cout, int k);
+int se3ds_conv2d_wgrad_swapped_preaffine(const void* x, const float* pre_scale,
+                                         const float* pre_shift, const void* dy, float* dw, int dtype,
+                                         int n, int h, int w, int cin, int cout, int k, int pad,
+                                         int accumulate, void* workspace, size_t workspace_bytes,
+                                         void* stream);
 
 int se3ds_mask_window(const float* mask, int n, int h, int w, int ho, int wo, int kh, int kw,
                       int stride, int pad_t, int pad_l, int wrap_w, float* ratio, float* um,
diff --git a/se3ds_amd/csrc/common.h b/se3ds_amd/csrc/common.h
--- a/se3ds_amd/csrc/common.h
+++ b/se3ds_amd/csrc/common.h
@@ -76,6 +76,20 @@
   return (uint16_t)(pack2_bf16(f, f) & 0xffffu);
 }
 
+__device__ __forceinline__ float norm_affine(float x, float sc, float sh) {
+  return __builtin_fmaf(x, sc, sh);
+}
+__device__ __forceinline__ uint4 norm_affine_bf16x8(const uint4 v, const float (&sc)[8],
+                                                    const float (&sh)[8]) {
+  const uint32_t q[4] = {v.x, v.y, v.z, v.w};
+  uint32_t o[4];
+#pragma unroll
+  for (int e = 0; e < 4; ++e)
+    o[e] = pack2_bf16(norm_affine(__uint_as_float(q[e] << 16), sc[2 * e], sh[2 * e]),
+                      norm_affine(__uint_as_float(q[e] & 0xffff0000u), sc[2 * e + 1], sh[2 * e + 1]));
+  return make_uint4(o[0], o[1], o[2], o[3]);
+}
+
 __device__ __forceinline__ float wave_sum(float v) {
 #pragma unroll
   for (int o = 32; o > 0; o >>= 1) v += __shfl_xor(v, o, 64);
diff --git a/se3ds_amd/csrc/conv.hip b/se3ds_amd/csrc/conv.hip
--- a/se3ds_amd/csrc/conv.hip
+++ b/se3ds_amd/csrc/conv.hip
@@ -72,12 +72,25 @@
   int bn_act; float bn_alpha;
   int64_t o_pitch, o_off;
   int bias_mod;
+  const float* pre_scale; const float* pre_shift;
 #ifdef SE3DS_PROBE
   int probe;
 #endif
 };
 
 __device__ __forceinline__ int swz(int row, int chunk) { return chunk ^ ((row >> 2) & 3); }
+
+__device__ __forceinline__ void put_col_stats(const IgemmParams& p, float* stats_row, int ch, float s1,
+                                              float s2) {
+  if (p.bias_mod) {
+    const int kx = ch / p.bias_mod, c = ch - kx * p.bias_mod;
+    stats_row[(2 * kx) * p.bias_mod + c] = s1;
+    stats_row[(2 * kx + 1) * p.bias_mod + c] = s2;
+  } else {
+    stats_row[ch] = s1;
+    stats_row[p.oC + ch] = s2;
+  }
+}
 
 __device__ __forceinline__ void pix_of(const IgemmParams& p, int cls, int64_t m, int cH, int cW, int& n,
                                        int& a, int& b) {
@@ -346,8 +359,7 @@
       *reinterpret_cast<float4*>(r2 + 4) = make_float4(bs2[4], bs2[5], bs2[6], bs2[7]);
     }
   } else if (NI == 2 && stats_row != nullptr) {
-    stats_row[co_base + lane] = cs1;
-    stats_row[p.oC + co_base + lane] = cs2;
+    put_col_stats(p, stats_row, co_base + lane, cs1, cs2);
   }
 }
 
@@ -555,8 +567,7 @@
       *reinterpret_cast<float4*>(r2 + 4) = make_float4(bs2[4], bs2[5], bs2[6], bs2[7]);
     }
   } else if (stats_row != nullptr) {
-    stats_row[co_base + lane] = cs1;
-    stats_row[p.oC + co_base + lane] = cs2;
+    put_col_stats(p, stats_row, co_base + lane, cs1, cs2);
   }
 }
 
@@ -3166,6 +3177,7 @@
 struct ThinCoutWgradParams {
   const uint16_t* x; const uint16_t* dy; float* part;
   int N, H, W, Cin, Cout, pad;
+  const float* pre_scale; const float* pre_shift;
 };
 constexpr int kThinQRows = 8, kThinQSlabs = 256;
 __host__ __device__ inline int thin_cw_pixel_bytes(int cin) { return cin * 2 + 32; }
@@ -3173,7 +3185,7 @@
   return (size_t)(kThinQRows + 2) * (kThinCols + 2) * thin_cw_pixel_bytes(cin) +
          (size_t)kThinQRows * kThinCols * 4 * 2;
 }
-template <int MAXT>
+template <int MAXT, bool PRE = false>
 __global__ void __launch_bounds__(kThinWThreads)
 thin_cout_wgrad_kernel(const ThinCoutWgradParams p) {
   typedef __attribute__((address_space(3))) s16x4_t* lds_seg;
@@ -3227,6 +3239,15 @@
     n = (int)nn;
   };
   uint4 nxt[NV];
+  static_assert(NV <= 32, "one bit of `loaded` per chunk");
+  uint32_t loaded = 0;
+  float* pre_lds = reinterpret_cast<float*>(tq_smem + thin_cout_wgrad_lds(Ci));
+  if constexpr (PRE) {
+    for (int i = tid; i < Ci; i += NT) {
+      pre_lds[i] = p.pre_scale[i];
+      pre_lds[Ci + i] = p.pre_shift[i];
+    }
+  }
   constexpr int ND = (PX * 4 + NT - 1) / NT;
   uint16_t nxd[ND];
   const int rowlen = kThinCols * Co;
@@ -3246,14 +3267,17 @@
     const int sy0 = oy0 - p.pad, sx0 = ox0 - p.pad;
     const bool interior = sy0 >= 0 && sy0 + PH <= p.H && sx0 >= 0 && sx0 + PW <= p.W;
     const int64_t base = (((int64_t)n * p.H + sy0) * p.W + sx0) * Ci;
+    loaded = 0;
 #pragma unroll
     for (int u = 0; u < NV; ++u) {
       int pix, c;
       nxt[u] = make_uint4(0u, 0u, 0u, 0u);
       if (chunk_of(u, pix, c)) {
         const int r = pix / PW, q = pix - r * PW;
-        if (interior || ((unsigned)(sy0 + r) < (unsigned)p.H && (unsigned)(sx0 + q) < (unsigned)p.W))
+        if (interior || ((unsigned)(sy0 + r) < (unsigned)p.H && (unsigned)(sx0 + q) < (unsigned)p.W)) {
           nxt[u] = *reinterpret_cast<const uint4*>(p.x + (base + (int64_t)((r * p.W + q) * Ci + c * 8)));
+          if constexpr (PRE) loaded |= 1u << u;
+        }
       }
     }
   };
@@ -3277,10 +3301,22 @@
         dys[c * PX + ry * kThinCols + cx] = nxd[u];
       }
     }
+    float psc[8], psh[8];
+    if constexpr (PRE) {
+      VT<float>::load(pre_lds + fc * 8, reinterpret_cast<float(&)[4]>(psc[0]));
+      VT<float>::load(pre_lds + fc * 8 + 4, reinterpret_cast<float(&)[4]>(psc[4]));
+      VT<float>::load(pre_lds + Ci + fc * 8, reinterpret_cast<float(&)[4]>(psh[0]));
+      VT<float>::load(pre_lds + Ci + fc * 8 + 4, reinterpret_cast<float(&)[4]>(psh[4]));
+    }
 #pragma unroll
     for (int u = 0; u < NV; ++u) {
       int pix, c;
-      if (chunk_of(u, pix, c)) *reinterpret_cast<uint4*>(xs + pix * PB + c * 16) = nxt[u];
+      if (chunk_of(u, pix, c)) {
+        uint4 v = nxt[u];
+        if constexpr (PRE)
+          if ((loaded >> u) & 1u) v = norm_affine_bf16x8(v, psc, psh);
+        *reinterpret_cast<uint4*>(xs + pix * PB + c * 16) = v;
+      }
     }
     __syncthreads();
     if (tile + gridDim.x < n_tiles) fetch(tile + gridDim.x);
@@ -3479,6 +3515,7 @@
   return (size_t)kThinPH * kThinPW * thin_pixel_bytes(cin) + (size_t)(cout + 1) * thin_weight_bytes(cin);
 }
 
+template <bool PRE>
 __global__ void __launch_bounds__(256)
 thin_cout_fwd_kernel(const IgemmParams p) {
   extern __shared__ __attribute__((aligned(16))) unsigned char t_smem[];
@@ -3516,12 +3553,22 @@
     n = (int)nn;
   };
   uint4 nxt[NV];
+  static_assert(NV <= 32, "one bit of `loaded` per chunk");
+  uint32_t loaded = 0;
+  float psc[8], psh[8];
+  if constexpr (PRE) {
+    VT<float>::load(p.pre_scale + fc * 8, reinterpret_cast<float(&)[4]>(psc[0]));
+    VT<float>::load(p.pre_scale + fc * 8 + 4, reinterpret_cast<float(&)[4]>(psc[4]));
+    VT<float>::load(p.pre_shift + fc * 8, reinterpret_cast<float(&)[4]>(psh[0]));
+    VT<float>::load(p.pre_shift + fc * 8 + 4, reinterpret_cast<float(&)[4]>(psh[4]));
+  }
   auto fetch = [&](int64_t tile) {
     int n, oy0, ox0;
     tile_pos((uint32_t)tile, n, oy0, ox0);
     const int sy0 = oy0 - p.pad_t, sx0 = ox0 - p.pad_l;
     const bool interior = sy0 >= 0 && sy0 + kThinPH <= p.sH && sx0 >= 0 && sx0 + kThinPW <= p.sW;
     const int64_t rowbase = ((int64_t)n * p.sH + sy0) * p.sW;
+    loaded = 0;
 #pragma unroll
     for (int u = 0; u < NV; ++u) {
       const int pix = fp0 + u * fpp;
@@ -3531,12 +3578,15 @@
         if (interior) {
           nxt[u] = *reinterpret_cast<const uint4*>(
               src + ((rowbase + sx0) * C + (int64_t)((r * p.sW + q) * C + fc * 8)));
+          if constexpr (PRE) loaded |= 1u << u;
         } else {
           int sx = sx0 + q;
           if (p.wrap_w) sx = sx < 0 ? sx + p.sW : (sx >= p.sW ? sx - p.sW : sx);
-          if ((unsigned)(sy0 + r) < (unsigned)p.sH && (unsigned)sx < (unsigned)p.sW)
+          if ((unsigned)(sy0 + r) < (unsigned)p.sH && (unsigned)sx < (unsigned)p.sW) {
             nxt[u] = *reinterpret_cast<const uint4*>(
                 src + ((rowbase + (int64_t)r * p.sW + sx) * C + fc * 8));
+            if constexpr (PRE) loaded |= 1u << u;
+          }
         }
       }
     }
@@ -3549,7 +3599,12 @@
 #pragma unroll
   for (int u = 0; u < NV; ++u) {
     const int pix = fp0 + u * fpp;
-    if (pix < kThinPH * kThinPW) *reinterpret_cast<uint4*>(xs + pix * pstride + fc * 16) = nxt[u];
+    if (pix < kThinPH * kThinPW) {
+      uint4 v = nxt[u];
+      if constexpr (PRE)
+        if ((loaded >> u) & 1u) v = norm_affine_bf16x8(v, psc, psh);
+      *reinterpret_cast<uint4*>(xs + pix * pstride + fc * 16) = v;
+    }
   }
   __syncthreads();
   if (tile + gridDim.x < n_tiles) fetch(tile + gridDim.x);
@@ -3797,7 +3852,8 @@
                        const void* bn_x = nullptr, const uint8_t* bn_mask = nullptr,
                        const float* bn_mean = nullptr, const float* bn_rstd = nullptr,
                        int bn_act = 0, float bn_alpha = 0.f, int64_t o_pitch = 0, int64_t o_off = 0,
-                       int bias_mod = 0) {
+                       int bias_mod = 0, const float* pre_scale = nullptr,
+                       const float* pre_shift = nullptr) {
   if (n <= 0 || h <= 0 || wdt <= 0 || cin <= 0 || ho <= 0 || wo <= 0 || cout <= 0 || kh <= 0 ||
       kw <= 0 || stride <= 0 || stride > 2)
     return SE3DS_E_BADSHAPE;
@@ -3824,6 +3880,7 @@
   p.o_pitch = o_pitch > 0 ? o_pitch : p.oW;
   p.o_off = o_off;
   p.bias_mod = bias_mod;
+  p.pre_scale = pre_scale; p.pre_shift = pre_shift;
   const bool pitched = o_pitch > 0 || bias_mod > 0;
 #ifdef SE3DS_PROBE
   { const char* e = getenv("SE3DS_PROBE_MODE"); p.probe = e ? atoi(e) : 0; }
@@ -3882,16 +3939,22 @@
     const size_t lds = thin_lds_bytes(cin, cout);
     static size_t lds_set = 0;
     if (lds > lds_set) {
-      if (hipFuncSetAttribute((const void*)thin_cout_fwd_kernel,
+      if (hipFuncSetAttribute((const void*)thin_cout_fwd_kernel<false>,
+                              hipFuncAttributeMaxDynamicSharedMemorySize, (int)lds) != hipSuccess ||
+          hipFuncSetAttribute((const void*)thin_cout_fwd_kernel<true>,
                               hipFuncAttributeMaxDynamicSharedMemorySize, (int)lds) != hipSuccess)
         return SE3DS_E_LAUNCH;
       lds_set = lds;
     }
     int64_t blocks = (int64_t)p.N * ceil_div(p.oH, kThinRows) * ceil_div(p.oW, kThinCols);
     if (blocks > 2 * 256) blocks = 2 * 256;
-    SE3DS_LAUNCH(thin_cout_fwd, thin_cout_fwd_kernel, dim3((unsigned)blocks), dim3(256), lds, s, p);
+    if (pre_scale != nullptr)
+      SE3DS_LAUNCH(thin_cout_fwd, thin_cout_fwd_kernel<true>, dim3((unsigned)blocks), dim3(256), lds, s, p);
+    else
+      SE3DS_LAUNCH(thin_cout_fwd, thin_cout_fwd_kernel<false>, dim3((unsigned)blocks), dim3(256), lds, s, p);
     return check_launch("conv2d_fwd(thin)");
   }
+  if (pre_scale != nullptr) return SE3DS_E_UNSUPPORTED;
   if (glds && dtype == SE3DS_BF16 && stride == 1 && kh == 3 && kw == 3) {
     const int co = halo_tile_channels(p);
     if (co) {
@@ -3983,13 +4046,32 @@
                      act_alpha, stream);
 }
 
+int se3ds_conv2d_fwd_preaffine_supported(int dtype, int cin, int cout, int kh, int kw, int stride) {
+  return dtype == SE3DS_BF16 && kh == 3 && kw == 3 && stride == 1 && cout <= 4 && (cin % 64) == 0 &&
+         cin <= 128 && thin_on();
+}
+
+int se3ds_conv2d_fwd_preaffine(const void* x, const float* pre_scale, const float* pre_shift,
+                               const void* wt, void* y, int dtype, int n, int h, int w, int cin,
+                               int ho, int wo, int cout, int kh, int kw, int stride, int pad_t,
+                               int pad_l, int wrap_w, const float* scale, const float* bias, int act,
+                               float act_alpha, void* stream) {
+  if (pre_scale == nullptr || pre_shift == nullptr ||
+      !se3ds_conv2d_fwd_preaffine_supported(dtype, cin, cout, kh, kw, stride))
+    return SE3DS_E_UNSUPPORTED;
+  return conv_common(MODE_FWD, x, wt, y, dtype, n, h, w, cin, ho, wo, cout, kh, kw, stride, pad_t,
+                     pad_l, wrap_w, nullptr, 0, scale, bias, nullptr, nullptr, act, act_alpha, stream,
+                     nullptr, nullptr, nullptr, nullptr, nullptr, nullptr, 0, 0.f, 0, 0, 0, pre_scale,
+                     pre_shift);
+}
+
 int64_t se3ds_conv2d_fwd_stats_rows(int dtype, int n, int cin, int ho, int wo, int cout, int kh,
                                     int kw, int stride, int has_in_mask, int in_mask_binary) {
   if (dtype != SE3DS_BF16 || stride < 1 || stride > 2 || (cin % 64) != 0 ||
       (has_in_mask && !in_mask_binary))
     return 0;
   const char* e = getenv("SE3DS_FUSED_BN_STATS");
-  const int lvl = e ? atoi(e) : 2;
+  const int lvl = e ? atoi(e) : 3;
   if (lvl == 0) return 0;
   IgemmParams p;
   p.N = n; p.oH = ho; p.oW = wo; p.oC = cout; p.stride = stride;
@@ -3997,19 +4079,46 @@
   return fwd_stats_rows(p, dtype, stride, kh, kw, true);
 }
 
-int se3ds_conv_transpose2x2_fwd(const void* x, const void* wn, void* y, int dtype, int n, int hi, int wi,
-                                int cin, int cout, const float* bias, void* stream) {
+static int64_t convt2x2_launch_rows(int dtype, int n, int hi, int wi, int cin, int cout) {
+  if (dtype != SE3DS_BF16 || (cin % 64) != 0 || (cout % 64) != 0) return 0;
+  IgemmParams p;
+  p.N = n; p.oH = hi; p.oW = wi; p.oC = 2 * cout; p.stride = 1;
+  return fwd_stats_rows(p, dtype, 1, 1, 1, true);
+}
+
+static int convt2x2_fwd(const void* x, const void* wn, void* y, int dtype, int n, int hi, int wi, int cin,
+                        int cout, const float* bias, float* stats, int64_t launch_rows, void* stream) {
   if (cout % 4 != 0) return SE3DS_E_UNSUPPORTED;
   const size_t esz = dtype == SE3DS_F32 ? 4 : 2;
   for (int py = 0; py < 2; ++py) {
     const char* wpy = (const char*)wn + (size_t)py * 2 * cout * cin * esz;
+    float* spy = stats ? stats + (int64_t)py * launch_rows * 2 * (2 * cout) : nullptr;
     const int rc = conv_common(MODE_FWD, x, wpy, y, dtype, n, hi, wi, cin, hi, wi, 2 * cout, 1, 1, 1, 0, 0,
-                               0, nullptr, 0, nullptr, bias, nullptr, nullptr, 0, 0.f, stream, nullptr,
+                               0, nullptr, 0, nullptr, bias, nullptr, nullptr, 0, 0.f, stream, spy,
                                nullptr, nullptr, nullptr, nullptr, nullptr, 0, 0.f, 2 * (int64_t)wi,
                                (int64_t)py * wi, cout);
     if (rc != SE3DS_OK) return rc;
   }
   return SE3DS_OK;
+}
+
+int se3ds_conv_transpose2x2_fwd(const void* x, const void* wn, void* y, int dtype, int n, int hi, int wi,
+                                int cin, int cout, const float* bias, void* stream) {
+  return convt2x2_fwd(x, wn, y, dtype, n, hi, wi, cin, cout, bias, nullptr, 0, stream);
+}
+
+int64_t se3ds_conv_transpose2x2_fwd_stats_rows(int dtype, int n, int hi, int wi, int cin, int cout) {
+  const char* e = getenv("SE3DS_FUSED_BN_STATS");
+  if ((e ? atoi(e) : 3) < 3) return 0;
+  return 4 * convt2x2_launch_rows(dtype, n, hi, wi, cin, cout);
+}
+
+int se3ds_conv_transpose2x2_fwd_stats(const void* x, const void* wn, void* y, int dtype, int n, int hi,
+                                      int wi, int cin, int cout, const float* bias, float* stats,
+                                      void* stream) {
+  const int64_t rows = convt2x2_launch_rows(dtype, n, hi, wi, cin, cout);
+  if (stats == nullptr || rows <= 0) return SE3DS_E_UNSUPPORTED;
+  return convt2x2_fwd(x, wn, y, dtype, n, hi, wi, cin, cout, bias, stats, rows, stream);
 }
 
 int se3ds_conv2d_fwd_stats(const void* x, const void* wt, void* y, int dtype, int n, int h, int w,
@@ -4050,6 +4159,17 @@
   IgemmParams p;
   p.N = n; p.oH = h; p.oW = w; p.oC = cin; p.stride = stride;
   return fwd_stats_rows(p, dtype, stride, kh, kw, true, MODE_DGRAD);
+}
+
+#ifndef SE3DS_DGRAD_BN_STATS_HEADS
+#define SE3DS_DGRAD_BN_STATS_HEADS 0
+#endif
+int se3ds_conv2d_dgrad_bn_stats_profitable(int dtype, int n, int h, int w, int cin, int cout, int kh,
+                                           int kw, int stride) {
+  if (se3ds_conv2d_dgrad_bnstats_rows(dtype, n, h, w, cin, cout, kh, kw, stride, 0) <= 0) return 0;
+  const bool heads = cin == 128 && cout == 128 && kh == 3 && kw == 3 && stride == 1 &&
+                     (int64_t)n * h * w >= ((int64_t)1 << 21);
+  return (SE3DS_DGRAD_BN_STATS_HEADS != 0 && heads) ? 1 : 0;
 }
 
 int se3ds_conv2d_dgrad_bnstats(const void* dy, const void* wn, void* dx, int dtype, int n, int h,
@@ -4271,11 +4391,20 @@
   return ab > c ? ab : c;
 }
 
-int se3ds_conv2d_wgrad_swapped(const void* x, const void* dy, float* dw, int dtype, int n, int h,
-                               int w, int cin, int cout, int k, int pad, int accumulate,
-                               void* workspace, size_t workspace_bytes, void* stream) {
+int se3ds_conv2d_wgrad_swapped_preaffine_supported(int dtype, int cin, int cout, int k) {
+  return dtype == SE3DS_BF16 && k == 3 && cout <= 4 && (cin == 32 || cin == 64 || cin == 128) &&
+         thin_on();
+}
+
+static int wgrad_swapped(const void* x, const float* pre_scale, const float* pre_shift,
+                         const void* dy, float* dw, int dtype, int n, int h, int w, int cin, int cout,
+                         int k, int pad, int accumulate, void* workspace, size_t workspace_bytes,
+                         void* stream) {
   if (workspace_bytes < se3ds_conv2d_wgrad_swapped_workspace_bytes(n, h, w, cin, cout, k))
     return SE3DS_E_WORKSPACE;
+  const bool pre = pre_scale != nullptr;
+  if (pre && !se3ds_conv2d_wgrad_swapped_preaffine_supported(dtype, cin, cout, k))
+    return SE3DS_E_UNSUPPORTED;
   if (dtype == SE3DS_BF16 && k == 3 && cout <= 4 && (cin % 32) == 0 && cin <= 128 &&
       workspace_bytes >= sizeof(float) * (size_t)kThinQSlabs * 9 * cin * cout &&
       thin_on()) {
@@ -4283,21 +4412,29 @@
     ThinCoutWgradParams q;
     q.x = (const uint16_t*)x; q.dy = (const uint16_t*)dy; q.part = (float*)workspace;
     q.N = n; q.H = h; q.W = w; q.Cin = cin; q.Cout = cout; q.pad = pad;
-    const size_t lds = thin_cout_wgrad_lds(cin);
+    q.pre_scale = pre_scale; q.pre_shift = pre_shift;
+    const size_t lds = thin_cout_wgrad_lds(cin) + (pre ? sizeof(float) * 2 * cin : 0);
     int64_t blocks = (int64_t)n * ceil_div(h, kThinQRows) * ceil_div(w, kThinCols);
     if (blocks > kThinQSlabs) blocks = kThinQSlabs;
     const int tiles_per_wave = ceil_div(9 * (cin / 32), 8);
 #define SE3DS_THIN_CW(M)                                                                          \
   do {                                                                                            \
     static size_t lds_set = 0;                                                                    \
-    if (lds > lds_set) {                                                                          \
-      if (hipFuncSetAttribute((const void*)thin_cout_wgrad_kernel<M>,                             \
-                              hipFuncAttributeMaxDynamicSharedMemorySize, (int)lds) != hipSuccess) \
+    if (lds > lds_set) {    \
+      const int both = (int)(thin_cout_wgrad_lds(cin) + sizeof(float) * 2 * cin);                 \
+      if (hipFuncSetAttribute((const void*)thin_cout_wgrad_kernel<M, false>,                      \
+                              hipFuncAttributeMaxDynamicSharedMemorySize, both) != hipSuccess ||  \
+          hipFuncSetAttribute((const void*)thin_cout_wgrad_kernel<M, true>,                       \
+                              hipFuncAttributeMaxDynamicSharedMemorySize, both) != hipSuccess)    \
         return SE3DS_E_LAUNCH;                                                                    \
-      lds_set = lds;                                                                              \
+      lds_set = (size_t)both;                                                                     \
     }                                                                                             \
-    SE3DS_LAUNCH(thin_cout_wgrad_t##M, thin_cout_wgrad_kernel<M>, dim3((unsigned)blocks),         \
-                 dim3(kThinWThreads), lds, s, q);                                                 \
+    if (pre)                                                                                      \
+      SE3DS_LAUNCH(thin_cout_wgrad_t##M, (thin_cout_wgrad_kernel<M, true>), dim3((unsigned)blocks), \
+                   dim3(kThinWThreads), lds, s, q);                                               \
+    else                                                                                          \
+      SE3DS_LAUNCH(thin_cout_wgrad_t##M, (thin_cout_wgrad_kernel<M, false>), dim3((unsigned)blocks), \
+                   dim3(kThinWThreads), lds, s, q);                                               \
   } while (0)
     switch (tiles_per_wave) {
       case 2: SE3DS_THIN_CW(2); break;
@@ -4310,6 +4447,7 @@
     launch_wgrad_reduce((const float*)workspace, (int)blocks, tnel, accumulate, nullptr, dw, s);
     return check_launch("conv2d_wgrad(thin cout)");
   }
+  if (pre) return SE3DS_E_UNSUPPORTED;
   if (dtype == SE3DS_BF16) {
     int tsteps = 0;
     const int tsplits = wgrad_taps_thin_splits(n, h, w, cin, cout, k, &tsteps);
@@ -4348,6 +4486,23 @@
   return check_launch("conv2d_wgrad_swapped");
 }
 
+int se3ds_conv2d_wgrad_swapped(const void* x, const void* dy, float* dw, int dtype, int n, int h,
+                               int w, int cin, int cout, int k, int pad, int accumulate,
+                               void* workspace, size_t workspace_bytes, void* stream) {
+  return wgrad_swapped(x, nullptr, nullptr, dy, dw, dtype, n, h, w, cin, cout, k, pad, accumulate,
+                       workspace, workspace_bytes, stream);
+}
+
+int se3ds_conv2d_wgrad_swapped_preaffine(const void* x, const float* pre_scale,
+                                         const float* pre_shift, const void* dy, float* dw, int dtype,
+                                         int n, int h, int w, int cin, int cout, int k, int pad,
+                                         int accumulate, void* workspace, size_t workspace_bytes,
+                                         void* stream) {
+  if (pre_scale == nullptr || pre_shift == nullptr) return SE3DS_E_UNSUPPORTED;
+  return wgrad_swapped(x, pre_scale, pre_shift, dy, dw, dtype, n, h, w, cin, cout, k, pad, accumulate,
+                       workspace, workspace_bytes, stream);
+}
+
 int se3ds_debug_conv_route_history(int back) {
   if (back < 0 || back >= kRouteRing || (unsigned)back >= t_route_n) return -1;
   return t_route_ring[(t_route_n - 1 - (unsigned)back) % kRouteRing];
diff --git a/se3ds_amd/csrc/norm.hip b/se3ds_amd/csrc/norm.hip
--- a/se3ds_amd/csrc/norm.hip
+++ b/se3ds_amd/csrc/norm.hip
@@ -420,7 +420,7 @@
     unsigned bits = 0;
 #pragma unroll
     for (int e = 0; e < VEC; ++e) {
-      float v = xv[e] * sc[e] + sh[e];
+      float v = norm_affine(xv[e], sc[e], sh[e]);
       if (HAS_RES) v += rv[e];
       if (ACT == 1) v = v > 0.f ? v : 0.f;
       if (ACT == 2) v = v > 0.f ? v : v * alpha;
diff --git a/se3ds_amd/hipops/nn.py b/se3ds_amd/hipops/nn.py
--- a/se3ds_amd/hipops/nn.py
+++ b/se3ds_amd/hipops/nn.py
@@ -174,14 +174,16 @@
 BnSrc = namedtuple('BnSrc', 'x amask mean rstd act alpha')
 BnStats = namedtuple('BnStats', 'rows gver')
 RowSink = namedtuple('RowSink', 'out_scale bias_scale bias_grad')
+PreAffine = namedtuple('PreAffine', 'scale shift apply')
 
 
 class Var:
-  __slots__ = ('data', '_grad', 'gver', 'requires_grad', 'col_stats', 'grad_pre_act', 'shared',
-               'grad_ev', 'bn_src', 'bn_stats', 'row_sink', 'grad_scaled')
-
-  def __init__(self, data, requires_grad=True):
-    self.data = data
+  __slots__ = ('_data', '_grad', 'gver', 'requires_grad', 'col_stats', 'grad_pre_act', 'shared',
+               'grad_ev', 'bn_src', 'bn_stats', 'row_sink', 'grad_scaled', 'pre_affine')
+
+  def __init__(self, data, requires_grad=True, pre_affine=None):
+    self._data = data
+    self.pre_affine = pre_affine
     self._grad = None
     self.gver = 0
     self.bn_src = None
@@ -195,8 +197,19 @@
     self.grad_ev = None
 
   @property
+  def data(self):
+    pre = self.pre_affine
+    if pre is not None:
+      self._data, self.pre_affine = pre.apply(), None
+    return self._data
+
+  @property
+  def raw(self):
+    return self._data
+
+  @property
   def shape(self):
-    return self.data.shape
+    return self._data.shape
 
   @property
   def grad(self):
@@ -940,15 +953,20 @@
 def conv2d(ctx: Ctx, x: Var, layer: ConvLayer, pad=0, wrap=False, mask=None, act=ACT_NONE,
            alpha=0.0):
   assert not layer.transpose
-  xd = x.data
-  n, h, w, cin = xd.shape
+  n, h, w, cin = x.shape
   assert cin == layer.cin, (cin, layer.cin)
   k, s = layer.k, layer.stride
+  L = _L()
+  pre = x.pre_affine
+  if pre is not None and not (
+      mask is None and layer.kind in ('plain', 'spectral') and pre.scale.shape[0] == 1 and
+      L.se3ds_conv2d_fwd_preaffine_supported(ctx.code, cin, layer.cout, k, k, s)):
+    pre = None
+  xd = x.raw if pre is not None else x.data
   ho, pt = conv_out_size(h, k, s, layer.padding, pad)
   wo, pl = conv_out_size(w, k, s, layer.padding, pad)
   geo = _Geom(ctx.code, n, h, w, cin, ho, wo, layer.cout, k, k, s, pt, pl,
               1 if (wrap and pad > 0) else 0)
-  L = _L()
   wt, wn = layer.operands(ctx)
   partial = layer.kind in ('partial', 'partial_spectral')
   recording = ctx.tape is not None
@@ -968,7 +986,12 @@
           _lib.ptr(um if (partial and bias is not None) else None), act, float(alpha))
   out = Var(y)
   with _Timed('fwd', flops, tag):
-    if stats_rows > 0:
+    if pre is not None:
+      _chk(L.se3ds_conv2d_fwd_preaffine(xd.data_ptr(), pre.scale.data_ptr(), pre.shift.data_ptr(),
+                                        wt.data_ptr(), y.data_ptr(), *geo, _lib.ptr(scale),
+                                        _lib.ptr(bias), act, float(alpha), _lib.stream()),
+           'se3ds_conv2d_fwd_preaffine')
+    elif stats_rows > 0:
       out.col_stats = torch.empty((stats_rows, 2, layer.cout), dtype=torch.float32, device=ctx.device)
       _chk(L.se3ds_conv2d_fwd_stats(*args, out.col_stats.data_ptr(), _lib.stream()),
            'se3ds_conv2d_fwd_stats')
@@ -982,7 +1005,7 @@
   if recording:
     sv = SimpleNamespace(ctx=ctx, x=x, out=out, layer=layer, geo=geo, act=act, alpha=float(alpha),
                          partial=partial, ratio=ratio, ru=ru, bu=bu, in_mask=in_mask, wn=wn,
-                         scale=scale, flops=flops, tag=tag)
+                         scale=scale, flops=flops, tag=tag, pre=pre)
     ctx.record(lambda: _conv2d_bwd(sv))
   return (out, um) if partial else out
 
@@ -1032,18 +1055,29 @@
 def _conv2d_bwd_params(sv, geo, dy, dys, row_scale, bias_done):
   ctx, layer, L = sv.ctx, sv.layer, _L()
   _, n, h, w, cin, ho, wo, cout, k, _, s, pt, pl, wrap = geo
-  xd, st = sv.x.data, layer.store
+  st = layer.store
   if layer.has_bias and not bias_done:
     _colsum(ctx, dy.data_ptr(), ctx.code, n * ho * wo, cout,
             row_scale=sv.bu if sv.partial else None, out=st.grad_views[layer.name + '/bias'])
+  swapped = (cout <= 16 and cin > 16 and s == 1 and ho == h and wo == w and pt == pl and not wrap and
+             not sv.partial)
+  pre = sv.pre if sv.pre is not None and sv.x.pre_affine is sv.pre else None
+  if pre is not None and not (
+      swapped and L.se3ds_conv2d_wgrad_swapped_preaffine_supported(ctx.code, cin, cout, k)):
+    pre = None
+  xd = sv.x.raw if pre is not None else sv.x.data
   ptrs = (xd.data_ptr(), dys.data_ptr(), st.grad_views[layer.name + '/kernel'].data_ptr())
-  if (cout <= 16 and cin > 16 and s == 1 and ho == h and wo == w and pt == pl and not wrap and
-      not sv.partial):
+  if swapped:
     wsz = L.se3ds_conv2d_wgrad_swapped_workspace_bytes(n, h, w, cin, cout, k)
     ws = _global_ws(ctx.device, 'wgrad', wsz)
+    tail = (ctx.code, n, h, w, cin, cout, k, pt, 0, ws.data_ptr(), ws.numel(), _lib.stream())
     with _Timed('wgrad', sv.flops, sv.tag):
-      _chk(L.se3ds_conv2d_wgrad_swapped(*ptrs, ctx.code, n, h, w, cin, cout, k, pt, 0, ws.data_ptr(),
-                                        ws.numel(), _lib.stream()), 'se3ds_conv2d_wgrad_swapped')
+      if pre is not None:
+        _chk(L.se3ds_conv2d_wgrad_swapped_preaffine(ptrs[0], pre.scale.data_ptr(),
+                                                    pre.shift.data_ptr(), *ptrs[1:], *tail),
+             'se3ds_conv2d_wgrad_swapped_preaffine')
+      else:
+        _chk(L.se3ds_conv2d_wgrad_swapped(*ptrs, *tail), 'se3ds_conv2d_wgrad_swapped')
   else:
     wsz = L.se3ds_conv2d_wgrad_workspace_bytes(n, ho, wo, cin, cout, k, k)
     with _Timed('wgrad', sv.flops, sv.tag):
@@ -1052,15 +1086,15 @@
 
 
 def _conv2d_bwd_input(sv, geo, dys, row_scale, lim):
-  ctx, x, xd, n, L = sv.ctx, sv.x, sv.x.data, geo.n, _L()
+  ctx, x, xd, n, L = sv.ctx, sv.x, sv.x.raw, geo.n, _L()
   prev = x.grad
   shape = (n,) + tuple(xd.shape[1:])
   have_prev = prev is not None and tuple(prev.shape) == shape and prev.dtype == xd.dtype
   bn_rows = 0
-  if (x.bn_src is not None and row_scale is None and lim is None and _FUSED_BN_BWD and
-      (prev is None or have_prev)):
-    bn_rows = int(L.se3ds_conv2d_dgrad_bnstats_rows(ctx.code, n, geo.h, geo.w, geo.cin, geo.cout,
-                                                    geo.kh, geo.kw, geo.stride, 0))
+  if (x.bn_src is not None and row_scale is None and lim is None and (prev is None or have_prev)):
+    layer_key = (ctx.code, n, geo.h, geo.w, geo.cin, geo.cout, geo.kh, geo.kw, geo.stride)
+    if _FUSED_BN_BWD or L.se3ds_conv2d_dgrad_bn_stats_profitable(*layer_key):
+      bn_rows = int(L.se3ds_conv2d_dgrad_bnstats_rows(*layer_key, 0))
   if bn_rows > 0:
     stats = torch.empty((bn_rows, 2, geo.cin), dtype=torch.float32, device=ctx.device)
   if have_prev:
@@ -1105,16 +1139,25 @@
   bias = layer.bias
   flops = 2.0 * n * hi * wi * cin_t * layer.cout * k * k
   tag = f'convT {k}x{k}s2 {cin_t}->{layer.cout} @{hi}x{wi}->{H}x{W} n{n}'
+  out = Var(y)
   with _Timed('convT_fwd', flops, tag):
     if k == 2 and layer.cout % 4 == 0 and _CONVT_2X2:
-      _chk(L.se3ds_conv_transpose2x2_fwd(xd.data_ptr(), wn.data_ptr(), y.data_ptr(), ctx.code, n, hi,
-                                         wi, cin_t, layer.cout, _lib.ptr(bias), _lib.stream()),
-           'se3ds_conv_transpose2x2_fwd')
+      args = (xd.data_ptr(), wn.data_ptr(), y.data_ptr(), ctx.code, n, hi, wi, cin_t, layer.cout,
+              _lib.ptr(bias))
+      stats_rows = 0
+      if CONVT_STATS and ctx.training and ctx.tape is not None and not ctx.bn_use_moving:
+        stats_rows = int(L.se3ds_conv_transpose2x2_fwd_stats_rows(*args[3:9]))
+      if stats_rows > 0:
+        out.col_stats = torch.empty((stats_rows, 2, layer.cout), dtype=torch.float32,
+                                    device=ctx.device)
+        _chk(L.se3ds_conv_transpose2x2_fwd_stats(*args, out.col_stats.data_ptr(), _lib.stream()),
+             'se3ds_conv_transpose2x2_fwd_stats')
+      else:
+        _chk(L.se3ds_conv_transpose2x2_fwd(*args, _lib.stream()), 'se3ds_conv_transpose2x2_fwd')
     else:
       _chk(L.se3ds_conv2d_dgrad(xd.data_ptr(), wn.data_ptr(), y.data_ptr(), *geo, None, None,
                                 _lib.ptr(bias), None, ACT_NONE, 0.0, _lib.stream()),
            'se3ds_conv2d_dgrad')
-  out = Var(y)
   if ctx.tape is not None:
     def bwd():
       dy = out.grad
@@ -1205,25 +1248,36 @@
   return scale, shift, mean, rstd, count
 
 
+HEAD_PREAFFINE = False
+CONVT_STATS = False
+
+
 def norm_act(ctx: Ctx, x: Var, layer: NormLayer, act=ACT_NONE, alpha=0.0, res: Var = None,
-             post: Var = None, in_act=None) -> Var:
+             post: Var = None, in_act=None, defer_apply=False) -> Var:
   xd, inst = x.data, layer.kind == 'instance'
   n, h, w, c = xd.shape
   g, r = (n, h * w) if inst else (1, n * h * w)
   use_moving = (not inst) and (not ctx.training or ctx.bn_use_moving)
   scale, shift, mean, rstd, count = _norm_stats(ctx, x, layer, g, r, c, use_moving)
-  y = ctx.empty(xd.shape)
   amask = None
   if (ctx.tape is not None and act != ACT_NONE and post is None and c % 8 == 0 and
       xd.dtype == torch.bfloat16):
     amask = torch.empty(xd.numel() // 8, dtype=torch.uint8, device=ctx.device)
-  _chk(_L().se3ds_norm_apply(xd.data_ptr(), ctx.code, g, r, c, scale.data_ptr(), shift.data_ptr(),
-                             _lib.ptr(res.data if res is not None else None),
-                             _lib.ptr(post.data if post is not None else None), act, float(alpha),
-                             y.data_ptr(), _lib.ptr(amask), _lib.stream()), 'se3ds_norm_apply')
-  out = Var(y)
+
+  def apply():
+    y = ctx.empty(xd.shape)
+    _chk(_L().se3ds_norm_apply(xd.data_ptr(), ctx.code, g, r, c, scale.data_ptr(), shift.data_ptr(),
+                               _lib.ptr(res.data if res is not None else None),
+                               _lib.ptr(post.data if post is not None else None), act, float(alpha),
+                               y.data_ptr(), _lib.ptr(amask), _lib.stream()), 'se3ds_norm_apply')
+    return y
+  if (defer_apply and HEAD_PREAFFINE and act == ACT_NONE and res is None and post is None and
+      xd.dtype == torch.bfloat16 and not (use_moving and ctx.tape is not None)):
+    out = Var(xd, pre_affine=PreAffine(scale, shift, apply))
+  else:
+    out = Var(apply())
   if act != ACT_NONE and ctx.act_taps is not None:
-    ctx.act_taps[layer.name] = y
+    ctx.act_taps[layer.name] = out.data
   if (ctx.tape is not None and not inst and not use_moving and post is None and c % 8 == 0 and
       xd.dtype == torch.bfloat16 and (act == ACT_NONE or amask is not None)):
     out.bn_src = BnSrc(xd, amask, mean, rstd, act, alpha)
@@ -1277,6 +1331,10 @@
     accumulate(sv.res, dres)
 
 
+def _norm_y_ptr(sv):
+  return sv.out.raw.data_ptr()
+
+
 def _norm_bwd_sums(sv, dy, g, ws, fused):
   ctx, xd, c, L = sv.ctx, sv.x.data, sv.c, _L()
   bs = torch.empty((g, 2, c), dtype=torch.float32, device=ctx.device)
@@ -1292,7 +1350,7 @@
     _norm_debug('fused-bwd', xd, sv.layer)
   else:
     _chk(L.se3ds_norm_bwd_stats(
-        dy.data_ptr(), sv.out.data.data_ptr(), xd.data_ptr(), ctx.code, g, sv.r, c,
+        dy.data_ptr(), _norm_y_ptr(sv), xd.data_ptr(), ctx.code, g, sv.r, c,
         sv.mean.data_ptr(), sv.rstd.data_ptr(), sv.act, sv.alpha, bs.data_ptr(), dst('/beta'),
         dst('/gamma'), _lib.ptr(sv.amask), ws.data_ptr(), ws.numel(), _lib.stream()),
          'se3ds_norm_bwd_stats')
@@ -1364,7 +1422,7 @@
         _chk(rc, 'se3ds_norm_bwd_apply_rows')
     if rc != 0:
       in_a, in_alpha = sv.in_act or (0, 0.0)
-      _chk(L.se3ds_norm_bwd_apply(dy.data_ptr(), sv.out.data.data_ptr(), xd.data_ptr(), ctx.code,
+      _chk(L.se3ds_norm_bwd_apply(dy.data_ptr(), _norm_y_ptr(sv), xd.data_ptr(), ctx.code,
                                   g, *shared, in_a, float(in_alpha), _lib.stream()),
            'se3ds_norm_bwd_apply')
     _norm_deliver(sv, dx, dres, bool(sv.in_act), scaled=rc == 0)
diff --git a/se3ds_amd/models/image_models.py b/se3ds_amd/models/image_models.py
--- a/se3ds_amd/models/image_models.py
+++ b/se3ds_amd/models/image_models.py
@@ -228,7 +228,7 @@
 
   def __call__(self, ctx, x):
     for i in range(3):
-      x = self.bn[i](ctx, x, in_act=(ACT_LRELU, 0.3) if i > 0 else None)
+      x = self.bn[i](ctx, x, in_act=(ACT_LRELU, 0.3) if i > 0 else None, defer_apply=i == 2)
       x = self.conv[i](ctx, x, pad=self.pad, act=ACT_LRELU if i < 2 else ACT_NONE, alpha=0.3)
     return x
 
diff --git a/se3ds_amd/models/layers.py b/se3ds_amd/models/layers.py
--- a/se3ds_amd/models/layers.py
+++ b/se3ds_amd/models/layers.py
@@ -85,8 +85,9 @@
     self.norm = NormLayer(store, name, channels, 'batch')
 
   def __call__(self, ctx: Ctx, x: Var, act=ACT_NONE, alpha=0.0, res: Var = None,
-               in_act=None) -> Var:
-    return nn.norm_act(ctx, x, self.norm, act=act, alpha=alpha, res=res, in_act=in_act)
+               in_act=None, defer_apply=False) -> Var:
+    return nn.norm_act(ctx, x, self.norm, act=act, alpha=alpha, res=res, in_act=in_act,
+                       defer_apply=defer_apply)
 
 
 class InstanceNormalization:
```

Result: no change. 41.67 panoramas/sec (-0.1%).
